# Luckick/EAGCN

Hardware: AMD Instinct MI355X
Metric: molecules/sec fwd+bwd, 2-layer 5-view EAGCN, Tox21 batch (higher is better)
Workload: dtype f32 (bf16x3 split, fp32 accumulate): every fp32 operand leaves its producer as three bf16 planes, six v_mfma_f32_32x32x16_bf16 piece products per 16 k rebuild the fp32 product (csrc/gemm_bx3.hip); aggregation, BatchNorm, head, first layer fp32

## Files before the change

### eagcn_amd/build.py

```python
import os
import shutil
import subprocess
import sys
from concurrent.futures import ThreadPoolExecutor

HERE = os.path.dirname(os.path.abspath(__file__))
CSRC = os.path.join(HERE, 'csrc')
LIBDIR = os.path.join(HERE, 'lib')
LIB = os.path.join(LIBDIR, 'libeagcn_hip.so')
HIP_SOURCES = ['index.hip', 'gemm.hip', 'gemm3.hip', 'gemm_bx3.hip', 'gemm_bx3w.hip', 'agg.hip', 'lagg.hip', 'lagg_in.hip', 'gat.hip', 'pool.hip', 'layer.hip', 'readout.hip', 'head.hip', 'head2.hip', 'loss.hip', 'attr.hip']
CPP_SOURCES = ['api.cpp']
HEADERS = ['common.h', 'kernels.h', 'lagg_kernel.h', 'gemm_x6.h', 'bx3.h', os.path.join('..', '..', 'include', 'eagcn_hip.h')]
ARCH = 'gfx950'


def _hipcc():
    for cand in (shutil.which('hipcc'), '/opt/rocm/bin/hipcc'):
        if cand and os.path.exists(cand):
            return cand
    raise RuntimeError('hipcc not found: the EAGCN HIP library cannot be built')


def _newest(paths):
    return max(os.path.getmtime(p) for p in paths)


def needs_build():
    srcs = [os.path.join(CSRC, s) for s in HIP_SOURCES + CPP_SOURCES + HEADERS if os.path.exists(os.path.join(CSRC, s))]
    return (not os.path.exists(LIB)) or os.path.getmtime(LIB) < _newest(srcs)


def build_library(force=False, verbose=False):
    if not force and not needs_build():
        return LIB
    hipcc = _hipcc()
    os.makedirs(LIBDIR, exist_ok=True)
    objdir = os.path.join(LIBDIR, 'obj')
    os.makedirs(objdir, exist_ok=True)
    flags = ['--offload-arch=' + ARCH, '-O3', '-std=c++17', '-fPIC', '-Wall', '-Wno-unused-function', '-munsafe-fp-atomics']

    hdr_time = _newest([os.path.join(CSRC, h) for h in HEADERS if os.path.exists(os.path.join(CSRC, h))])

    def compile_one(src):
        obj = os.path.join(objdir, os.path.splitext(src)[0] + '.o')
        if not force and os.path.exists(obj) and os.path.getmtime(obj) > max(hdr_time, os.path.getmtime(os.path.join(CSRC, src))):
            return obj
        cmd = [hipcc] + flags + ['-c', os.path.join(CSRC, src), '-o', obj]
        if src.endswith('.cpp'):
            cmd = [hipcc, '-O2', '-std=c++17', '-fPIC', '-c', os.path.join(CSRC, src), '-o', obj]
        r = subprocess.run(cmd, capture_output=True, text=True)
        if r.returncode != 0:
            raise RuntimeError('hipcc failed on %s:\n%s\n%s' % (src, r.stdout, r.stderr))
        if verbose and r.stderr.strip():
            print(r.stderr, file=sys.stderr)
        return obj

    sources = [s for s in HIP_SOURCES + CPP_SOURCES if os.path.exists(os.path.join(CSRC, s))]
    with ThreadPoolExecutor(max_workers=min(8, len(sources))) as ex:
        objs = list(ex.map(compile_one, sources))
    tmp = LIB + '.tmp'
    r = subprocess.run([hipcc, '--offload-arch=' + ARCH, '-shared', '-fPIC', '-o', tmp] + objs,
                       capture_output=True, text=True)
    if r.returncode != 0:
        raise RuntimeError('link failed:\n%s\n%s' % (r.stdout, r.stderr))
    os.replace(tmp, LIB)
    return LIB


if __name__ == '__main__':
    print(build_library(force='--force' in sys.argv, verbose=True))
```

### eagcn_amd/csrc/common.h

```cpp
#pragma once
#include <hip/hip_runtime.h>
#include <stdint.h>
#include <stdio.h>
#include <string.h>

#include "../../include/eagcn_hip.h"

namespace eagcn {

constexpr float TINY = 1e-9f;
constexpr int WAVE = 64;

void set_error(const char* fmt, ...);

#define EAGCN_CHECK_ARG(cond, ...)                 \
    do {                                           \
        if (!(cond)) {                             \
            ::eagcn::set_error(__VA_ARGS__);       \
            return EAGCN_ERR_ARG;                  \
        }                                          \
    } while (0)

#define EAGCN_HIP(call)                                                                   \
    do {                                                                                  \
        hipError_t e_ = (call);                                                           \
        if (e_ != hipSuccess) {                                                           \
            ::eagcn::set_error("%s:%d: %s -> %s", __FILE__, __LINE__, #call,              \
                               hipGetErrorString(e_));                                    \
            return EAGCN_ERR_HIP;                                                         \
        }                                                                                 \
    } while (0)

#define EAGCN_LAUNCH_CHECK() EAGCN_HIP(hipGetLastError())

inline int pad16(int w) { return (w + 15) & ~15; }
inline int pad4(int w) { return (w + 3) & ~3; }
inline int cdiv(int a, int b) { return (a + b - 1) / b; }
inline size_t align256(size_t x) { return (x + 255) & ~size_t(255); }

typedef float f32x4 __attribute__((ext_vector_type(4)));

__device__ __forceinline__ float sigmoidf_(float x) { return 1.0f / (1.0f + __expf(-x)); }

__device__ __forceinline__ float wave_sum(float v) {
#pragma unroll
    for (int o = 32; o > 0; o >>= 1) v += __shfl_xor(v, o);
    return v;
}
__device__ __forceinline__ double wave_sum(double v) {
#pragma unroll
    for (int o = 32; o > 0; o >>= 1) v += __shfl_xor(v, o);
    return v;
}
__device__ __forceinline__ int wave_sum(int v) {
#pragma unroll
    for (int o = 32; o > 0; o >>= 1) v += __shfl_xor(v, o);
    return v;
}
__device__ __forceinline__ int wave_max(int v) {
#pragma unroll
    for (int o = 32; o > 0; o >>= 1) v = max(v, __shfl_xor(v, o));
    return v;
}

constexpr int DOT_U = 10;
__device__ __forceinline__ float dot16(const float* __restrict__ a, const float* __restrict__ b, int sl, int n) {
    float acc = 0.0f;
    for (int c0 = sl; c0 < n; c0 += 16 * DOT_U) {
        float x[DOT_U], y[DOT_U];
#pragma unroll
        for (int u = 0; u < DOT_U; ++u) {
            const int c = c0 + 16 * u;
            const bool ok = c < n;
            x[u] = ok ? a[c] : 0.0f;
            y[u] = ok ? b[c] : 0.0f;
        }
#pragma unroll
        for (int u = 0; u < DOT_U; ++u) acc += x[u] * y[u];
    }
    return acc;
}

__device__ __forceinline__ void dot16x4(const float* __restrict__ a, const float* const (&p)[4], int sl, int n,
                                        float (&out)[4]) {
    out[0] = out[1] = out[2] = out[3] = 0.0f;
    constexpr int U = 5;
    for (int c0 = sl; c0 < n; c0 += 16 * U) {
        float x[U], y[4][U];
#pragma unroll
        for (int u = 0; u < U; ++u) {
            const int c = c0 + 16 * u;
            const bool ok = c < n;
            x[u] = ok ? a[c] : 0.0f;
#pragma unroll
            for (int h = 0; h < 4; ++h) y[h][u] = ok ? p[h][c] : 0.0f;
        }
#pragma unroll
        for (int u = 0; u < U; ++u)
#pragma unroll
            for (int h = 0; h < 4; ++h) out[h] += x[u] * y[h][u];
    }
}

constexpr int DOTV_U = 3;
__device__ __forceinline__ float dot16v(const float* __restrict__ a, const float* __restrict__ b, int sl, int n) {
    const int nf4 = n >> 2;
    float acc = 0.0f;
    for (int c0 = sl; c0 < nf4; c0 += 16 * DOTV_U) {
        float4 x[DOTV_U], y[DOTV_U];
#pragma unroll
        for (int u = 0; u < DOTV_U; ++u) {
            const int c = c0 + 16 * u;
            const bool ok = c < nf4;
            x[u] = ok ? *reinterpret_cast<const float4*>(a + 4 * c) : make_float4(0.f, 0.f, 0.f, 0.f);
            y[u] = ok ? *reinterpret_cast<const float4*>(b + 4 * c) : make_float4(0.f, 0.f, 0.f, 0.f);
        }
#pragma unroll
        for (int u = 0; u < DOTV_U; ++u) acc += (x[u].x * y[u].x + x[u].y * y[u].y) + (x[u].z * y[u].z + x[u].w * y[u].w);
    }
    return acc;
}
__device__ __forceinline__ void dot16x4v(const float* __restrict__ a, const float* const (&p)[4], int sl, int n, float (&out)[4]) {
    const int nf4 = n >> 2;
    out[0] = out[1] = out[2] = out[3] = 0.0f;
    constexpr int U = 2;
    for (int c0 = sl; c0 < nf4; c0 += 16 * U) {
        float4 x[U], y[4][U];
#pragma unroll
        for (int u = 0; u < U; ++u) {
            const int c = c0 + 16 * u;
            const bool ok = c < nf4;
            x[u] = ok ? *reinterpret_cast<const float4*>(a + 4 * c) : make_float4(0.f, 0.f, 0.f, 0.f);
#pragma unroll
            for (int h = 0; h < 4; ++h) y[h][u] = ok ? *reinterpret_cast<const float4*>(p[h] + 4 * c) : make_float4(0.f, 0.f, 0.f, 0.f);
        }
#pragma unroll
        for (int u = 0; u < U; ++u)
#pragma unroll
            for (int h = 0; h < 4; ++h)
                out[h] += (x[u].x * y[h][u].x + x[u].y * y[h][u].y) + (x[u].z * y[h][u].z + x[u].w * y[h][u].w);
    }
}

__device__ __forceinline__ uint32_t rng_u32(uint64_t seed, uint64_t idx) {
    uint64_t z = idx * 0x9E3779B97F4A7C15ull + seed;
    z ^= z >> 32;
    z *= 0xD6E8FEB86659FD93ull;
    z ^= z >> 32;
    z *= 0xD6E8FEB86659FD93ull;
    z ^= z >> 32;
    return (uint32_t)z;
}
__device__ __forceinline__ uint64_t rng_u64(uint64_t seed, uint64_t idx) {
    uint64_t z = idx * 0x9E3779B97F4A7C15ull + seed;
    z ^= z >> 32;
    z *= 0xD6E8FEB86659FD93ull;
    z ^= z >> 32;
    z *= 0xD6E8FEB86659FD93ull;
    z ^= z >> 32;
    return z;
}
constexpr uint64_t PAD_STREAM_BASE = 1ull << 40;
__device__ __forceinline__ float drop_scale(uint64_t seed, uint64_t idx, uint32_t thr, float inv_keep) {
    return rng_u32(seed, idx) >= thr ? inv_keep : 0.0f;
}

__device__ __forceinline__ float drop_scale_el(uint64_t seed, uint64_t idx, uint32_t thr, float inv_keep) {
    const uint64_t z = rng_u64(seed, idx >> 2);
    return ((uint32_t)(z >> (16 * (int)(idx & 3))) & 0xFFFFu) >= (thr >> 16) ? inv_keep : 0.0f;
}
__device__ __forceinline__ void drop_scale4(uint64_t seed, uint64_t idx, uint32_t thr, float inv_keep, float (&out)[4]) {
    const uint64_t z = rng_u64(seed, idx >> 2);
    const uint32_t lo = (uint32_t)z, hi = (uint32_t)(z >> 32), t16 = thr >> 16;
    out[0] = (lo & 0xFFFFu) >= t16 ? inv_keep : 0.0f;
    out[1] = (lo >> 16) >= t16 ? inv_keep : 0.0f;
    out[2] = (hi & 0xFFFFu) >= t16 ? inv_keep : 0.0f;
    out[3] = (hi >> 16) >= t16 ? inv_keep : 0.0f;
}

__device__ __forceinline__ int dev_rows(const eagcn_batch& bt) { return min(bt.meta[EAGCN_META_T], bt.T); }
__device__ __forceinline__ int dev_n(const eagcn_batch& bt) { const int v = bt.meta[EAGCN_META_NLOG]; return v > 0 ? min(v, bt.N) : bt.N; }
__device__ __forceinline__ int dev_tiles(const eagcn_batch& bt) { return min(bt.meta[EAGCN_META_NTILES], bt.n_tiles); }

struct ViewCols {
    int K;
    int off[EAGCN_MAX_VIEWS + 1];
    int width[EAGCN_MAX_VIEWS];
};
inline ViewCols view_cols(const eagcn_layer_params* p) {
    ViewCols v;
    v.K = p->K;
    int o = 0;
    for (int k = 0; k < p->K; ++k) {
        v.off[k] = o;
        v.width[k] = p->width[k];
        o += pad16(p->width[k]);
    }
    for (int k = p->K; k <= EAGCN_MAX_VIEWS; ++k) v.off[k] = o;
    for (int k = p->K; k < EAGCN_MAX_VIEWS; ++k) v.width[k] = 0;
    return v;
}
inline int layout_ld(const eagcn_layout* l) {
    int s = 0;
    for (int i = 0; i < l->nseg; ++i) s += l->pad[i];
    return s;
}
inline int layout_width(const eagcn_layout* l) {
    int s = 0;
    for (int i = 0; i < l->nseg; ++i) s += l->width[i];
    return s;
}

enum ProfTag { PROF_INDEX = 0, PROF_PACK, PROF_GEMM, PROF_AGG, PROF_BN, PROF_EDGE, PROF_READOUT, PROF_HEAD, PROF_GEMM_PAIR,
               PROF_NTAGS };
bool prof_on();
void prof_begin(int tag, hipStream_t s, double work);
void prof_end(int tag, hipStream_t s);
struct ProfScope {
    int tag; hipStream_t s; bool on;
    ProfScope(int t, hipStream_t st, double work = 0.0) : tag(t), s(st), on(prof_on()) { if (on) prof_begin(tag, s, work); }
    ~ProfScope() { if (on) prof_end(tag, s); }
};

hipEvent_t pool_event();
inline int stream_after(hipStream_t waiter, hipStream_t producer) {
    hipEvent_t e = pool_event();
    if (!e) return EAGCN_ERR_HIP;
    if (hipEventRecord(e, producer) != hipSuccess) return EAGCN_ERR_HIP;
    if (hipStreamWaitEvent(waiter, e, 0) != hipSuccess) return EAGCN_ERR_HIP;
    return EAGCN_OK;
}

struct GemmDesc {
    int ta, tb;
    int M, N, K;
    const float* A; int lda;
    const float* B; int ldb;
    float* C; int ldc;
    int splits;
    size_t slab;
    double work = 0.0;
    int vecA = 1, vecB = 1;
    const int* M_dev = nullptr;
    const int* K_dev = nullptr;
    int prof_tag = PROF_GEMM;
};
int launch_gemm(const GemmDesc& g, hipStream_t s);
int launch_gemm_pair(const GemmDesc& dx, const GemmDesc& dw, hipStream_t s);

}
```

### eagcn_amd/csrc/gemm.hip

```cpp
#include <stdlib.h>

#include <algorithm>

#include "common.h"
#include "gemm_x6.h"

namespace eagcn {

constexpr int gemm_lds_floats(int BM, int BN, int BK, bool a_kc, bool b_kc) {
    return 2 * ((a_kc ? BM * (BK + 2) : BK * (BM + 16)) + (b_kc ? BN * (BK + 2) : BK * (BN + 16)));
}

template <int BM, int BN, int BK, bool A_KC, bool B_KC, int D, bool EXT_LDS = false>
__device__ __forceinline__ void gemm_tile(const GemmDesc& g, const int Mx, const int Kx, const int tile_x,
                                          const int tile_y, const int z, const int nsp, float* shared = nullptr) {
    constexpr int WM = BM / 2, WN = BN / 2;
    constexpr int MR = WM / 16, NR = WN / 16;
    constexpr int LDA_S = A_KC ? (BK + 2) : (BM + 16);
    constexpr int LDB_S = B_KC ? (BK + 2) : (BN + 16);
    constexpr int A_SZ = A_KC ? BM * LDA_S : BK * LDA_S;
    constexpr int B_SZ = B_KC ? BN * LDB_S : BK * LDB_S;
    constexpr int A_TPR = A_KC ? BK / 4 : BM / 4;
    constexpr int A_RPP = 256 / A_TPR;
    constexpr int A_PASS = (A_KC ? BM : BK) / A_RPP;
    constexpr int B_TPR = B_KC ? BK / 4 : BN / 4;
    constexpr int B_RPP = 256 / B_TPR;
    constexpr int B_PASS = (B_KC ? BN : BK) / B_RPP;
    static_assert(A_PASS >= 1 && B_PASS >= 1, "tile too small for 256 threads");

    float* smem;
    if constexpr (EXT_LDS) {
        smem = shared;
    } else {
        __shared__ __attribute__((aligned(16))) float own_smem[2 * (A_SZ + B_SZ)];
        smem = own_smem;
    }
    auto kc_row = [](int x) -> int {
        if constexpr (BK == 16) {
            const int g = x >> 2, rs = x & 3;
            return ((g >> 2) << 4) + ((g & 3) << 1) + (rs & 1) + ((rs >> 1) << 3);
        } else {
            return x;
        }
    };
    auto As = [&](int buf) -> float* { return smem + buf * (A_SZ + B_SZ); };
    auto Bs = [&](int buf) -> float* { return smem + buf * (A_SZ + B_SZ) + A_SZ; };

    const int tid = threadIdx.x, lane = tid & 63, wave = tid >> 6;
    const int li = lane & 15, q = lane >> 4;
    const int wm = (wave >> 1) * WM, wn = (wave & 1) * WN;
    const int m0 = tile_y * BM, n0 = tile_x * BN;
    const int kchunk = ((Kx + nsp - 1) / nsp + BK - 1) / BK * BK;
    const int kbeg = z * kchunk;
    const int kend = min(Kx, kbeg + kchunk);
    float* C = g.C + (size_t)z * g.slab;

    float4 ra_[D][A_PASS], rb_[D][B_PASS];
    auto load_tiles = [&](int k0, float4 (&ra)[A_PASS], float4 (&rb)[B_PASS]) {
#pragma unroll
        for (int p = 0; p < A_PASS; ++p) {
            float4 v = make_float4(0.f, 0.f, 0.f, 0.f);
            if constexpr (A_KC) {
                int row = p * A_RPP + kc_row(tid / A_TPR), kq = (tid % A_TPR) * 4;
                if (m0 + row < Mx && k0 + kq < kend) {
                    const float* src = g.A + (size_t)(m0 + row) * g.lda + k0 + kq;
                    if (g.vecA) v = *reinterpret_cast<const float4*>(src);
                    else {
                        v.x = src[0];
                        if (k0 + kq + 1 < kend) v.y = src[1];
                        if (k0 + kq + 2 < kend) v.z = src[2];
                        if (k0 + kq + 3 < kend) v.w = src[3];
                    }
                }
            } else {
                int k = p * A_RPP + tid / A_TPR, mq = (tid % A_TPR) * 4;
                if (k0 + k < kend && m0 + mq < Mx) {
                    const float* src = g.A + (size_t)(k0 + k) * g.lda + m0 + mq;
                    if (g.vecA) v = *reinterpret_cast<const float4*>(src);
                    else {
                        v.x = src[0];
                        if (m0 + mq + 1 < Mx) v.y = src[1];
                        if (m0 + mq + 2 < Mx) v.z = src[2];
                        if (m0 + mq + 3 < Mx) v.w = src[3];
                    }
                }
            }
            ra[p] = v;
        }
#pragma unroll
        for (int p = 0; p < B_PASS; ++p) {
            float4 v = make_float4(0.f, 0.f, 0.f, 0.f);
            if constexpr (B_KC) {
                int row = p * B_RPP + kc_row(tid / B_TPR), kq = (tid % B_TPR) * 4;
                if (n0 + row < g.N && k0 + kq < kend) {
                    const float* src = g.B + (size_t)(n0 + row) * g.ldb + k0 + kq;
                    if (g.vecB) v = *reinterpret_cast<const float4*>(src);
                    else {
                        v.x = src[0];
                        if (k0 + kq + 1 < kend) v.y = src[1];
                        if (k0 + kq + 2 < kend) v.z = src[2];
                        if (k0 + kq + 3 < kend) v.w = src[3];
                    }
                }
            } else {
                int k = p * B_RPP + tid / B_TPR, nq = (tid % B_TPR) * 4;
                if (k0 + k < kend && n0 + nq < g.N) {
                    const float* src = g.B + (size_t)(k0 + k) * g.ldb + n0 + nq;
                    if (g.vecB) v = *reinterpret_cast<const float4*>(src);
                    else {
                        v.x = src[0];
                        if (n0 + nq + 1 < g.N) v.y = src[1];
                        if (n0 + nq + 2 < g.N) v.z = src[2];
                        if (n0 + nq + 3 < g.N) v.w = src[3];
                    }
                }
            }
            rb[p] = v;
        }
    };
    auto store_tiles = [&](int buf, const float4 (&ra)[A_PASS], const float4 (&rb)[B_PASS]) {
#pragma unroll
        for (int p = 0; p < A_PASS; ++p) {
            if constexpr (A_KC) {
                int row = p * A_RPP + kc_row(tid / A_TPR), kq = (tid % A_TPR) * 4;
                float2* d = reinterpret_cast<float2*>(As(buf) + row * LDA_S + kq);
                d[0] = make_float2(ra[p].x, ra[p].y);
                d[1] = make_float2(ra[p].z, ra[p].w);
            } else {
                int k = p * A_RPP + tid / A_TPR, mq = (tid % A_TPR) * 4;
                *reinterpret_cast<float4*>(As(buf) + k * LDA_S + mq) = ra[p];
            }
        }
#pragma unroll
        for (int p = 0; p < B_PASS; ++p) {
            if constexpr (B_KC) {
                int row = p * B_RPP + kc_row(tid / B_TPR), kq = (tid % B_TPR) * 4;
                float2* d = reinterpret_cast<float2*>(Bs(buf) + row * LDB_S + kq);
                d[0] = make_float2(rb[p].x, rb[p].y);
                d[1] = make_float2(rb[p].z, rb[p].w);
            } else {
                int k = p * B_RPP + tid / B_TPR, nq = (tid % B_TPR) * 4;
                *reinterpret_cast<float4*>(Bs(buf) + k * LDB_S + nq) = rb[p];
            }
        }
    };

    f32x4 acc[MR][NR];
#pragma unroll
    for (int i = 0; i < MR; ++i)
#pragma unroll
        for (int j = 0; j < NR; ++j) acc[i][j] = (f32x4){0.f, 0.f, 0.f, 0.f};

    const int nk = (kend > kbeg) ? (kend - kbeg + BK - 1) / BK : 0;
#pragma unroll
    for (int d = 0; d < D; ++d)
        if (d < nk) load_tiles(kbeg + d * BK, ra_[d], rb_[d]);
    if (nk > 0) store_tiles(0, ra_[0], rb_[0]);
    __syncthreads();
    for (int kt0 = 0; kt0 < nk; kt0 += D) {
#pragma unroll
        for (int d = 0; d < D; ++d) {
            const int kt = kt0 + d;
            if (kt < nk) {
                const int cur = kt & 1;
                if (kt + D < nk) load_tiles(kbeg + (kt + D) * BK, ra_[d], rb_[d]);
                const float* a_s = As(cur);
                const float* b_s = Bs(cur);
#pragma unroll
                for (int ks = 0; ks < BK / 4; ++ks) {
                    float af[MR], bf[NR];
#pragma unroll
                    for (int i = 0; i < MR; ++i) {
                        if constexpr (A_KC) af[i] = a_s[(wm + i * 16 + li) * LDA_S + ks * 4 + q];
                        else af[i] = a_s[(ks * 4 + q) * LDA_S + wm + i * 16 + li];
                    }
#pragma unroll
                    for (int j = 0; j < NR; ++j) {
                        if constexpr (B_KC) bf[j] = b_s[(wn + j * 16 + li) * LDB_S + ks * 4 + q];
                        else bf[j] = b_s[(ks * 4 + q) * LDB_S + wn + j * 16 + li];
                    }
#pragma unroll
                    for (int i = 0; i < MR; ++i)
#pragma unroll
                        for (int j = 0; j < NR; ++j)
                            acc[i][j] = __builtin_amdgcn_mfma_f32_16x16x4f32(af[i], bf[j], acc[i][j], 0, 0, 0);
                }
                if (kt + 1 < nk) store_tiles(cur ^ 1, ra_[(d + 1) % D], rb_[(d + 1) % D]);
                __syncthreads();
            }
        }
    }
#pragma unroll
    for (int i = 0; i < MR; ++i)
#pragma unroll
        for (int j = 0; j < NR; ++j) {
            const int col = n0 + wn + j * 16 + li;
#pragma unroll
            for (int r = 0; r < 4; ++r) {
                const int row = m0 + wm + i * 16 + q * 4 + r;
                if (row < Mx && col < g.N) C[(size_t)row * g.ldc + col] = acc[i][j][r];
            }
        }
}

__device__ __forceinline__ int eff_splits(const GemmDesc& g, int Kx) {
    return g.K_dev ? max(1, min(g.splits, Kx >> 7)) : g.splits;
}

__device__ __forceinline__ int xcd_remap(int lin, int nwg) {
    const int xcd = lin & 7, qn = nwg >> 3, rn = nwg & 7;
    return (xcd < rn ? xcd * (qn + 1) : rn * (qn + 1) + (xcd - rn) * qn) + (lin >> 3);
}

template <int BM, int BN, int BK, bool A_KC, bool B_KC, int D, int X6 = 0>
__global__ __launch_bounds__(256) void gemm_f32_kernel(GemmDesc g) {
    const int Mx = g.M_dev ? min(*g.M_dev, g.M) : g.M;
    const int Kx = g.K_dev ? min(*g.K_dev, g.K) : g.K;
    const int nsp = eff_splits(g, Kx);
    int tile_x, tile_y, z;
    {
        const int gx = gridDim.x;
        const int per_z = gx * ((Mx + BM - 1) / BM);
        const int nwg = per_z * nsp;
        if (blockIdx.y * gx + blockIdx.x >= per_z || (int)blockIdx.z >= nsp) return;
        const int lin = blockIdx.z * per_z + blockIdx.y * gx + blockIdx.x;
        const int nid = xcd_remap(lin, nwg);
        z = nid / per_z;
        const int rem = nid - z * per_z;
        tile_y = rem / gx;
        tile_x = rem - tile_y * gx;
    }
    if constexpr (X6 != 0) {
        constexpr int NP = X6 == 2 ? 1 : 3;
        __shared__ __attribute__((aligned(16))) unsigned char x6_smem[x6_lds_bytes(BM, BN, NP)];
        gemm_tile_x6<A_KC, B_KC, BM, BN, NP>(g, Mx, Kx, tile_x, tile_y, z, nsp, x6_smem);
    }
    else gemm_tile<BM, BN, BK, A_KC, B_KC, D>(g, Mx, Kx, tile_x, tile_y, z, nsp);
}

template <int BM, int BN, int BK, int D, int X6 = 0>
__global__ __launch_bounds__(256) void gemm_f32_pair_kernel(GemmDesc g0, GemmDesc g1, int first1) {
    constexpr int F32_LDS = gemm_lds_floats(BM, BN, BK, true, true) > gemm_lds_floats(BM, BN, BK, false, false)
                                ? gemm_lds_floats(BM, BN, BK, true, true) : gemm_lds_floats(BM, BN, BK, false, false);
    constexpr int NP = X6 == 2 ? 1 : 3;
    __shared__ __attribute__((aligned(16))) unsigned char x6_smem[X6 ? x6_lds_bytes(64, 64, NP) : F32_LDS * 4];
    float* f32_smem = reinterpret_cast<float*>(x6_smem);
    const int b = blockIdx.x;
    if (b < first1) {
        const int Mx = g0.M_dev ? min(*g0.M_dev, g0.M) : g0.M;
        const int gx = (g0.N + BN - 1) / BN;
        const int nreal = gx * ((Mx + BM - 1) / BM);
        if (b >= nreal) return;
        const int nid = xcd_remap(b, nreal);
        const int ty = nid / gx;
        if constexpr (X6 != 0) gemm_tile_x6<true, true, 64, 64, NP>(g0, Mx, g0.K, nid - ty * gx, ty, 0, 1, x6_smem);
        else gemm_tile<BM, BN, BK, true, true, D, true>(g0, Mx, g0.K, nid - ty * gx, ty, 0, 1, f32_smem);
    } else {
        const int lin = b - first1;
        const int Kx = g1.K_dev ? min(*g1.K_dev, g1.K) : g1.K;
        const int gx = (g1.N + BN - 1) / BN;
        const int per_z = gx * ((g1.M + BM - 1) / BM);
        const int nsp = eff_splits(g1, Kx);
        const int nwg = per_z * nsp;
        if (lin >= nwg) return;
        const int nid = xcd_remap(lin, nwg);
        const int z = nid / per_z, rem = nid - z * per_z;
        const int ty = rem / gx;
        if constexpr (X6 != 0) gemm_tile_x6<false, false, 64, 64, NP>(g1, g1.M, Kx, rem - ty * gx, ty, z, nsp, x6_smem);
        else gemm_tile<BM, BN, BK, false, false, D, true>(g1, g1.M, Kx, rem - ty * gx, ty, z, nsp, f32_smem);
    }
}


template <int BM, int BN, int BK, int D>
static int launch_cfg(const GemmDesc& g, hipStream_t s) {
    dim3 grid(cdiv(g.N, BN), cdiv(g.M, BM), g.splits);
    ProfScope ps(g.prof_tag, s, g.work > 0.0 ? g.work : 2.0 * g.M * g.N * g.K);
    if (g.ta == 0 && g.tb == 0) gemm_f32_kernel<BM, BN, BK, true, false, D><<<grid, 256, 0, s>>>(g);
    else if (g.ta == 0 && g.tb == 1) gemm_f32_kernel<BM, BN, BK, true, true, D><<<grid, 256, 0, s>>>(g);
    else if (g.ta == 1 && g.tb == 0) gemm_f32_kernel<BM, BN, BK, false, false, D><<<grid, 256, 0, s>>>(g);
    else gemm_f32_kernel<BM, BN, BK, false, true, D><<<grid, 256, 0, s>>>(g);
    EAGCN_LAUNCH_CHECK();
    return EAGCN_OK;
}

static int g_gemm_x6 = [] { const char* e = getenv("EAGCN_GEMM_X6"); return e ? atoi(e) : 3; }();
static int use_x6(const GemmDesc& g) { return ((g_gemm_x6 == 1 || g_gemm_x6 == 2) && g.K >= 64 && g.prof_tag != PROF_HEAD) ? g_gemm_x6 : 0; }
int gemm_mode() { return g_gemm_x6; }
template <int BM, int BN, int X6>
static int launch_x6_cfg(const GemmDesc& g, hipStream_t s) {
    dim3 grid(cdiv(g.N, BN), cdiv(g.M, BM), g.splits);
    ProfScope ps(g.prof_tag, s, g.work > 0.0 ? g.work : 2.0 * g.M * g.N * g.K);
    if (g.ta == 0 && g.tb == 0) gemm_f32_kernel<BM, BN, 16, true, false, 4, X6><<<grid, 256, 0, s>>>(g);
    else if (g.ta == 0 && g.tb == 1) gemm_f32_kernel<BM, BN, 16, true, true, 4, X6><<<grid, 256, 0, s>>>(g);
    else if (g.ta == 1 && g.tb == 0) gemm_f32_kernel<BM, BN, 16, false, false, 4, X6><<<grid, 256, 0, s>>>(g);
    else gemm_f32_kernel<BM, BN, 16, false, true, 4, X6><<<grid, 256, 0, s>>>(g);
    EAGCN_LAUNCH_CHECK();
    return EAGCN_OK;
}
static int launch_x6(const GemmDesc& g, hipStream_t s, int mode) {
    if (mode == 2) return launch_x6_cfg<64, 64, 2>(g, s);
    static const int tile = [] { const char* e = getenv("EAGCN_X6_TILE"); return e ? atoi(e) : 0; }();
    if (tile == 2 && g.M > 64 && g.N > 64) return launch_x6_cfg<128, 128, 1>(g, s);
    if (tile >= 1 && g.M > 64) return launch_x6_cfg<128, 64, 1>(g, s);
    return launch_x6_cfg<64, 64, 1>(g, s);
}

int launch_gemm(const GemmDesc& g0, hipStream_t s) {
    if (g0.M <= 0 || g0.N <= 0) return EAGCN_OK;
    EAGCN_CHECK_ARG(g0.splits >= 1, "gemm: splits must be >= 1");
    GemmDesc g = g0;
    g.vecA = (g.lda % 4) == 0 && ((g.ta ? g.M : g.K) % 4) == 0 && (reinterpret_cast<uintptr_t>(g.A) % 16) == 0;
    g.vecB = (g.ldb % 4) == 0 && ((g.tb ? g.K : g.N) % 4) == 0 && (reinterpret_cast<uintptr_t>(g.B) % 16) == 0;
    if (g.splits > 1) EAGCN_CHECK_ARG(g.vecA && g.vecB, "gemm: split-K needs float4-aligned operands");
    static const int forced = [] { const char* e = getenv("EAGCN_GEMM_CFG"); return e ? atoi(e) : -1; }();
    int cfg = forced;
    if (cfg < 0 && use_x6(g)) return launch_x6(g, s, use_x6(g));
    if (cfg < 0) {
        const long tiles128 = (long)cdiv(g.M, 128) * cdiv(g.N, 128) * g.splits;
        cfg = (g.K >= 1024 && tiles128 >= 512 && g.M > 64 && g.N > 64) ? 3 : 0;
    }
    switch (cfg) {
        case 1: return launch_cfg<64, 64, 32, 3>(g, s);
        case 2: return launch_cfg<64, 64, 16, 2>(g, s);
        case 3: return launch_cfg<128, 128, 16, 3>(g, s);
        case 4: return launch_cfg<64, 64, 16, 6>(g, s);
        case 5: return launch_cfg<64, 64, 16, 1>(g, s);
        default: return launch_cfg<64, 64, 16, 4>(g, s);
    }
}

int launch_gemm_pair(const GemmDesc& dx, const GemmDesc& dw, hipStream_t s) {
    GemmDesc g0 = dx, g1 = dw;
    g0.vecA = (g0.lda % 4) == 0 && (g0.K % 4) == 0 && (reinterpret_cast<uintptr_t>(g0.A) % 16) == 0;
    g0.vecB = (g0.ldb % 4) == 0 && (g0.K % 4) == 0 && (reinterpret_cast<uintptr_t>(g0.B) % 16) == 0;
    g1.vecA = (g1.lda % 4) == 0 && (g1.M % 4) == 0 && (reinterpret_cast<uintptr_t>(g1.A) % 16) == 0;
    g1.vecB = (g1.ldb % 4) == 0 && (g1.N % 4) == 0 && (reinterpret_cast<uintptr_t>(g1.B) % 16) == 0;
    const bool ok = g0.ta == 0 && g0.tb == 1 && g0.splits == 1 && !g0.K_dev && g1.ta == 1 && g1.tb == 0 && !g1.M_dev &&
                    (g1.splits == 1 || (g1.vecA && g1.vecB)) && g0.M > 0 && g0.N > 0 && g1.M > 0 && g1.N > 0;
    if (!ok) {
        int rc = launch_gemm(dw, s);
        return rc ? rc : launch_gemm(dx, s);
    }
    const int first1 = (cdiv(g0.M, 64) * cdiv(g0.N, 64) + 7) / 8 * 8;
    const int n1 = cdiv(g1.M, 64) * cdiv(g1.N, 64) * g1.splits;
    const double w0 = g0.work > 0.0 ? g0.work : 2.0 * g0.M * g0.N * g0.K;
    const double w1 = g1.work > 0.0 ? g1.work : 2.0 * g1.M * g1.N * g1.K;
    ProfScope ps(PROF_GEMM_PAIR, s, w0 + w1);
    if (use_x6(g0) == 2 && use_x6(g1) == 2) gemm_f32_pair_kernel<64, 64, 16, 4, 2><<<first1 + n1, 256, 0, s>>>(g0, g1, first1);
    else if (use_x6(g0) && use_x6(g1)) gemm_f32_pair_kernel<64, 64, 16, 4, 1><<<first1 + n1, 256, 0, s>>>(g0, g1, first1);
    else gemm_f32_pair_kernel<64, 64, 16, 4><<<first1 + n1, 256, 0, s>>>(g0, g1, first1);
    EAGCN_LAUNCH_CHECK();
    return EAGCN_OK;
}

}

using namespace eagcn;

extern "C" int eagcn_set_gemm_mode(int mode) {
    const int old = eagcn::g_gemm_x6;
    eagcn::g_gemm_x6 = mode;
    return old;
}

extern "C" int eagcn_gemm_f32(int ta, int tb, int M, int N, int K, const float* A, int lda, const float* B,
                              int ldb, float* C, int ldc, void* stream) {
    EAGCN_CHECK_ARG(A && B && C, "eagcn_gemm_f32: null operand");
    GemmDesc g{ta, tb, M, N, K, A, lda, B, ldb, C, ldc, 1, 0};
    return launch_gemm(g, (hipStream_t)stream);
}

extern "C" int eagcn_gemm_f32_dev(int ta, int tb, int M, int N, int K, const float* A, int lda, const float* B,
                                  int ldb, float* C, int ldc, const int32_t* extent_dev, int which, void* stream) {
    EAGCN_CHECK_ARG(A && B && C && extent_dev && (which == 0 || which == 2), "eagcn_gemm_f32_dev: bad argument");
    GemmDesc g{ta, tb, M, N, K, A, lda, B, ldb, C, ldc, 1, 0};
    if (which == 0) g.M_dev = extent_dev; else g.K_dev = extent_dev;
    return launch_gemm(g, (hipStream_t)stream);
}
```

### eagcn_amd/csrc/head.hip

```cpp
#include <stdlib.h>

#include <algorithm>

#include "common.h"
#include "kernels.h"

namespace eagcn {

__global__ void wait_counter_kernel(const uint32_t* __restrict__ word, uint32_t value, int* __restrict__ err,
                                    unsigned long long budget_ticks) {
    if (threadIdx.x == 0) {
        const unsigned long long t0 = wall_clock64();
        while ((int32_t)(__hip_atomic_load(word, __ATOMIC_ACQUIRE, __HIP_MEMORY_SCOPE_AGENT) - value) < 0) {
            __builtin_amdgcn_s_sleep(64);
            if (wall_clock64() - t0 > budget_ticks) {
                if (err) __hip_atomic_store(err, 1, __ATOMIC_RELAXED, __HIP_MEMORY_SCOPE_SYSTEM);
                break;
            }
        }
    }
}



static int* g_wait_err_host = nullptr;
static int* g_wait_err_dev = nullptr;
static int* wait_err_word() {
    if (!g_wait_err_dev) {
        void* h = nullptr;
        if (hipHostMalloc(&h, 64, hipHostMallocMapped) != hipSuccess) return nullptr;
        memset(h, 0, 64);
        void* d = nullptr;
        if (hipHostGetDevicePointer(&d, h, 0) != hipSuccess) return nullptr;
        g_wait_err_host = (int*)h;
        g_wait_err_dev = (int*)d;
    }
    return g_wait_err_dev;
}
__global__ void signal_flag_kernel(uint32_t* __restrict__ flag) {
    if (threadIdx.x == 0) __hip_atomic_store(flag, 1u, __ATOMIC_RELEASE, __HIP_MEMORY_SCOPE_AGENT);
}
__global__ void wait_flag_kernel(uint32_t* __restrict__ flag, int* __restrict__ err, unsigned long long budget_ticks) {
    if (threadIdx.x == 0) {
        const unsigned long long t0 = wall_clock64();
        while (__hip_atomic_load(flag, __ATOMIC_ACQUIRE, __HIP_MEMORY_SCOPE_AGENT) == 0u) {
            __builtin_amdgcn_s_sleep(8);
            if (wall_clock64() - t0 > budget_ticks) {
                if (err) __hip_atomic_store(err, 1, __ATOMIC_RELAXED, __HIP_MEMORY_SCOPE_SYSTEM);
                break;
            }
        }
        __hip_atomic_store(flag, 0u, __ATOMIC_RELAXED, __HIP_MEMORY_SCOPE_AGENT);
    }
}
__global__ void handoff_kernel(HandOff h) {
    if (threadIdx.x == 0) handoff_body(h);
}
static int launch_wait_flag(uint32_t* flag, double budget_s, hipStream_t s) {
    wait_flag_kernel<<<1, 64, 0, s>>>(flag, wait_err_word(), (unsigned long long)(budget_s * 1e8));
    EAGCN_LAUNCH_CHECK();
    return EAGCN_OK;
}

struct Carver2 {
    char* base;
    size_t off = 0;
    explicit Carver2(void* p) : base((char*)p) {}
    template <typename T>
    T* take(size_t n) {
        T* p = base ? (T*)(base + off) : nullptr;
        off = align256(off + std::max<size_t>(n, 1) * sizeof(T));
        return p;
    }
};

struct LayerSaved { float *P, *Y, *rscale, *bn, *xout, *pad_row; void* packed; size_t packed_bytes; int fp, ldo, ld_in;
                    uint16_t* xout_planes; };
struct ModelSaved {
    float* x0;
    LayerSaved L[4];
    float *g, *h1, *h2, *bn_g, *bn_1, *bn_2;
    uint16_t* pad_cnt;
    float* padc;
    uint32_t* pad_tab;
    size_t xout_last_off, pad_last_off;
};
static bool pad_sampled(const eagcn_model* m) {
    const eagcn_layer_params* last = &m->layer[m->n_layers - 1];
    return last->structure == EAGCN_STRUCT_WEIGHTED && m->training && last->dropout > 0.0f;
}

static size_t carve_saved(void* base, const eagcn_batch* b, const eagcn_model* m, ModelSaved* out) {
    Carver2 c(base);
    ModelSaved s;
    const size_t T = (size_t)b->T;
    s.x0 = c.take<float>(T * layout_ld(&m->layer[0].in));
    for (int l = 0; l < m->n_layers; ++l) {
        const eagcn_layer_params* p = &m->layer[l];
        LayerSaved& L = s.L[l];
        L.fp = eagcn_layer_fp(p);
        L.ldo = eagcn_layer_out_ld(p);
        L.ld_in = layout_ld(&p->in);
        L.P = c.take<float>(T * L.fp);
        L.Y = c.take<float>(T * L.fp);
        L.rscale = c.take<float>((size_t)p->K * T);
        L.bn = c.take<float>((size_t)4 * L.fp);
        if (l == m->n_layers - 1) s.xout_last_off = c.off;
        L.xout = c.take<float>(T * L.ldo);
        if (l == m->n_layers - 1) s.pad_last_off = c.off;
        L.pad_row = c.take<float>(L.ldo);
        L.packed_bytes = eagcn_layer_packed_bytes(b, p);
        L.packed = c.take<char>(L.packed_bytes);
        const int np = (l + 1 < m->n_layers && L.ldo >= 128 && (L.ldo & 15) == 0) ? gemm_planes() : 0;
        L.xout_planes = np ? c.take<uint16_t>((size_t)np * bx_plane_elems(T, L.ldo)) : nullptr;
    }
    const eagcn_head_params* h = &m->head;
    const size_t B = (size_t)b->B;
    s.g = c.take<float>(B * h->f_in);
    s.h1 = c.take<float>(B * h->n_den1);
    s.h2 = c.take<float>(B * h->n_den2);
    s.bn_g = c.take<float>((size_t)4 * h->f_in);
    s.bn_1 = c.take<float>((size_t)4 * h->n_den1);
    s.bn_2 = c.take<float>((size_t)4 * h->n_den2);
    {
        const eagcn_layer_params* last = &m->layer[m->n_layers - 1];
        const size_t ldo = (size_t)eagcn_layer_out_ld(last);
        const bool need = last->structure == EAGCN_STRUCT_WEIGHTED;
        s.pad_cnt = c.take<uint16_t>(need ? B * last->K * ldo : 1);
        s.padc = c.take<float>(need ? B * ldo : 1);
        const size_t nt = (size_t)(b->N + 1) * (b->N + 1);
        s.pad_tab = c.take<uint32_t>(need ? nt : 1);
    }
    if (out) *out = s;
    return c.off;
}

struct ModelScratch {
    float *da2, *da1, *dgn, *dg, *dxa, *dxb, *dpad;
    float* hdw; int hdw_ks;
    double* hst; int n_hst;
    double* hws;
    double* hsb;
    void* layer; size_t layer_bytes;
};
static size_t carve_scratch(void* base, const eagcn_batch* b, const eagcn_model* m, ModelScratch* out) {
    Carver2 c(base);
    ModelScratch s;
    const eagcn_head_params* h = &m->head;
    const size_t B = (size_t)b->B, T = (size_t)b->T;
    s.n_hst = 2 * (h->f_in + h->n_den1 + h->n_den2) + 6;
    s.hst = c.take<double>((size_t)(HEAD_COPIES + 1) * s.n_hst + HEAD_WS);
    s.hsb = s.hst + (size_t)HEAD_COPIES * s.n_hst;
    s.hws = s.hsb + s.n_hst;
    s.da2 = c.take<float>(B * h->n_den2);
    s.da1 = c.take<float>(B * h->n_den1);
    s.dgn = c.take<float>(B * h->f_in);
    s.dg = c.take<float>(B * h->f_in);
    s.hdw_ks = head_dw_chunks(b->B);
    s.hdw = c.take<float>(s.hdw_ks > 1 ? (size_t)s.hdw_ks * ((size_t)h->f_in * h->n_den1 + (size_t)h->n_den1 * h->n_den2 +
                                                             (size_t)h->n_den2 * h->nclass) : 1);
    int ldmax = 0;
    size_t lbytes = 0;
    for (int l = 0; l < m->n_layers; ++l) {
        ldmax = std::max(ldmax, eagcn_layer_out_ld(&m->layer[l]));
        lbytes = std::max(lbytes, eagcn_layer_fwd_scratch_bytes(b, &m->layer[l]));
        lbytes = std::max(lbytes, eagcn_layer_bwd_scratch_bytes(b, &m->layer[l]));
    }
    s.dxa = c.take<float>(T * ldmax);
    s.dxb = c.take<float>(T * ldmax);
    s.dpad = c.take<float>((size_t)EAGCN_MAX_VIEWS * ldmax);
    s.layer_bytes = lbytes;
    s.layer = c.take<char>(lbytes);
    if (out) *out = s;
    return c.off;
}

static int check_model(const eagcn_batch* b, const eagcn_model* m, const char* who) {
    EAGCN_CHECK_ARG(b && m, "%s: null argument", who);
    EAGCN_CHECK_ARG(m->n_layers >= 1 && m->n_layers <= 4, "%s: n_layers=%d", who, m->n_layers);
    const eagcn_head_params* h = &m->head;
    EAGCN_CHECK_ARG(h->f_in >= 1 && h->n_den1 >= 1 && h->n_den2 >= 1 && h->nclass >= 1, "%s: bad head sizes", who);
    EAGCN_CHECK_ARG(h->den1_w && h->den2_w && h->den3_w && h->gbn_w && h->gbn_b && h->gbn_rm && h->gbn_rv &&
                        h->bn1_w && h->bn1_b && h->bn1_rm && h->bn1_rv && h->bn2_w && h->bn2_b && h->bn2_rm &&
                        h->bn2_rv, "%s: null head parameter", who);
    const eagcn_layer_params* last = &m->layer[m->n_layers - 1];
    const int f_last = last->structure == EAGCN_STRUCT_CONCATE ? [&] { int s = 0; for (int k = 0; k < last->K; ++k) s += last->width[k]; return s; }()
                                                                 : last->width[0];
    EAGCN_CHECK_ARG(f_last == h->f_in, "%s: head expects %d features, last layer yields %d", who, h->f_in, f_last);
    EAGCN_CHECK_ARG(!m->training || b->B > 1, "%s: BatchNorm in training mode needs more than one molecule", who);
    return EAGCN_OK;
}

static eagcn_layout out_layout(const eagcn_layer_params* p) {
    eagcn_layout l;
    memset(&l, 0, sizeof(l));
    if (p->structure == EAGCN_STRUCT_CONCATE) {
        l.nseg = p->K;
        for (int k = 0; k < p->K; ++k) { l.width[k] = p->width[k]; l.pad[k] = pad16(p->width[k]); }
    } else {
        l.nseg = 1;
        l.width[0] = p->width[0];
        l.pad[0] = pad16(p->width[0]);
    }
    return l;
}

static bool fused_readout(const eagcn_model* m) {
    static const bool env = [] { const char* v = getenv("EAGCN_NO_FUSED_READOUT"); return !(v && v[0] == '1'); }();
    return env && m->fuse_readout && m->layer[m->n_layers - 1].structure == EAGCN_STRUCT_CONCATE;
}

static bool hidden_planes_only(const eagcn_batch* b, const eagcn_model* m, const ModelSaved& sv, int l) {
    return l + 1 < m->n_layers && sv.L[l].xout_planes && layer_reads_planes_only(b, &m->layer[l + 1], m->aux_stream != nullptr);
}

static void fill_drop(float p, int training, int* do_drop, uint32_t* thr, float* inv_keep) {
    *do_drop = (training && p > 0.0f) ? 1 : 0;
    *thr = (uint32_t)std::min(4294967295.0, (double)p * 4294967296.0);
    *inv_keep = 1.0f / (1.0f - p);
}

}

using namespace eagcn;

#define RC(call) do { int rc_ = (call); if (rc_) return rc_; } while (0)

extern "C" size_t eagcn_model_saved_bytes(const eagcn_batch* b, const eagcn_model* m) {
    return carve_saved(nullptr, b, m, nullptr);
}
extern "C" size_t eagcn_model_scratch_bytes(const eagcn_batch* b, const eagcn_model* m) {
    return carve_scratch(nullptr, b, m, nullptr);
}
extern "C" int eagcn_model_atom_rep(const eagcn_batch* b, const eagcn_model* m, size_t* xout_offset,
                                    size_t* pad_row_offset, int* ld) {
    EAGCN_CHECK_ARG(b && m && xout_offset && pad_row_offset && ld, "eagcn_model_atom_rep: null argument");
    ModelSaved s;
    carve_saved(nullptr, b, m, &s);
    *xout_offset = s.xout_last_off;
    *pad_row_offset = s.pad_last_off;
    *ld = eagcn_layer_out_ld(&m->layer[m->n_layers - 1]);
    return EAGCN_OK;
}

extern "C" int eagcn_model_atom_rep_materialize(const eagcn_batch* b, const eagcn_model* m, void* saved, size_t saved_bytes,
                                                 void* stream) {
    EAGCN_CHECK_ARG(b && m && saved, "eagcn_model_atom_rep_materialize: null argument");
    if (!fused_readout(m)) return EAGCN_OK;
    ModelSaved sv;
    EAGCN_CHECK_ARG(carve_saved(saved, b, m, &sv) <= saved_bytes, "eagcn_model_atom_rep_materialize: saved block too small");
    const int l = m->n_layers - 1;
    LayerSaved& L = sv.L[l];
    eagcn_layer_bufs w;
    memset(&w, 0, sizeof(w));
    w.Y = L.Y; w.bn = L.bn; w.xout = L.xout; w.pad_row = L.pad_row; w.packed = L.packed; w.packed_bytes = L.packed_bytes;
    return layer_apply_impl(b, &m->layer[l], &w, stream);
}

extern "C" int eagcn_model_pack_input(const eagcn_batch* b, const eagcn_model* m, const float* afm, void* saved,
                                      size_t saved_bytes, void* stream) {
    EAGCN_CHECK_ARG(b && m && afm && saved, "eagcn_model_pack_input: null argument");
    ModelSaved sv;
    EAGCN_CHECK_ARG(carve_saved(saved, b, m, &sv) <= saved_bytes, "eagcn_model_pack_input: saved block too small");
    return eagcn_pack_rows(b, afm, layout_width(&m->layer[0].in), &m->layer[0].in, sv.x0, stream);
}

struct HeadPlan {
    HeadFwd f1, f2, f3;
    HeadBwd b3, b2, b1;
    HeadGbn bg;
    double *st_g, *st_1, *st_2, *sb_g, *sb_1, *sb_2;
    bool sync;
};
static HeadPlan head_plan(const eagcn_batch* b, const eagcn_model* m, const ModelSaved& sv, const ModelScratch& sc, float* out,
                          float* graph_rep, const float* dout, const float* dgraph_rep, const eagcn_head_grads* hg) {
    HeadPlan P;
    const eagcn_head_params* h = &m->head;
    const int B = b->B, F = h->f_in, n1 = h->n_den1, n2 = h->n_den2, nc = h->nclass;
    P.st_g = sc.hst; P.st_1 = sc.hst + 2 * F + 2; P.st_2 = sc.hst + 2 * (F + n1) + 4;
    P.sb_g = sc.hsb; P.sb_1 = sc.hsb + 2 * F + 2; P.sb_2 = sc.hsb + 2 * (F + n1) + 4;
    P.sync = m->stats_hook && m->training;
    const int copies = P.sync ? 1 : HEAD_COPIES;
    HeadDrop nodrop{0, 0u, 1.0f, 0, nullptr}, drop1 = nodrop;
    {
        int on; uint32_t thr; float inv_keep;
        fill_drop(h->dropout, m->training, &on, &thr, &inv_keep);
        drop1 = HeadDrop{on, thr, inv_keep, m->head_seed, m->head_seed_dev};
    }
    P.f1 = HeadFwd{B, F, n1, sv.g, P.st_g, h->gbn_w, h->gbn_b, h->gbn_rm, h->gbn_rv, sv.bn_g, h->den1_w, sv.h1, nullptr, P.st_1,
                   m->training, 0, h->bn_eps, h->bn_momentum, nodrop};
    P.f2 = HeadFwd{B, n1, n2, sv.h1, P.st_1, h->bn1_w, h->bn1_b, h->bn1_rm, h->bn1_rv, sv.bn_1, h->den2_w, sv.h2, graph_rep, P.st_2,
                   m->training, 1, h->bn_eps, h->bn_momentum, drop1};
    P.f3 = HeadFwd{B, n2, nc, sv.h2, P.st_2, h->bn2_w, h->bn2_b, h->bn2_rm, h->bn2_rv, sv.bn_2, h->den3_w, out, nullptr, nullptr,
                   m->training, 1, h->bn_eps, h->bn_momentum, nodrop};
    if (P.sync) { P.f1.cnt_in = P.st_g + 2 * F; P.f2.cnt_in = P.st_1 + 2 * n1; P.f3.cnt_in = P.st_2 + 2 * n2; }
    P.f3.nw = 8;
    P.f1.signal = m->fwd_signal;
    P.f1.st_copies = P.f2.st_copies = P.f3.st_copies = copies;
    P.f1.st_stride = P.f2.st_stride = P.f3.st_stride = sc.n_hst;
    if (!hg) return P;
    const double *cn_g = sc.hst + 2 * F, *cn_1 = sc.hst + 2 * F + 2 + 2 * n1, *cn_2 = sc.hst + 2 * (F + n1) + 4 + 2 * n2;
    const float gscale = P.sync && m->stats_world > 1 ? 1.0f / (float)m->stats_world : 1.0f;
    P.b3 = HeadBwd{B, n2, nc, sv.h2, sv.bn_2, 1, nodrop, h->den3_w, dout, nullptr, nullptr, nullptr, nullptr, nullptr, nullptr,
                   sc.da2, P.sb_2, hg->d_den3_w, m->training};
    P.b2 = HeadBwd{B, n1, n2, sv.h1, sv.bn_1, 1, drop1, h->den2_w, sc.da2, sv.h2, sv.bn_2, P.sb_2, dgraph_rep, hg->d_bn2_w, hg->d_bn2_b,
                   sc.da1, P.sb_1, hg->d_den2_w, m->training};
    P.b1 = HeadBwd{B, F, n1, sv.g, sv.bn_g, 0, nodrop, h->den1_w, sc.da1, sv.h1, sv.bn_1, P.sb_1, nullptr, hg->d_bn1_w, hg->d_bn1_b,
                   sc.dgn, P.sb_g, hg->d_den1_w, m->training};
    if (P.sync) { P.b2.cnt_y = cn_2; P.b2.gscale = gscale; P.b1.cnt_y = cn_1; P.b1.gscale = gscale; }
    P.b3.nw = 8;
    const int ks = sc.hdw_ks;
    float* part3 = sc.hdw;
    float* part2 = part3 + (size_t)ks * n2 * nc;
    float* part1 = part2 + (size_t)ks * n1 * n2;
    if (ks > 1) {
        P.b3.ks = ks; P.b3.dW_part = part3;
        P.b2.ks = ks; P.b2.dW_part = part2;
        P.b1.ks = ks; P.b1.dW_part = part1;
    }
    P.bg = HeadGbn{B, F, sc.dgn, sv.g, sv.bn_g, P.sb_g, sc.dg, hg->d_gbn_w, hg->d_gbn_b, m->training};
    if (P.sync) { P.bg.cnt = cn_g; P.bg.gscale = gscale; }
    if (ks > 1) {
        P.bg.sum[0] = HeadDwSum{hg->d_den3_w, part3, n2 * nc, ks};
        P.bg.sum[1] = HeadDwSum{hg->d_den2_w, part2, n1 * n2, ks};
        P.bg.sum[2] = HeadDwSum{hg->d_den1_w, part1, F * n1, ks};
        P.bg.nsum = 3;
    }
    return P;
}

static int model_forward_trunk(const eagcn_batch* b, const eagcn_model* m, const float* afm, const int64_t* size, void* saved,
                               size_t saved_bytes, void* scratch, size_t scratch_bytes, ModelSaved& sv, ModelScratch& sc,
                               void* stream, const char* who) {
    hipStream_t s = (hipStream_t)stream;
    RC(check_model(b, m, who));
    EAGCN_CHECK_GEMM3(who);
    EAGCN_CHECK_ARG((afm || m->input_packed) && saved && scratch, "%s: null buffer", who);
    EAGCN_CHECK_ARG(m->molfp_mode == 0 || size, "%s: 'ave' read-out needs size", who);
    EAGCN_CHECK_ARG(carve_saved(saved, b, m, &sv) <= saved_bytes, "%s: saved block too small", who);
    EAGCN_CHECK_ARG(carve_scratch(scratch, b, m, &sc) <= scratch_bytes, "%s: scratch too small", who);
    const eagcn_head_params* h = &m->head;
    HandOff ho{m->start_signal, m->wait_flag, wait_err_word(), 200000000ull};
    if (!m->input_packed && (m->wait_flag || m->start_signal)) {
        handoff_kernel<<<1, 64, 0, s>>>(ho);
        EAGCN_LAUNCH_CHECK();
        ho.start = nullptr; ho.flag = nullptr;
    }
    ZeroJob zj;
    RC(gemm3_zero_job(sc.layer, sc.layer_bytes, sc.hst, (HEAD_COPIES + 1) * sc.n_hst + HEAD_WS, &zj));
    if (!m->input_packed)
        RC(eagcn_pack_rows(b, afm, layout_width(&m->layer[0].in), &m->layer[0].in, sv.x0, stream));
    const float* x = sv.x0;
    {
        const eagcn_layer_params* ps[4];
        void* pk[4];
        size_t pkb[4];
        for (int l = 0; l < m->n_layers; ++l) { ps[l] = &m->layer[l]; pk[l] = sv.L[l].packed; pkb[l] = sv.L[l].packed_bytes; }
        RC(pack_params_all(b, ps, pk, pkb, m->n_layers, stream, &zj, &ho));
    }
    for (int l = 0; l < m->n_layers; ++l) {
        LayerSaved& L = sv.L[l];
        eagcn_layer_bufs w;
        memset(&w, 0, sizeof(w));
        w.x = x; w.P = L.P; w.Y = L.Y; w.rscale = L.rscale; w.bn = L.bn; w.xout = L.xout; w.pad_row = L.pad_row;
        w.scratch = sc.layer; w.scratch_bytes = sc.layer_bytes; w.packed = L.packed; w.packed_bytes = L.packed_bytes;
        w.stats_hook = m->stats_hook; w.stats_user = m->stats_user;
        w.x_planes = l > 0 ? sv.L[l - 1].xout_planes : nullptr; w.xout_planes = L.xout_planes;
        const bool po = hidden_planes_only(b, m, sv, l);
        RC(layer_forward_impl(b, &m->layer[l], &w, stream, true, l == m->n_layers - 1 && fused_readout(m), po));
        x = po ? nullptr : L.xout;
    }
    const eagcn_layer_params* last = &m->layer[m->n_layers - 1];
    const LayerSaved& LL = sv.L[m->n_layers - 1];
    const eagcn_layout lay = out_layout(last);
    const int B = b->B, F = h->f_in, n1 = h->n_den1, n2 = h->n_den2;
    double *st_g = sc.hst, *st_1 = sc.hst + 2 * F + 2, *st_2 = sc.hst + 2 * (F + n1) + 4;
    const int copies = (m->stats_hook && m->training) ? 1 : HEAD_COPIES;
    if (fused_readout(m)) {
        ReadoutBn rb;
        rb.Y = LL.Y; rb.ldy = LL.fp; rb.bn = LL.bn; rb.fp = LL.fp;
        fill_drop(last->dropout, last->training, &rb.do_drop, &rb.thr, &rb.inv_keep);
        rb.seed = last->seed; rb.seed_dev = last->seed_dev;
        rb.size = size; rb.mode = m->molfp_mode; rb.g = sv.g; rb.F = F; rb.st = st_g;
        rb.cnt0 = st_g + 2 * F; rb.cnt1 = st_1 + 2 * n1; rb.cnt2 = st_2 + 2 * n2;
        rb.st_copies = copies; rb.st_stride = sc.n_hst;
        RC(readout_bn_forward(b, &lay, rb, stream));
    } else if (pad_sampled(m))
        RC(readout_forward_sampled(b, LL.xout, &lay, last, LL.bn + (size_t)LL.fp , size,
                                   m->molfp_mode, sv.g, F, sv.pad_cnt, sv.padc, sv.pad_tab, stream));
    else
        RC(eagcn_readout_forward(b, LL.xout, &lay, last->structure == EAGCN_STRUCT_WEIGHTED ? LL.pad_row : nullptr,
                                 size, m->molfp_mode, sv.g, F, stream));
    if (!fused_readout(m)) RC(head_colstats(sv.g, B, F, st_g, s, st_g + 2 * F, st_1 + 2 * n1, st_2 + 2 * n2));
    return EAGCN_OK;
}

static int stats_hook_call(const eagcn_model* m, bool sync, double* buf, int n, void* stream) {
    if (!sync) return EAGCN_OK;
    if (m->stats_hook(buf, n, stream, m->stats_user)) {
        set_error("eagcn_model: the sync-BatchNorm all-reduce hook failed");
        return EAGCN_ERR_HIP;
    }
    return EAGCN_OK;
}

static int head_forward_launches(const eagcn_model* m, const HeadPlan& P, void* stream) {
    hipStream_t s = (hipStream_t)stream;
    const eagcn_head_params* h = &m->head;
    RC(stats_hook_call(m, P.sync, P.st_g, 2 * h->f_in + 1, stream));
    RC(head_fwd(P.f1, s));
    RC(stats_hook_call(m, P.sync, P.st_1, 2 * h->n_den1 + 1, stream));
    RC(head_fwd(P.f2, s));
    RC(stats_hook_call(m, P.sync, P.st_2, 2 * h->n_den2 + 1, stream));
    RC(head_fwd(P.f3, s));
    return EAGCN_OK;
}
static int head_backward_launches(const eagcn_model* m, const HeadPlan& P, void* stream) {
    hipStream_t s = (hipStream_t)stream;
    const eagcn_head_params* h = &m->head;
    RC(head_bwd(P.b3, s));
    RC(stats_hook_call(m, P.sync, P.sb_2, 2 * h->n_den2, stream));
    RC(head_bwd(P.b2, s));
    RC(stats_hook_call(m, P.sync, P.sb_1, 2 * h->n_den1, stream));
    RC(head_bwd(P.b1, s));
    RC(stats_hook_call(m, P.sync, P.sb_g, 2 * h->f_in, stream));
    RC(head_gbn_bwd(P.bg, s));
    return EAGCN_OK;
}
static int readout_pad_backward(const eagcn_batch* b, const eagcn_model* m, const int64_t* size, const ModelSaved& sv,
                                const ModelScratch& sc, void* stream) {
    const eagcn_layer_params* last = &m->layer[m->n_layers - 1];
    const eagcn_layout lay = out_layout(last);
    const int F = m->head.f_in;
    if (pad_sampled(m)) return readout_backward_pad_views(b, sc.dg, &lay, size, m->molfp_mode, F, last->K, sv.pad_cnt, last->dropout, sc.dpad, stream);
    if (last->structure == EAGCN_STRUCT_WEIGHTED) return readout_backward_pad(b, sc.dg, &lay, size, m->molfp_mode, F, sc.dpad, stream);
    return EAGCN_OK;
}

extern "C" int eagcn_model_forward(const eagcn_batch* b, const eagcn_model* m, const float* afm,
                                   const int64_t* size, void* saved, size_t saved_bytes, void* scratch,
                                   size_t scratch_bytes, float* out, float* graph_rep, void* stream) {
    EAGCN_CHECK_ARG(out && graph_rep, "eagcn_model_forward: null buffer");
    ModelSaved sv;
    ModelScratch sc;
    RC(model_forward_trunk(b, m, afm, size, saved, saved_bytes, scratch, scratch_bytes, sv, sc, stream, "eagcn_model_forward"));
    const HeadPlan P = head_plan(b, m, sv, sc, out, graph_rep, nullptr, nullptr, nullptr);
    return head_forward_launches(m, P, stream);
}

namespace eagcn {
static int check_head(const eagcn_head_params* h, int B, int training, const char* who) {
    EAGCN_CHECK_ARG(h, "%s: null argument", who);
    EAGCN_CHECK_ARG(B >= 1 && h->f_in >= 1 && h->n_den1 >= 1 && h->n_den2 >= 1 && h->nclass >= 1, "%s: bad head sizes", who);
    EAGCN_CHECK_ARG(h->den1_w && h->den2_w && h->den3_w && h->gbn_w && h->gbn_b && h->gbn_rm && h->gbn_rv && h->bn1_w && h->bn1_b &&
                        h->bn1_rm && h->bn1_rv && h->bn2_w && h->bn2_b && h->bn2_rm && h->bn2_rv, "%s: null head parameter", who);
    EAGCN_CHECK_ARG(!training || B > 1, "%s: BatchNorm in training mode needs more than one molecule", who);
    return EAGCN_OK;
}
static size_t carve_head_saved(void* base, const eagcn_head_params* h, int B, ModelSaved* out) {
    Carver2 c(base);
    ModelSaved s;
    memset(&s, 0, sizeof(s));
    s.h1 = c.take<float>((size_t)B * h->n_den1);
    s.h2 = c.take<float>((size_t)B * h->n_den2);
    s.bn_g = c.take<float>((size_t)4 * h->f_in);
    s.bn_1 = c.take<float>((size_t)4 * h->n_den1);
    s.bn_2 = c.take<float>((size_t)4 * h->n_den2);
    if (out) *out = s;
    return c.off;
}
static size_t carve_head_scratch(void* base, const eagcn_head_params* h, int B, ModelScratch* out) {
    Carver2 c(base);
    ModelScratch s;
    memset(&s, 0, sizeof(s));
    s.n_hst = 2 * (h->f_in + h->n_den1 + h->n_den2) + 6;
    s.hst = c.take<double>((size_t)(HEAD_COPIES + 1) * s.n_hst + HEAD_WS);
    s.hsb = s.hst + (size_t)HEAD_COPIES * s.n_hst;
    s.hws = s.hsb + s.n_hst;
    s.da2 = c.take<float>((size_t)B * h->n_den2);
    s.da1 = c.take<float>((size_t)B * h->n_den1);
    s.dgn = c.take<float>((size_t)B * h->f_in);
    s.hdw_ks = head_dw_chunks(B);
    s.hdw = c.take<float>(s.hdw_ks > 1 ? (size_t)s.hdw_ks * ((size_t)h->f_in * h->n_den1 + (size_t)h->n_den1 * h->n_den2 +
                                                             (size_t)h->n_den2 * h->nclass) : 1);
    if (out) *out = s;
    return c.off;
}
__global__ __launch_bounds__(256) void head_zero_kernel(double* __restrict__ p, int n) {
    for (int i = blockIdx.x * blockDim.x + threadIdx.x; i < n; i += gridDim.x * blockDim.x) p[i] = 0.0;
}
static int head_zero(double* p, size_t n, hipStream_t s) {
    head_zero_kernel<<<(unsigned)std::max<size_t>(1, std::min<size_t>((n + 255) / 256, 64)), 256, 0, s>>>(p, (int)n);
    EAGCN_LAUNCH_CHECK();
    return EAGCN_OK;
}
static void head_alone_model(const eagcn_head_params* h, int B, int training, uint64_t seed, const uint64_t* seed_dev,
                             eagcn_batch* b, eagcn_model* m) {
    memset(b, 0, sizeof(*b));
    memset(m, 0, sizeof(*m));
    b->B = B;
    m->head = *h; m->training = training ? 1 : 0; m->head_seed = seed; m->head_seed_dev = seed_dev;
}
}

extern "C" size_t eagcn_head_saved_bytes(const eagcn_head_params* h, int B) { return h ? carve_head_saved(nullptr, h, B, nullptr) : 0; }
extern "C" size_t eagcn_head_scratch_bytes(const eagcn_head_params* h, int B) { return h ? carve_head_scratch(nullptr, h, B, nullptr) : 0; }

extern "C" int eagcn_head_forward(const eagcn_head_params* h, int B, int training, uint64_t seed, const uint64_t* seed_dev,
                                  const float* g, void* saved, size_t saved_bytes, void* scratch, size_t scratch_bytes, float* out,
                                  float* graph_rep, void* stream) {
    hipStream_t s = (hipStream_t)stream;
    RC(check_head(h, B, training, "eagcn_head_forward"));
    EAGCN_CHECK_GEMM3("eagcn_head_forward");
    EAGCN_CHECK_ARG(g && saved && scratch && out && graph_rep, "eagcn_head_forward: null buffer");
    ModelSaved sv;
    ModelScratch sc;
    EAGCN_CHECK_ARG(carve_head_saved(saved, h, B, &sv) <= saved_bytes, "eagcn_head_forward: saved block too small");
    EAGCN_CHECK_ARG(carve_head_scratch(scratch, h, B, &sc) <= scratch_bytes, "eagcn_head_forward: scratch too small");
    eagcn_batch b;
    eagcn_model m;
    head_alone_model(h, B, training, seed, seed_dev, &b, &m);
    sv.g = const_cast<float*>(g);
    const int F = h->f_in, n1 = h->n_den1, n2 = h->n_den2;
    RC(head_zero(sc.hst, (size_t)(HEAD_COPIES + 1) * sc.n_hst + HEAD_WS, s));
    double *st_g = sc.hst, *st_1 = sc.hst + 2 * F + 2, *st_2 = sc.hst + 2 * (F + n1) + 4;
    RC(head_colstats(g, B, F, st_g, s, st_g + 2 * F, st_1 + 2 * n1, st_2 + 2 * n2));
    const HeadPlan P = head_plan(&b, &m, sv, sc, out, graph_rep, nullptr, nullptr, nullptr);
    return head_forward_launches(&m, P, stream);
}

extern "C" int eagcn_head_backward(const eagcn_head_params* h, int B, int training, uint64_t seed, const uint64_t* seed_dev,
                                   const float* g, void* saved, size_t saved_bytes, void* scratch, size_t scratch_bytes,
                                   const float* dout, const float* dgraph_rep, const eagcn_head_grads* hg, float* dg, void* stream) {
    hipStream_t s = (hipStream_t)stream;
    RC(check_head(h, B, training, "eagcn_head_backward"));
    EAGCN_CHECK_GEMM3("eagcn_head_backward");
    EAGCN_CHECK_ARG(g && saved && scratch && dout && hg && dg, "eagcn_head_backward: null buffer");
    EAGCN_CHECK_ARG(hg->d_den1_w && hg->d_den2_w && hg->d_den3_w && hg->d_gbn_w && hg->d_gbn_b && hg->d_bn1_w && hg->d_bn1_b &&
                        hg->d_bn2_w && hg->d_bn2_b, "eagcn_head_backward: null head gradient");
    ModelSaved sv;
    ModelScratch sc;
    EAGCN_CHECK_ARG(carve_head_saved(saved, h, B, &sv) <= saved_bytes, "eagcn_head_backward: saved block too small");
    EAGCN_CHECK_ARG(carve_head_scratch(scratch, h, B, &sc) <= scratch_bytes, "eagcn_head_backward: scratch too small");
    eagcn_batch b;
    eagcn_model m;
    head_alone_model(h, B, training, seed, seed_dev, &b, &m);
    sv.g = const_cast<float*>(g);
    sc.dg = dg;
    RC(head_zero(sc.hsb, (size_t)sc.n_hst, s));
    const HeadPlan P = head_plan(&b, &m, sv, sc, nullptr, nullptr, dout, dgraph_rep, hg);
    return head_backward_launches(&m, P, stream);
}

namespace eagcn {
__global__ void scale_loss_kernel(float* __restrict__ loss, float* __restrict__ dout, int n, const float* __restrict__ scale) {
    const float sc = *scale;
    const int i = blockIdx.x * blockDim.x + threadIdx.x;
    if (i < n) dout[i] *= sc;
    if (i == 0) loss[0] *= sc;
}
}

extern "C" int eagcn_model_forward_step(const eagcn_batch* b, const eagcn_model* m, const float* afm, const int64_t* size,
                                        void* saved, size_t saved_bytes, void* scratch, size_t scratch_bytes, float* out,
                                        float* graph_rep, const eagcn_step_loss* loss, const float* dgraph_rep,
                                        const eagcn_head_grads* hg, void* stream) {
    hipStream_t s = (hipStream_t)stream;
    EAGCN_CHECK_ARG(out && graph_rep && loss && hg, "eagcn_model_forward_step: null argument");
    EAGCN_CHECK_ARG(m && m->training, "eagcn_model_forward_step: a training-mode model is required");
    EAGCN_CHECK_ARG((loss->kind == 0 || loss->kind == 1) && loss->labels && loss->loss && loss->dout && (loss->kind == 1 || loss->class_weight),
                    "eagcn_model_forward_step: bad loss descriptor");
    EAGCN_CHECK_ARG(hg->d_den1_w && hg->d_den2_w && hg->d_den3_w && hg->d_gbn_w && hg->d_gbn_b && hg->d_bn1_w &&
                        hg->d_bn1_b && hg->d_bn2_w && hg->d_bn2_b, "eagcn_model_forward_step: null head gradient");
    ModelSaved sv;
    ModelScratch sc;
    RC(model_forward_trunk(b, m, afm, size, saved, saved_bytes, scratch, scratch_bytes, sv, sc, stream, "eagcn_model_forward_step"));
    const HeadPlan P = head_plan(b, m, sv, sc, out, graph_rep, loss->dout, dgraph_rep, hg);
    const eagcn_head_params* h = &m->head;
    if (!P.sync && head_mid_ok(h->n_den2, h->nclass)) {
        HeadPlan Q = P;
        unsigned* words = reinterpret_cast<unsigned*>(sc.hws);
        if (loss->kind == 0) { Q.f2.lab = loss->labels; Q.f2.nlab = b->B * h->nclass; Q.f2.lab_cnt = words + 1; }
        RC(head_fwd(Q.f1, s));
        RC(head_fwd(Q.f2, s));
        HeadMid M;
        M.f3 = Q.f3; M.b3 = Q.b3;
        M.L = HeadLoss{loss->kind, loss->labels, loss->class_weight, loss->loss, loss->scale, loss->dout};
        M.ws = sc.hws;
        RC(head_mid(M, s));
        RC(head_bwd_pair(Q.b2, Q.b3, HeadLossFin{loss->loss, sc.hws, loss->scale, loss->kind, b->B * h->nclass}, s));
        RC(head_bwd(Q.b1, s));
        RC(head_gbn_bwd(Q.bg, s));
    } else {
        RC(head_forward_launches(m, P, stream));
        if (loss->kind == 0) RC(eagcn_bce_loss(out, loss->labels, loss->class_weight, b->B, h->nclass, loss->loss, loss->dout, stream));
        else RC(eagcn_mse_loss(out, loss->labels, b->B * h->nclass, loss->loss, loss->dout, stream));
        if (loss->scale) {
            const int n = b->B * h->nclass;
            scale_loss_kernel<<<cdiv(n, 256), 256, 0, s>>>(loss->loss, loss->dout, n, loss->scale);
            EAGCN_LAUNCH_CHECK();
        }
        RC(head_backward_launches(m, P, stream));
    }
    return readout_pad_backward(b, m, size, sv, sc, stream);
}

extern "C" int eagcn_model_backward(const eagcn_batch* b, const eagcn_model* m, const int64_t* size, void* saved,
                                    size_t saved_bytes, void* scratch, size_t scratch_bytes, const float* dout,
                                    const float* dgraph_rep, const eagcn_layer_grads* lg,
                                    const eagcn_head_grads* hg, void* stream) {
    EAGCN_CHECK_ARG(m, "eagcn_model_backward: null model");
    return eagcn_model_backward_range(b, m, size, saved, saved_bytes, scratch, scratch_bytes, dout, dgraph_rep, lg, hg, 1,
                                      m->n_layers - 1, 0, stream);
}

static int model_backward_impl(const eagcn_batch* b, const eagcn_model* m, const int64_t* size, void* saved, size_t saved_bytes,
                               void* scratch, size_t scratch_bytes, const float* dout, const float* dgraph_rep,
                               const eagcn_layer_grads* lg, const eagcn_head_grads* hg, int with_head, int layer_hi, int layer_lo,
                               float* dx0, bool input_only, void* stream) {
    hipStream_t s = (hipStream_t)stream;
    EAGCN_CHECK_ARG(saved && scratch && dout && (lg || input_only) && hg, "eagcn_model_backward: null buffer");
    EAGCN_CHECK_ARG(hg->d_den1_w && hg->d_den2_w && hg->d_den3_w && hg->d_gbn_w && hg->d_gbn_b && hg->d_bn1_w &&
                        hg->d_bn1_b && hg->d_bn2_w && hg->d_bn2_b, "eagcn_model_backward: null head gradient");
    EAGCN_CHECK_ARG(layer_hi < m->n_layers && layer_lo >= 0 && layer_lo <= layer_hi + 1,
                    "eagcn_model_backward_range: layers %d..%d of %d", layer_hi, layer_lo, m->n_layers);
    EAGCN_CHECK_ARG(!with_head || layer_hi == m->n_layers - 1 || layer_hi < layer_lo,
                    "eagcn_model_backward_range: the head's backward is followed by the top layer");
    ModelSaved sv;
    ModelScratch sc;
    EAGCN_CHECK_ARG(carve_saved(saved, b, m, &sv) <= saved_bytes, "eagcn_model_backward: saved block too small");
    EAGCN_CHECK_ARG(carve_scratch(scratch, b, m, &sc) <= scratch_bytes, "eagcn_model_backward: scratch too small");
    const int F = m->head.f_in;
    const ZeroJob zb{nullptr, 0, sc.hsb, sc.n_hst};
    hipStream_t side = m->aux_stream ? (hipStream_t)m->aux_stream : s;
    const bool forked = side != s;
    const eagcn_layer_params* last = &m->layer[m->n_layers - 1];
    const eagcn_layout lay = out_layout(last);
    const bool weighted = last->structure == EAGCN_STRUCT_WEIGHTED;
    const bool sampled = pad_sampled(m);
    if (with_head) {
        const HeadPlan P = head_plan(b, m, sv, sc, nullptr, nullptr, dout, dgraph_rep, hg);
        RC(head_backward_launches(m, P, stream));
        if (!(input_only && !m->training)) RC(readout_pad_backward(b, m, size, sv, sc, stream));
    }
    ReadoutGrad rgd;
    memset(&rgd, 0, sizeof(rgd));
    rgd.dg = sc.dg; rgd.F = F; rgd.size = size; rgd.mode = m->molfp_mode; rgd.map = make_colmap(&lay);
    const int top_l = m->n_layers - 1;
    EdgeDrain pend_in, pend_out;
    pend_in.eacc = nullptr;
    pend_out.eacc = nullptr;
    for (int l = layer_hi; l >= layer_lo; --l) {
        const int t = top_l - l;
        float* cur = (t & 1) ? sc.dxb : sc.dxa;
        float* other = (t & 1) ? sc.dxa : sc.dxb;
        LayerSaved& L = sv.L[l];
        eagcn_layer_bufs w;
        memset(&w, 0, sizeof(w));
        w.x = l == 0 ? sv.x0 : (hidden_planes_only(b, m, sv, l - 1) ? nullptr : sv.L[l - 1].xout);
        w.P = L.P; w.Y = L.Y; w.rscale = L.rscale; w.bn = L.bn; w.xout = L.xout; w.pad_row = L.pad_row;
        w.scratch = sc.layer; w.scratch_bytes = sc.layer_bytes; w.packed = L.packed; w.packed_bytes = L.packed_bytes;
        w.aux_stream = m->aux_stream;
        w.stats_hook = m->stats_hook; w.stats_user = m->stats_user;
        w.x_planes = l > 0 ? sv.L[l - 1].xout_planes : nullptr;
        const bool top = l == top_l;
        const float* dpad = (weighted && top) ? sc.dpad : nullptr;
        RC(layer_backward_impl(b, &m->layer[l], &w, top ? nullptr : cur, top ? &rgd : nullptr, dpad,
                               l > 0 ? other : dx0, input_only ? nullptr : &lg[l], stream, top && sampled, top ? &zb : nullptr,
                               pend_in.eacc ? &pend_in : nullptr, (l > layer_lo && !input_only) ? &pend_out : nullptr, input_only));
        pend_in = pend_out;
        if (l == layer_lo) pend_in.eacc = nullptr;
    }
    if (forked) RC(stream_after(s, side));
    return EAGCN_OK;
}

extern "C" int eagcn_model_backward_range(const eagcn_batch* b, const eagcn_model* m, const int64_t* size, void* saved,
                                          size_t saved_bytes, void* scratch, size_t scratch_bytes, const float* dout,
                                          const float* dgraph_rep, const eagcn_layer_grads* lg,
                                          const eagcn_head_grads* hg, int with_head, int layer_hi, int layer_lo, void* stream) {
    RC(check_model(b, m, "eagcn_model_backward"));
    EAGCN_CHECK_GEMM3("eagcn_model_backward");
    return model_backward_impl(b, m, size, saved, saved_bytes, scratch, scratch_bytes, dout, dgraph_rep, lg, hg, with_head, layer_hi,
                               layer_lo, nullptr, false, stream);
}

struct InputScratch { float* dx0; eagcn_head_grads hg; };
static size_t carve_input_scratch(void* base, const eagcn_batch* b, const eagcn_model* m, InputScratch* out) {
    Carver2 c(base);
    c.off = carve_scratch(nullptr, b, m, nullptr);
    InputScratch t;
    const eagcn_head_params* h = &m->head;
    const size_t F = h->f_in, n1 = h->n_den1, n2 = h->n_den2, nc = h->nclass;
    t.dx0 = c.take<float>((size_t)std::max(b->T, 1) * layout_ld(&m->layer[0].in));
    t.hg.d_den1_w = c.take<float>(F * n1);
    t.hg.d_den2_w = c.take<float>(n1 * n2);
    t.hg.d_den3_w = c.take<float>(n2 * nc);
    t.hg.d_gbn_w = c.take<float>(F);
    t.hg.d_gbn_b = c.take<float>(F);
    t.hg.d_bn1_w = c.take<float>(n1);
    t.hg.d_bn1_b = c.take<float>(n1);
    t.hg.d_bn2_w = c.take<float>(n2);
    t.hg.d_bn2_b = c.take<float>(n2);
    if (out) *out = t;
    return c.off;
}

static int check_engine_model(const eagcn_batch* b, const eagcn_model* m, const char* who) {
    RC(check_model(b, m, who));
    EAGCN_CHECK_ARG(m->molfp_mode == 0 || m->molfp_mode == 1, "%s: read-out mode %d has no engine path", who, m->molfp_mode);
    for (int l = 0; l < m->n_layers; ++l)
        EAGCN_CHECK_ARG(m->layer[l].structure == EAGCN_STRUCT_CONCATE || m->layer[l].structure == EAGCN_STRUCT_WEIGHTED,
                        "%s: layer %d has structure %d, which the engine does not run", who, l, m->layer[l].structure);
    return EAGCN_OK;
}

int eagcn::model_backward_input_packed(const eagcn_batch* b, const eagcn_model* m, const int64_t* size, void* saved, size_t saved_bytes,
                                       void* scratch, size_t scratch_bytes, const float* dout, const float* dgraph_rep,
                                       const eagcn_layer_grads* lg, const eagcn_head_grads* hg, float** dx0, void* stream,
                                       const char* who) {
    EAGCN_CHECK_ARG(b && m, "%s: null argument", who);
    EAGCN_CHECK_ARG((lg == nullptr) == (hg == nullptr), "%s: lg and hg are both given (full backward) or both NULL (input-only)", who);
    RC(check_engine_model(b, m, who));
    EAGCN_CHECK_GEMM3(who);
    EAGCN_CHECK_ARG(saved && scratch && dout, "%s: null buffer", who);
    InputScratch is;
    EAGCN_CHECK_ARG(carve_input_scratch(scratch, b, m, &is) <= scratch_bytes, "%s: scratch too small (eagcn_model_input_scratch_bytes)", who);
    *dx0 = is.dx0;
    const bool input_only = lg == nullptr;
    return model_backward_impl(b, m, size, saved, saved_bytes, scratch, scratch_bytes, dout, dgraph_rep, lg, input_only ? &is.hg : hg, 1,
                               m->n_layers - 1, 0, is.dx0, input_only, stream);
}

int eagcn::model_input_slot(const eagcn_batch* b, const eagcn_model* m, void* saved, size_t saved_bytes, float** x0, const char* who) {
    ModelSaved sv;
    EAGCN_CHECK_ARG(carve_saved(saved, b, m, &sv) <= saved_bytes, "%s: saved block too small", who);
    *x0 = sv.x0;
    return EAGCN_OK;
}

extern "C" size_t eagcn_model_input_scratch_bytes(const eagcn_batch* b, const eagcn_model* m) {
    return (b && m) ? carve_input_scratch(nullptr, b, m, nullptr) : 0;
}

extern "C" int eagcn_model_backward_input(const eagcn_batch* b, const eagcn_model* m, const int64_t* size, void* saved,
                                          size_t saved_bytes, void* scratch, size_t scratch_bytes, const float* dout,
                                          const float* dgraph_rep, const eagcn_layer_grads* lg, const eagcn_head_grads* hg,
                                          float* dafm, void* stream) {
    EAGCN_CHECK_ARG(dafm, "eagcn_model_backward_input: null dafm");
    float* dx0 = nullptr;
    RC(model_backward_input_packed(b, m, size, saved, saved_bytes, scratch, scratch_bytes, dout, dgraph_rep, lg, hg, &dx0, stream,
                                   "eagcn_model_backward_input"));
    return launch_attr_dense(b, &m->layer[0].in, dx0, nullptr, nullptr, dafm, nullptr, (hipStream_t)stream);
}

extern "C" int eagcn_stream_signal_flag(uint32_t* flag, void* stream) {
    EAGCN_CHECK_ARG(flag != nullptr, "eagcn_stream_signal_flag: null flag");
    eagcn::signal_flag_kernel<<<1, 64, 0, (hipStream_t)stream>>>(flag);
    EAGCN_LAUNCH_CHECK();
    return EAGCN_OK;
}
extern "C" int eagcn_stream_wait_flag(uint32_t* flag, double budget_seconds, void* stream) {
    EAGCN_CHECK_ARG(flag != nullptr && budget_seconds > 0.0, "eagcn_stream_wait_flag: null flag / no budget");
    return eagcn::launch_wait_flag(flag, budget_seconds, (hipStream_t)stream);
}
extern "C" int eagcn_stream_wait_timeouts(void) {
    return eagcn::g_wait_err_host ? __atomic_load_n(eagcn::g_wait_err_host, __ATOMIC_RELAXED) : 0;
}
extern "C" void eagcn_stream_wait_reset(void) {
    if (eagcn::g_wait_err_host) __atomic_store_n(eagcn::g_wait_err_host, 0, __ATOMIC_RELAXED);
}

extern "C" int eagcn_stream_wait_counter(const uint32_t* counter, uint32_t value, void* stream) {
    EAGCN_CHECK_ARG(counter != nullptr, "eagcn_stream_wait_counter: null counter");
    eagcn::wait_counter_kernel<<<1, 64, 0, (hipStream_t)stream>>>(counter, value, eagcn::wait_err_word(), 200000000ull);
    EAGCN_LAUNCH_CHECK();
    return EAGCN_OK;
}
```

### eagcn_amd/csrc/kernels.h

```cpp
#pragma once
#include "bx3.h"
#include "common.h"

namespace eagcn {

struct AggArgs {
    eagcn_batch bt;
    ViewCols vc;
    const float* src; int lds;
    float* dst; int ldd;
    const float* sig;
    const float* rsig;
    float* rscale;
    double* stats;
    int nchunk;
    int cpw = 1;
    int xcd = 0;
    bool w_rowm = false;
    BxOut planes = {nullptr, 0, 0, 0};
    const float* bn_tab = nullptr; const float* bn_cc = nullptr; int bn_fp = 0;
    const float* w_aw = nullptr;
    int w_drop = 0; uint32_t w_thr = 0; float w_inv_keep = 1.0f; uint64_t w_seed = 0; const uint64_t* w_seed_dev = nullptr;
};
int agg_grid_x(const eagcn_batch* b);
bool agg_ksplit(const eagcn_batch* b);
int launch_agg(AggArgs a, bool trans, hipStream_t s);
constexpr int LAGG_RB = 256;
constexpr int LAGG_MAXM = 16;
struct EdgeArgs;
int lagg_parts();
bool lagg_wfuse();
bool lagg_use(const eagcn_batch* b, int dir, bool absorbs_bn, const ViewCols* vc = nullptr);
bool lagg_wanted(int B, int N, int structure);
int lagg_block_rows(const eagcn_batch* b);
int lagg_slabs(const eagcn_batch* b);
int launch_lagg_fwd(AggArgs a, hipStream_t s);
int launch_lagg_bwd(AggArgs a, const EdgeArgs& e, hipStream_t s, bool edge = true);
int launch_lagg_bwd_input(const AggArgs& a, const EdgeArgs& e, dim3 grid, hipStream_t s);

struct EdgeArgs {
    eagcn_batch bt;
    ViewCols vc;
    const float* dY; const float* Y; const float* P; int ld;
    const float* sig; const float* rsig; const float* rscale;
    double* datt;
    int atomic;
    int xcd = 0;
};
constexpr int EDGE_SLAB = 264;
constexpr int EDGE_COPIES = 8;
inline size_t edge_acc_bytes() { return align256((size_t)EDGE_COPIES * EAGCN_MAX_VIEWS * EDGE_SLAB * sizeof(double)); }
int edge_grid_x(const eagcn_batch* b);
int launch_edge_grad(const EdgeArgs& a, hipStream_t s);
int launch_agg_edge(AggArgs a, const EdgeArgs& e, hipStream_t s);

enum { BN_SC = 0, BN_SH, BN_MU, BN_INV };

struct ColMapD {
    int nseg;
    int w[EAGCN_MAX_SEGS], p[EAGCN_MAX_SEGS];
};
inline ColMapD make_colmap(const eagcn_layout* l) {
    ColMapD m;
    m.nseg = l->nseg;
    for (int i = 0; i < EAGCN_MAX_SEGS; ++i) {
        m.w[i] = i < l->nseg ? l->width[i] : 0;
        m.p[i] = i < l->nseg ? l->pad[i] : 0;
    }
    return m;
}

struct ReadoutGrad {
    const float* dg; int F;
    const int64_t* size; int mode;
    ColMapD map;
};
int launch_readout_bwd_rows(const eagcn_batch* b, const ReadoutGrad& rg, int ld, float* dx, hipStream_t s);
struct G2Prob {
    const float* A; const float* B; float* C;
    int lda, ldb, ldc;
    int M, N, K;
    const int* M_dev;
    const int* K_dev;
};
struct DwScatter {
    float* dW[EAGCN_MAX_VIEWS];
    ViewCols vc;
    ColMapD in;
    int in_identity;
};
constexpr int G3_XSEG = 8;
struct G3Plan {
    int a[G3_XSEG + 1];
    int c[G3_XSEG + 1];
};
__host__ __device__ inline void g3_plan(int RB, int CT0, int ipt0, int T1, int ipt1, int G, G3Plan& pl) {
    const long total = (long)RB * CT0 * ipt0 + (long)T1 * ipt1;
    const int R = 4 * G;
    const long per = total / R, rem = total - per * R;
    const int qn = G >> 3, rn = G & 7;
    pl.a[0] = 0;
    pl.c[0] = 0;
    for (int x = 1; x < G3_XSEG; ++x) {
        const long L = 4L * (x * qn + (x < rn ? x : rn));
        const long tgt = L * per + (L < rem ? L : rem);
        int a = (int)(((long)RB * L + R / 2) / R);
        a = a < pl.a[x - 1] ? pl.a[x - 1] : (a > RB ? RB : a);
        long cc = T1 > 0 ? (tgt - (long)a * CT0 * ipt0 + T1 / 2) / T1 : 0;
        if (tgt - (long)a * CT0 * ipt0 < 0) cc = 0;
        int c = (int)(cc > ipt1 ? ipt1 : cc);
        c = c < pl.c[x - 1] ? pl.c[x - 1] : c;
        pl.a[x] = a;
        pl.c[x] = c;
    }
    pl.a[G3_XSEG] = RB;
    pl.c[G3_XSEG] = ipt1;
}
size_t gemm3_workspace_bytes();
bool gemm3_xk_enabled();
int gemm3_grid();
int gemm3_clear_flags(void* workspace, size_t bytes, hipStream_t s, double* zero = nullptr, int nzero = 0);
int gemm3_failed();
#define EAGCN_CHECK_GEMM3(who)                                                                                         \
    do {                                                                                                               \
        if (::eagcn::gemm3_failed()) {                                                                                 \
            ::eagcn::set_error("%s: a stream-K hand-off of an earlier GEMM launch timed out (a contributor wave was not " \
                               "co-resident with its owner): that launch's results are NaN-poisoned; call "           \
                               "eagcn_gemm_sk_reset_failed() after fixing the cause (EAGCN_GEMM3_WGS, concurrent work)", who); \
            return EAGCN_ERR_HIP;                                                                                      \
        }                                                                                                              \
    } while (0)
int gemm_mode();
inline int gemm_planes() { const int m = gemm_mode(); return m == 3 ? 3 : m == 4 ? 1 : 0; }
struct ZeroJob { unsigned* u; int nu; double* d; int nd; };
struct HandOff { uint32_t* start; uint32_t* flag; int* err; unsigned long long budget; };
__device__ __forceinline__ void handoff_body(const HandOff& h) {
    if (h.start) __hip_atomic_fetch_add(h.start, 1u, __ATOMIC_RELEASE, __HIP_MEMORY_SCOPE_AGENT);
    if (h.flag) {
        const unsigned long long t0 = wall_clock64();
        while (__hip_atomic_load(h.flag, __ATOMIC_ACQUIRE, __HIP_MEMORY_SCOPE_AGENT) == 0u) {
            __builtin_amdgcn_s_sleep(8);
            if (wall_clock64() - t0 > h.budget) {
                if (h.err) __hip_atomic_store(h.err, 1, __ATOMIC_RELAXED, __HIP_MEMORY_SCOPE_SYSTEM);
                break;
            }
        }
        __hip_atomic_store(h.flag, 0u, __ATOMIC_RELAXED, __HIP_MEMORY_SCOPE_AGENT);
    }
}
int gemm3_zero_job(void* workspace, size_t bytes, double* zero, int nzero, ZeroJob* out);
int zero_fill(void* p, size_t bytes, hipStream_t s);
bool gemm3_ok(const GemmDesc& g);
int launch_gemm3(const GemmDesc& g, const DwScatter* sc, void* workspace, size_t bytes, hipStream_t s);
int launch_gemm3_pair(const GemmDesc& dx, const GemmDesc& dw, const DwScatter* sc, void* workspace, size_t bytes, hipStream_t s,
                      size_t xk_slab = 0);

constexpr int HEAD_COPIES = 8;
struct HeadDrop { int on; uint32_t thr; float inv_keep; uint64_t seed; const uint64_t* seed_dev; };
struct HeadFwd {
    int B, K, N;
    const float* x; const double* st_in; const float *gamma, *beta; float *run_mean, *run_var; float* bn;
    const float* W; float* y; float* y2; double* st_out;
    int training, relu; float eps, momentum; HeadDrop drop;
    const double* cnt_in = nullptr;
    int st_copies = 1, st_stride = 0;
    const float* lab = nullptr; int nlab = 0; unsigned* lab_cnt = nullptr;
    int nw = 0;
    uint32_t* signal = nullptr;
};
struct HeadBwd {
    int B, K, N;
    const float* x; const float* bnp; int relu_p; HeadDrop drop; const float* W;
    const float* dy; const float* y; const float* bny; const double* sb_y; const float* extra;
    float *dgamma_y, *dbeta_y; float* dyp; double* sb_p; float* dW; int training;
    const double* cnt_y = nullptr;
    float gscale = 1.0f;
    int ks = 1; float* dW_part = nullptr;
    int nw = 0;
};
inline int head_dw_chunks(int B) { return B > 256 ? (B + 255) / 256 < 16 ? (B + 255) / 256 : 16 : 1; }
struct HeadDwSum { float* dst; const float* part; int n, ks; };
struct HeadGbn { int B, F; const float *dgn, *g, *bn; const double* sb; float *dg, *dgamma, *dbeta; int training;
                 const double* cnt = nullptr; float gscale = 1.0f;
                 HeadDwSum sum[3] = {}; int nsum = 0; };
struct HeadLoss { int kind;
                  const float* labels; const float* weight; float* loss; const float* scale; float* dout; };
struct HeadMid { HeadFwd f3; HeadBwd b3; HeadLoss L;
                 double* ws; };
constexpr int HEAD_WS = 4;
struct HeadLossFin { float* loss; const double* ws; const float* scale; int kind, n; };
bool head_mid_ok(int n_den2, int nclass);
int head_mid(const HeadMid& a, hipStream_t s);
int head_bwd_pair(const HeadBwd& a, const HeadBwd& e, const HeadLossFin& lf, hipStream_t s);
int head_colstats(const float* g, int B, int F, double* st, hipStream_t s, double* cnt0 = nullptr, double* cnt1 = nullptr,
                  double* cnt2 = nullptr);
int head_fwd(const HeadFwd& a, hipStream_t s);
int head_bwd(const HeadBwd& a, hipStream_t s);
int head_gbn_bwd(const HeadGbn& a, hipStream_t s);

struct EdgeDrain {
    double* eacc; int K;
    float* datt_w[EAGCN_MAX_VIEWS]; float* dself_r[EAGCN_MAX_VIEWS]; int channels[EAGCN_MAX_VIEWS];
    const float* rsig;
};
int layer_backward_impl(const eagcn_batch* b, const eagcn_layer_params* p, const eagcn_layer_bufs* w,
                        const float* dxout, const ReadoutGrad* rg, const float* dpad_row, float* dx,
                        const eagcn_layer_grads* g, void* stream, bool dpad_views = false,
                        const ZeroJob* zero_after = nullptr, const EdgeDrain* drain_in = nullptr, EdgeDrain* drain_out = nullptr,
                        bool input_only = false);
int model_backward_input_packed(const eagcn_batch* b, const eagcn_model* m, const int64_t* size, void* saved, size_t saved_bytes,
                                void* scratch, size_t scratch_bytes, const float* dout, const float* dgraph_rep,
                                const eagcn_layer_grads* lg, const eagcn_head_grads* hg, float** dx0, void* stream, const char* who);
int launch_attr_dense(const eagcn_batch* b, const eagcn_layout* in, const float* acc, const float* x, const float* base, float* attr,
                      float* score, hipStream_t s);
int model_input_slot(const eagcn_batch* b, const eagcn_model* m, void* saved, size_t saved_bytes, float** x0, const char* who);
int layer_forward_impl(const eagcn_batch* b, const eagcn_layer_params* p, const eagcn_layer_bufs* w, void* stream,
                       bool prepacked, bool skip_apply = false, bool planes_only = false);
bool layer_reads_planes_only(const eagcn_batch* b, const eagcn_layer_params* p, bool aux_stream);
int layer_apply_impl(const eagcn_batch* b, const eagcn_layer_params* p, const eagcn_layer_bufs* w, void* stream);
int pack_params_all(const eagcn_batch* b, const eagcn_layer_params* const* ps, void* const* packed,
                    const size_t* packed_bytes, int n, void* stream, const ZeroJob* zj = nullptr, const HandOff* ho = nullptr);
struct ReadoutBn {
    const float* Y; int ldy;
    const float* bn; int fp;
    int do_drop; uint32_t thr; float inv_keep; uint64_t seed; const uint64_t* seed_dev;
    const int64_t* size; int mode;
    float* g; int F;
    double* st;
    int st_copies = 1, st_stride = 0;
    bool pair = false;
    double *cnt0, *cnt1, *cnt2;
};
int readout_bn_forward(const eagcn_batch* b, const eagcn_layout* lay, const ReadoutBn& a, void* stream);
int readout_forward_sampled(const eagcn_batch* b, const float* x, const eagcn_layout* lay, const eagcn_layer_params* p,
                            const float* bn_sh, const int64_t* size, int mode, float* g, int F, uint16_t* cnt, float* padc,
                            uint32_t* tab, void* stream);
int readout_backward_pad_views(const eagcn_batch* b, const float* dg, const eagcn_layout* lay, const int64_t* size, int mode,
                               int F, int K, const uint16_t* cnt, float dropout, float* dpad, void* stream);
int readout_backward_pad(const eagcn_batch* b, const float* dg, const eagcn_layout* lay, const int64_t* size,
                         int mode, int F, float* dpad_row, void* stream);

}
```

### eagcn_amd/csrc/layer.hip

```cpp
#include <algorithm>

#include <stdlib.h>

#include "common.h"
#include "kernels.h"

namespace eagcn {

struct ParamPtrs {
    const float* att_w[EAGCN_MAX_VIEWS];
    const float* self_r[EAGCN_MAX_VIEWS];
    const float* W[EAGCN_MAX_VIEWS];
    const float* bias[EAGCN_MAX_VIEWS];
    const float* gamma[EAGCN_MAX_VIEWS];
    const float* beta[EAGCN_MAX_VIEWS];
    float* run_mean[EAGCN_MAX_VIEWS];
    float* run_var[EAGCN_MAX_VIEWS];
    const float* ave_w;
    int channels[EAGCN_MAX_VIEWS];
    const float* rel_vec[EAGCN_MAX_VIEWS];
    int rel_c[EAGCN_MAX_VIEWS];
};
__device__ __forceinline__ float att_logit(const ParamPtrs& pp, int k, int c) {
    if (!pp.rel_vec[k]) return pp.att_w[k][c - 1];
    const float* v = pp.rel_vec[k] + (size_t)(c - 1) * pp.rel_c[k];
    float s = 0.0f;
    for (int ch = 0; ch < pp.rel_c[k]; ++ch) s = fmaf(pp.att_w[k][ch], v[ch], s);
    return s;
}
struct GradPtrs {
    float* dW[EAGCN_MAX_VIEWS];
    float* dbias[EAGCN_MAX_VIEWS];
    float* dgamma[EAGCN_MAX_VIEWS];
    float* dbeta[EAGCN_MAX_VIEWS];
    float* datt_w[EAGCN_MAX_VIEWS];
    float* dself_r[EAGCN_MAX_VIEWS];
    float* dave_w;
};

enum { CP_GAMMA = 0, CP_BETA, CP_BIAS, CP_RMEAN, CP_RVAR, CP_AVEW, CP_ROWS = 8 };

__device__ __forceinline__ int col_view(const ViewCols& vc, int cp) {
    int k = 0;
#pragma unroll
    for (int v = 1; v < EAGCN_MAX_VIEWS; ++v) k += (v < vc.K && cp >= vc.off[v]) ? 1 : 0;
    return k;
}
__device__ __forceinline__ int packed_to_exact(const ColMapD& m, int cp) {
    int eo = 0, po = 0;
    for (int s = 0; s < m.nseg; ++s) {
        if (cp < po + m.p[s]) return (cp - po < m.w[s]) ? eo + (cp - po) : -1;
        eo += m.w[s];
        po += m.p[s];
    }
    return -1;
}

__device__ __forceinline__ void pack_params_body(const ParamPtrs& pp, const ViewCols& vc, const ColMapD& in, int ld_in,
                                                 int fp, float* __restrict__ Wcat, float* __restrict__ WcatT,
                                                 float* __restrict__ colp, float* __restrict__ sig, float* __restrict__ rsig,
                                                 const BxOut wp = BxOut{nullptr, 0, 0, 0}, const BxOut wtp = BxOut{nullptr, 0, 0, 0}) {
    __shared__ float tile[32][33];
    const int tx = threadIdx.x & 31, ty = threadIdx.x >> 5;
    const int ntx = (fp + 31) >> 5, nty = (ld_in + 31) >> 5;
    for (int t = blockIdx.x; t < ntx * nty; t += gridDim.x) {
        const int ip0 = (t / ntx) << 5, cp0 = (t % ntx) << 5;
        {
            const int cp = cp0 + tx;
            const int k = cp < fp ? col_view(vc, cp) : 0;
            const int f = cp - vc.off[k];
#pragma unroll
            for (int j = 0; j < 4; ++j) {
                const int ip = ip0 + ty + 8 * j;
                float v = 0.0f;
                if (ip < ld_in && cp < fp) {
                    const int fi = packed_to_exact(in, ip);
                    if (fi >= 0 && f < vc.width[k]) v = pp.W[k][(size_t)fi * vc.width[k] + f];
                    Wcat[(size_t)ip * fp + cp] = v;
                }
                tile[ty + 8 * j][tx] = v;
            }
        }
        __syncthreads();
#pragma unroll
        for (int j = 0; j < 4; ++j) {
            const int cp = cp0 + ty + 8 * j, ip = ip0 + tx;
            if (cp < fp && ip < ld_in) WcatT[(size_t)cp * ld_in + ip] = tile[tx][ty + 8 * j];
        }
        if (wp.p) {
            const int r = threadIdx.x >> 3, c4 = (threadIdx.x & 7) << 2;
            if (ip0 + r < ld_in && cp0 + c4 < fp)
                bx_store4(wp, ip0 + r, cp0 + c4, make_float4(tile[r][c4], tile[r][c4 + 1], tile[r][c4 + 2], tile[r][c4 + 3]));
            if (cp0 + r < fp && ip0 + c4 < ld_in)
                bx_store4(wtp, cp0 + r, ip0 + c4, make_float4(tile[c4][r], tile[c4 + 1][r], tile[c4 + 2][r], tile[c4 + 3][r]));
        }
        __syncthreads();
    }
    for (int cp = blockIdx.x * blockDim.x + threadIdx.x; cp < fp; cp += gridDim.x * blockDim.x) {
        const int k = col_view(vc, cp), f = cp - vc.off[k];
        const bool ok = f < vc.width[k];
        colp[CP_GAMMA * fp + cp] = ok ? pp.gamma[k][f] : 0.0f;
        colp[CP_BETA * fp + cp] = ok ? pp.beta[k][f] : 0.0f;
        colp[CP_BIAS * fp + cp] = ok ? pp.bias[k][f] : 0.0f;
        colp[CP_RMEAN * fp + cp] = ok ? pp.run_mean[k][f] : 0.0f;
        colp[CP_RVAR * fp + cp] = ok ? pp.run_var[k][f] : 1.0f;
        colp[CP_AVEW * fp + cp] = pp.ave_w ? pp.ave_w[k] : 1.0f;
    }
    for (int e = blockIdx.x * blockDim.x + threadIdx.x; e < vc.K * 256; e += gridDim.x * blockDim.x) {
        const int k = e >> 8, c = e & 255;
        sig[e] = (c >= 1 && c <= pp.channels[k]) ? sigmoidf_(att_logit(pp, k, c)) : 0.0f;
    }
    if (blockIdx.x == 0 && threadIdx.x < vc.K) rsig[threadIdx.x] = sigmoidf_(pp.self_r[threadIdx.x][0]);
}
__global__ __launch_bounds__(256) void pack_params_kernel(ParamPtrs pp, ViewCols vc, ColMapD in, int ld_in, int fp,
                                                           float* __restrict__ Wcat, float* __restrict__ WcatT,
                                                           float* __restrict__ colp, float* __restrict__ sig,
                                                           float* __restrict__ rsig, BxOut wp, BxOut wtp) {
    pack_params_body(pp, vc, in, ld_in, fp, Wcat, WcatT, colp, sig, rsig, wp, wtp);
}
struct PackJob {
    ParamPtrs pp; ViewCols vc; ColMapD in; int ld_in, fp;
    float *Wcat, *WcatT, *colp, *sig, *rsig;
    BxOut wp, wtp;
};
struct PackJobs { PackJob j0, j1, j2, j3; };
__global__ __launch_bounds__(256) void pack_params_multi_kernel(PackJobs jobs, ZeroJob zj, HandOff ho) {
    if (blockIdx.y == 0) {
        for (int i = blockIdx.x * blockDim.x + threadIdx.x; i < max(zj.nu, zj.nd); i += gridDim.x * blockDim.x) {
            if (i < zj.nu) zj.u[i] = 0u;
            if (i < zj.nd) zj.d[i] = 0.0;
        }
    }
    if (blockIdx.y == 0) pack_params_body(jobs.j0.pp, jobs.j0.vc, jobs.j0.in, jobs.j0.ld_in, jobs.j0.fp, jobs.j0.Wcat, jobs.j0.WcatT, jobs.j0.colp, jobs.j0.sig, jobs.j0.rsig, jobs.j0.wp, jobs.j0.wtp);
    else if (blockIdx.y == 1) pack_params_body(jobs.j1.pp, jobs.j1.vc, jobs.j1.in, jobs.j1.ld_in, jobs.j1.fp, jobs.j1.Wcat, jobs.j1.WcatT, jobs.j1.colp, jobs.j1.sig, jobs.j1.rsig, jobs.j1.wp, jobs.j1.wtp);
    else if (blockIdx.y == 2) pack_params_body(jobs.j2.pp, jobs.j2.vc, jobs.j2.in, jobs.j2.ld_in, jobs.j2.fp, jobs.j2.Wcat, jobs.j2.WcatT, jobs.j2.colp, jobs.j2.sig, jobs.j2.rsig, jobs.j2.wp, jobs.j2.wtp);
    else pack_params_body(jobs.j3.pp, jobs.j3.vc, jobs.j3.in, jobs.j3.ld_in, jobs.j3.fp, jobs.j3.Wcat, jobs.j3.WcatT, jobs.j3.colp, jobs.j3.sig, jobs.j3.rsig, jobs.j3.wp, jobs.j3.wtp);
    if (blockIdx.x == 0 && blockIdx.y == 0 && threadIdx.x == 0) handoff_body(ho);
}

template <int L>
__device__ __forceinline__ void slab_sum(const double* __restrict__ slab, int nslab, int fp, int cp, int sl,
                                           double& s1, double& s2) {
    s1 = 0.0;
    s2 = 0.0;
    for (int s0 = sl; s0 < nslab; s0 += L * 8) {
        double2 v[8];
#pragma unroll
        for (int u = 0; u < 8; ++u) {
            const int s = s0 + L * u;
            v[u] = s < nslab ? *reinterpret_cast<const double2*>(slab + ((size_t)s * fp + cp) * 2) : make_double2(0.0, 0.0);
        }
#pragma unroll
        for (int u = 0; u < 8; ++u) { s1 += v[u].x; s2 += v[u].y; }
    }
#pragma unroll
    for (int o = L / 2; o > 0; o >>= 1) {
        s1 += __shfl_xor(s1, o);
        s2 += __shfl_xor(s2, o);
    }
}

constexpr int BWD_ROWS = 7;
template <int L>
__global__ __launch_bounds__(256) void bn_stats_sum_kernel(const double* __restrict__ slab, int nslab, int fp, double M,
                                                            double* __restrict__ out, const int32_t* __restrict__ meta,
                                                            int mode, int tiles_per_wg, int nvirt, int batch_B) {
    if (meta[EAGCN_META_NLOG] > 0) M = (double)batch_B * (double)meta[EAGCN_META_NLOG];
    if (mode == 1 && tiles_per_wg > 0) nslab = min(nslab, (meta[EAGCN_META_NTILES] + tiles_per_wg - 1) / tiles_per_wg);
    if (mode == 1 && tiles_per_wg < 0) nslab = min(nslab, meta[EAGCN_META_NBLK]);
    if (mode == 2) nslab = max(1, min(nslab, (meta[EAGCN_META_T] + nvirt + BWD_ROWS - 1) / BWD_ROWS));
    const int cpr = blockIdx.x * (256 / L) + threadIdx.x / L, sl = threadIdx.x % L;
    const int cp = min(cpr, fp - 1);
    double s1, s2;
    slab_sum<L>(slab, nslab, fp, cp, sl, s1, s2);
    if (cpr < fp && sl == 0) { out[2 * cp] = s1; out[2 * cp + 1] = s2; }
    if (blockIdx.x == 0 && threadIdx.x == 0) out[2 * fp] = M;
}

template <int L>
__global__ __launch_bounds__(256) void bn_finalize_kernel(const double* __restrict__ slab, int nslab, int fp,
                                                           double M, int training, float eps, float momentum,
                                                           const float* __restrict__ colp, ParamPtrs pp,
                                                           ViewCols vc, float* __restrict__ bn,
                                                           const int32_t* __restrict__ meta, int tiles_per_wg, int batch_B,
                                                           const double* __restrict__ M_dev) {
    if (meta[EAGCN_META_NLOG] > 0) M = (double)batch_B * (double)meta[EAGCN_META_NLOG];
    if (M_dev) M = *M_dev;
    if (tiles_per_wg > 0) nslab = min(nslab, (meta[EAGCN_META_NTILES] + tiles_per_wg - 1) / tiles_per_wg);
    if (tiles_per_wg < 0) nslab = min(nslab, meta[EAGCN_META_NBLK]);
    const int cpr = blockIdx.x * (256 / L) + threadIdx.x / L, sl = threadIdx.x % L;
    const int cp = min(cpr, fp - 1);
    double s1 = 0.0, s2 = 0.0;
    if (training) slab_sum<L>(slab, nslab, fp, cp, sl, s1, s2);
    if (cpr >= fp || sl != 0) return;
    const int k = col_view(vc, cp), f = cp - vc.off[k];
    const float gamma = colp[CP_GAMMA * fp + cp], beta = colp[CP_BETA * fp + cp];
    const float bias = colp[CP_BIAS * fp + cp];
    float mu, inv;
    if (training) {
        const double mean = s1 / M;
        double var = s2 / M - mean * mean;
        var = var > 0.0 ? var : 0.0;
        mu = (float)mean;
        inv = (float)(1.0 / sqrt(var + (double)eps));
        if (f < vc.width[k]) {
            const double unbiased = var * (M / (M - 1.0));
            pp.run_mean[k][f] = (float)((1.0 - momentum) * (double)colp[CP_RMEAN * fp + cp] + momentum * (mean + (double)bias));
            pp.run_var[k][f] = (float)((1.0 - momentum) * (double)colp[CP_RVAR * fp + cp] + momentum * unbiased);
        }
    } else {
        mu = colp[CP_RMEAN * fp + cp] - bias;
        inv = 1.0f / sqrtf(colp[CP_RVAR * fp + cp] + eps);
    }
    const float sc = gamma * inv;
    bn[BN_SC * fp + cp] = sc;
    bn[BN_SH * fp + cp] = beta - mu * sc;
    bn[BN_MU * fp + cp] = mu;
    bn[BN_INV * fp + cp] = inv;
}

struct ApplyArgs {
    eagcn_batch bt;
    ViewCols vc;
    int structure, fp;
    const float* Y; int ldy;
    const float* bn;
    const float* colp;
    float* out; int ldo;
    float* pad_row;
    int do_drop; uint32_t thr; float inv_keep; uint64_t seed; const uint64_t* seed_dev;
    BxOut planes;
    int tile_map;
};

__global__ __launch_bounds__(256) void bn_apply_kernel(ApplyArgs a) {
    const int fp = a.fp;
    const uint64_t seed = a.seed_dev ? *a.seed_dev : a.seed;
    if (blockIdx.x == 0) {
        for (int c = threadIdx.x; c < a.ldo; c += blockDim.x) {
            float v = 0.0f;
            if (a.structure == EAGCN_STRUCT_WEIGHTED)
                for (int k = 0; k < a.vc.K; ++k) {
                    const int cp = a.vc.off[k] + c;
                    v += a.colp[CP_AVEW * fp + cp] * fmaxf(a.bn[BN_SH * fp + cp], 0.0f);
                }
            a.pad_row[c] = v;
        }
    }
    const int T = dev_rows(a.bt);
    if (a.structure == EAGCN_STRUCT_CONCATE) {
        const uint32_t g4 = a.tile_map ? ((uint32_t)(fp + 31) >> 5) : fp / 4;
        const uint32_t total = a.tile_map ? (((uint32_t)T + 7) >> 3) * g4 * 64u : (uint32_t)T * g4;
        for (uint32_t e = blockIdx.x * blockDim.x + threadIdx.x; e < total; e += gridDim.x * blockDim.x) {
            int r, c;
            if (a.tile_map) {
                const uint32_t it = e >> 6, rg = it / g4;
                r = (int)(rg * 8u + ((e >> 3) & 7u)); c = (int)((it - rg * g4) * 32u + (e & 7u) * 4u);
                if (r >= T || c >= fp) continue;
            } else {
                r = (int)(e / g4); c = (int)(e - (uint32_t)r * g4) * 4;
            }
            const float4 y = *reinterpret_cast<const float4*>(a.Y + (size_t)r * a.ldy + c);
            const float4 sc = *reinterpret_cast<const float4*>(a.bn + BN_SC * fp + c);
            const float4 sh = *reinterpret_cast<const float4*>(a.bn + BN_SH * fp + c);
            const float m = a.bt.row_m[r];
            float4 o;
            o.x = fmaxf(y.x * sc.x + sh.x, 0.0f) * m;
            o.y = fmaxf(y.y * sc.y + sh.y, 0.0f) * m;
            o.z = fmaxf(y.z * sc.z + sh.z, 0.0f) * m;
            o.w = fmaxf(y.w * sc.w + sh.w, 0.0f) * m;
            if (a.do_drop) {
                float ds[4];
                drop_scale4(seed, (uint64_t)r * fp + c, a.thr, a.inv_keep, ds);
                o.x *= ds[0]; o.y *= ds[1]; o.z *= ds[2]; o.w *= ds[3];
            }
            if (a.out) *reinterpret_cast<float4*>(a.out + (size_t)r * a.ldo + c) = o;
            if (a.planes.p) bx_store4(a.planes, r, c, o);
        }
    } else {
        const uint32_t g4 = a.tile_map ? ((uint32_t)(a.ldo + 31) >> 5) : a.ldo / 4;
        const uint32_t total = a.tile_map ? (((uint32_t)T + 7) >> 3) * g4 * 64u : (uint32_t)T * g4;
        for (uint32_t e = blockIdx.x * blockDim.x + threadIdx.x; e < total; e += gridDim.x * blockDim.x) {
            int r, f;
            if (a.tile_map) {
                const uint32_t it = e >> 6, rg = it / g4;
                r = (int)(rg * 8u + ((e >> 3) & 7u)); f = (int)((it - rg * g4) * 32u + (e & 7u) * 4u);
                if (r >= T || f >= a.ldo) continue;
            } else {
                r = (int)(e / g4); f = (int)(e - (uint32_t)r * g4) * 4;
            }
            float4 y[EAGCN_MAX_VIEWS];
#pragma unroll
            for (int k = 0; k < EAGCN_MAX_VIEWS; ++k)
                if (k < a.vc.K) y[k] = *reinterpret_cast<const float4*>(a.Y + (size_t)r * a.ldy + a.vc.off[k] + f);
            float4 acc = {0.0f, 0.0f, 0.0f, 0.0f};
#pragma unroll
            for (int k = 0; k < EAGCN_MAX_VIEWS; ++k)
                if (k < a.vc.K) {
                    const int cp = a.vc.off[k] + f;
                    const float4 sc = *reinterpret_cast<const float4*>(a.bn + BN_SC * fp + cp);
                    const float4 sh = *reinterpret_cast<const float4*>(a.bn + BN_SH * fp + cp);
                    const float4 w = *reinterpret_cast<const float4*>(a.colp + CP_AVEW * fp + cp);
                    float4 p;
                    p.x = fmaxf(y[k].x * sc.x + sh.x, 0.0f);
                    p.y = fmaxf(y[k].y * sc.y + sh.y, 0.0f);
                    p.z = fmaxf(y[k].z * sc.z + sh.z, 0.0f);
                    p.w = fmaxf(y[k].w * sc.w + sh.w, 0.0f);
                    if (a.do_drop) {
                        float ds[4];
                        drop_scale4(seed, (uint64_t)r * fp + cp, a.thr, a.inv_keep, ds);
                        p.x *= ds[0]; p.y *= ds[1]; p.z *= ds[2]; p.w *= ds[3];
                    }
                    acc.x += w.x * p.x; acc.y += w.y * p.y; acc.z += w.z * p.z; acc.w += w.w * p.w;
                }
            if (a.out) *reinterpret_cast<float4*>(a.out + (size_t)r * a.ldo + f) = acc;
            if (a.planes.p) bx_store4(a.planes, r, f, acc);
        }
    }
}

struct BwdArgs {
    const int32_t* meta; int Tcap;
    const int32_t* row_mol;
    const float* row_m;
    ViewCols vc;
    int structure, fp, nvirt;
    const float* dxout; int ldo;
    ReadoutGrad rg;
    const float* dpad;
    int dpad_views;
    const float* Y; int ldy;
    const float* bn;
    const float* colp;
    float* dH;
    double* slab;
    double* slab_da;
    int do_drop; uint32_t thr; float inv_keep; uint64_t seed; const uint64_t* seed_dev;
    double* zero; int nzero;
    EdgeDrain drain;
    const float* cc;
    int store_dh;
};

template <bool WEIGHTED, bool DG, bool DROP, bool APPLY>
__global__ __launch_bounds__(256) void bn_bwd_reduce_kernel(BwdArgs a) {
    __shared__ double da_s[EAGCN_MAX_VIEWS];
    const uint64_t seed = DROP ? (a.seed_dev ? *a.seed_dev : a.seed) : 0ull;
    const int fp = a.fp, T = min(a.meta[EAGCN_META_T], a.Tcap);
    const int rows = T + (APPLY ? 0 : a.nvirt);
    const int nwg = max(1, min((int)gridDim.x, (rows + BWD_ROWS - 1) / BWD_ROWS));
    if (!APPLY && a.drain.eacc && blockIdx.x == 0 && blockIdx.y == 0) {
        const int K = a.drain.K;
        for (int e = threadIdx.x; e < K * EDGE_SLAB; e += blockDim.x) {
            const int k = e / EDGE_SLAB, c = e - k * EDGE_SLAB;
            if (c > 256) continue;
            double v[EDGE_COPIES];
#pragma unroll
            for (int z = 0; z < EDGE_COPIES; ++z) v[z] = a.drain.eacc[((size_t)z * K + k) * EDGE_SLAB + c];
            double t = 0.0;
#pragma unroll
            for (int z = 0; z < EDGE_COPIES; ++z) { t += v[z]; a.drain.eacc[((size_t)z * K + k) * EDGE_SLAB + c] = 0.0; }
            float* dw = nullptr;
            float* dr = nullptr;
            int ch = 0;
#pragma unroll
            for (int q = 0; q < EAGCN_MAX_VIEWS; ++q)
                if (q == k) { dw = a.drain.datt_w[q]; dr = a.drain.dself_r[q]; ch = a.drain.channels[q]; }
            if (c == 256) {
                const double r = (double)a.drain.rsig[k];
                dr[0] = (float)(t * r * (1.0 - r));
            } else if (c >= 1 && c <= ch) {
                dw[c - 1] = (float)t;
            }
        }
    }
    if ((int)blockIdx.x >= nwg || (APPLY && T == 0)) return;
    if constexpr (!APPLY) {
        if (threadIdx.x < EAGCN_MAX_VIEWS) da_s[threadIdx.x] = 0.0;
        __syncthreads();
    }
    constexpr bool weighted = WEIGHTED;
    double da[EAGCN_MAX_VIEWS];
#pragma unroll
    for (int k = 0; k < EAGCN_MAX_VIEWS; ++k) da[k] = 0.0;
    const int c_lo = blockIdx.y * (int)blockDim.x * 4;
    for (int cp = c_lo + threadIdx.x * 4; cp < min(fp, c_lo + (int)blockDim.x * 4); cp += blockDim.x * 4) {
        const int k = col_view(a.vc, cp), f = cp - a.vc.off[k];
        const float4 sc = *reinterpret_cast<const float4*>(a.bn + BN_SC * fp + cp);
        const float4 sh = *reinterpret_cast<const float4*>(a.bn + BN_SH * fp + cp);
        const float4 mu = *reinterpret_cast<const float4*>(a.bn + BN_MU * fp + cp);
        const float4 iv = *reinterpret_cast<const float4*>(a.bn + BN_INV * fp + cp);
        const float4 aw = *reinterpret_cast<const float4*>(a.colp + CP_AVEW * fp + cp);
        float4 c1 = make_float4(0.f, 0.f, 0.f, 0.f), c2 = c1;
        if constexpr (APPLY) {
            c1 = *reinterpret_cast<const float4*>(a.cc + cp);
            c2 = *reinterpret_cast<const float4*>(a.cc + fp + cp);
        }
        const int cu = weighted ? f : cp;
        auto exact = [&](int c) {
            int eo = 0, po = 0, res = -1;
            bool done = false;
#pragma unroll
            for (int sg = 0; sg < EAGCN_MAX_SEGS; ++sg) {
                if (sg < a.rg.map.nseg && !done) {
                    if (c < po + a.rg.map.p[sg]) { res = (c - po < a.rg.map.w[sg]) ? eo + (c - po) : -1; done = true; }
                    eo += a.rg.map.w[sg];
                    po += a.rg.map.p[sg];
                }
            }
            return res;
        };
        int ce0 = -1, ce1 = -1, ce2 = -1, ce3 = -1;
        bool ce4 = false;
        if constexpr (DG) {
            ce0 = exact(cu); ce1 = exact(cu + 1); ce2 = exact(cu + 2); ce3 = exact(cu + 3);
            ce4 = ce0 >= 0 && ce3 == ce0 + 3 && (ce0 & 3) == 0 && (a.rg.F & 3) == 0 &&
                  (reinterpret_cast<uintptr_t>(a.rg.dg) & 15) == 0;
        }
        double s1[4] = {0.0, 0.0, 0.0, 0.0}, s2[4] = {0.0, 0.0, 0.0, 0.0}, dak = 0.0;
        for (int rb = blockIdx.x; rb < rows; rb += BWD_ROWS * nwg) {
            float4 yv[BWD_ROWS], upv[BWD_ROWS];
#pragma unroll
            for (int u = 0; u < BWD_ROWS; ++u) {
                const int r = rb + u * nwg;
                yv[u] = make_float4(0.f, 0.f, 0.f, 0.f);
                upv[u] = make_float4(0.f, 0.f, 0.f, 0.f);
                if (r < T) {
                    yv[u] = *reinterpret_cast<const float4*>(a.Y + (size_t)r * a.ldy + cp);
                    if constexpr (DG) {
                        const int mol = a.row_mol[r];
                        const float* g = a.rg.dg + (size_t)mol * a.rg.F;
                        float4 v;
                        if (ce4) {
                            v = *reinterpret_cast<const float4*>(g + ce0);
                        } else {
                            v.x = ce0 >= 0 ? g[ce0] : 0.0f;
                            v.y = ce1 >= 0 ? g[ce1] : 0.0f;
                            v.z = ce2 >= 0 ? g[ce2] : 0.0f;
                            v.w = ce3 >= 0 ? g[ce3] : 0.0f;
                        }
                        if (a.rg.mode == 1) {
                            const float is = 1.0f / (float)a.rg.size[mol];
                            v.x *= is; v.y *= is; v.z *= is; v.w *= is;
                        }
                        upv[u] = v;
                    } else {
                        upv[u] = *reinterpret_cast<const float4*>(a.dxout + (size_t)r * a.ldo + cu);
                    }
                    if (!weighted) {
                        const float m = a.row_m[r];
                        upv[u].x *= m; upv[u].y *= m; upv[u].z *= m; upv[u].w *= m;
                    }
                } else if (r < rows) {
                    upv[u] = *reinterpret_cast<const float4*>(a.dpad + (size_t)(a.dpad_views ? k : (r - T)) * a.ldo + cu);
                }
            }
#pragma unroll
            for (int u = 0; u < BWD_ROWS; ++u) {
                const int r = rb + u * nwg;
                if (r >= rows) continue;
                const float yy[4] = {yv[u].x, yv[u].y, yv[u].z, yv[u].w};
                const float uu[4] = {upv[u].x, upv[u].y, upv[u].z, upv[u].w};
                const float scv[4] = {sc.x, sc.y, sc.z, sc.w}, shv[4] = {sh.x, sh.y, sh.z, sh.w};
                const float muv[4] = {mu.x, mu.y, mu.z, mu.w}, ivv[4] = {iv.x, iv.y, iv.z, iv.w};
                const float awv[4] = {aw.x, aw.y, aw.z, aw.w};
                const float c1v[4] = {c1.x, c1.y, c1.z, c1.w}, c2v[4] = {c2.x, c2.y, c2.z, c2.w};
                float dh[4], dsv[4] = {1.0f, 1.0f, 1.0f, 1.0f};
                if (DROP && r < T) drop_scale4(seed, (uint64_t)r * fp + cp, a.thr, a.inv_keep, dsv);
#pragma unroll
                for (int j = 0; j < 4; ++j) {
                    float up = uu[j];
                    const float ds = dsv[j];
                    const float h = yy[j] * scv[j] + shv[j];
                    if (weighted) { if constexpr (!APPLY) dak += (double)(up * ds * fmaxf(h, 0.0f)); up *= awv[j]; }
                    dh[j] = h > 0.0f ? up * ds : 0.0f;
                    const float xh = (yy[j] - muv[j]) * ivv[j];
                    if constexpr (APPLY) {
                        dh[j] = scv[j] * (dh[j] - c1v[j] - xh * c2v[j]);
                    } else {
                        s1[j] += (double)dh[j];
                        s2[j] += (double)(dh[j] * xh);
                    }
                }
                if ((APPLY || a.store_dh) && r < T)
                    *reinterpret_cast<float4*>(a.dH + (size_t)r * fp + cp) = make_float4(dh[0], dh[1], dh[2], dh[3]);
            }
        }
        if constexpr (!APPLY) {
            double* sl = a.slab + ((size_t)blockIdx.x * fp + cp) * 2;
            *reinterpret_cast<double4*>(sl) = make_double4(s1[0], s2[0], s1[1], s2[1]);
            *reinterpret_cast<double4*>(sl + 4) = make_double4(s1[2], s2[2], s1[3], s2[3]);
            if (weighted) {
#pragma unroll
                for (int v = 0; v < EAGCN_MAX_VIEWS; ++v) da[v] += (v == k) ? dak : 0.0;
            }
        }
    }
    if (weighted && !APPLY) {
#pragma unroll
        for (int v = 0; v < EAGCN_MAX_VIEWS; ++v) {
            const double t = wave_sum(da[v]);
            if ((threadIdx.x & 63) == 0 && t != 0.0) atomicAdd(&da_s[v], t);
        }
        __syncthreads();
        if (threadIdx.x < EAGCN_MAX_VIEWS)
            a.slab_da[((size_t)blockIdx.y * gridDim.x + blockIdx.x) * EAGCN_MAX_VIEWS + threadIdx.x] = da_s[threadIdx.x];
    }
}

template <int L>
__global__ __launch_bounds__(256) void bn_bwd_finalize_kernel(const double* __restrict__ slab,
                                                               const double* __restrict__ slab_da, int nslab,
                                                               int fp, double M, int training,
                                                               const float* __restrict__ bn, ViewCols vc,
                                                               GradPtrs gp, float* __restrict__ cc, const int32_t* __restrict__ meta, int nvirt,
                                                               int batch_B, int da_chunks, int da_stride,
                                                               const double* __restrict__ gsum, double* __restrict__ zero, int nzero) {
    if (blockIdx.x == 0 && zero)
        for (int i = threadIdx.x; i < nzero; i += blockDim.x) zero[i] = 0.0;
    if (meta[EAGCN_META_NLOG] > 0) M = (double)batch_B * (double)meta[EAGCN_META_NLOG];
    nslab = max(1, min(nslab, (meta[EAGCN_META_T] + nvirt + BWD_ROWS - 1) / BWD_ROWS));
    const int cpr = blockIdx.x * (256 / L) + threadIdx.x / L, sl = threadIdx.x % L;
    const int cp = min(cpr, fp - 1);
    if (blockIdx.x == 0 && gp.dave_w) {
        const int v = threadIdx.x >> 5, l = threadIdx.x & 31;
        double t = 0.0;
        if (v < vc.K)
            for (int y = 0; y < da_chunks; ++y)
                for (int s = l; s < nslab; s += 32) t += slab_da[((size_t)y * da_stride + s) * EAGCN_MAX_VIEWS + v];
#pragma unroll
        for (int o = 16; o > 0; o >>= 1) t += __shfl_xor(t, o);
        if (v < vc.K && l == 0) gp.dave_w[v] = (float)t;
    }
    double s1, s2;
    slab_sum<L>(slab, nslab, fp, cp, sl, s1, s2);
    if (cpr >= fp || sl != 0) return;
    {
        double g1 = s1, g2 = s2;
        if (gsum) { g1 = gsum[2 * cp]; g2 = gsum[2 * cp + 1]; M = gsum[2 * fp]; }
        cc[cp] = training ? (float)(g1 / M) : 0.0f;
        cc[fp + cp] = training ? (float)(g2 / M) : 0.0f;
    }
    const int k = col_view(vc, cp), f = cp - vc.off[k];
    if (f < vc.width[k]) {
        gp.dgamma[k][f] = (float)s2;
        gp.dbeta[k][f] = (float)s1;
        gp.dbias[k][f] = training ? 0.0f : (float)((double)bn[BN_SC * fp + cp] * s1);
    }
}

__global__ __launch_bounds__(256) void bn_bwd_apply_kernel(eagcn_batch bt, int fp, const float* __restrict__ Y, int ldy,
                                                            const float* __restrict__ bn,
                                                            const float* __restrict__ cc, float* __restrict__ dH) {
    const uint32_t g4 = fp / 4;
    const uint32_t total = (uint32_t)dev_rows(bt) * g4;
    for (uint32_t e = blockIdx.x * blockDim.x + threadIdx.x; e < total; e += gridDim.x * blockDim.x) {
        const int r = (int)(e / g4), c = (int)(e - (uint32_t)r * g4) * 4;
        const float4 y = *reinterpret_cast<const float4*>(Y + (size_t)r * ldy + c);
        float4 d = *reinterpret_cast<float4*>(dH + (size_t)r * fp + c);
        const float4 sc = *reinterpret_cast<const float4*>(bn + BN_SC * fp + c);
        const float4 mu = *reinterpret_cast<const float4*>(bn + BN_MU * fp + c);
        const float4 iv = *reinterpret_cast<const float4*>(bn + BN_INV * fp + c);
        const float4 c1 = *reinterpret_cast<const float4*>(cc + c);
        const float4 c2 = *reinterpret_cast<const float4*>(cc + fp + c);
        d.x = sc.x * (d.x - c1.x - (y.x - mu.x) * iv.x * c2.x);
        d.y = sc.y * (d.y - c1.y - (y.y - mu.y) * iv.y * c2.y);
        d.z = sc.z * (d.z - c1.z - (y.z - mu.z) * iv.z * c2.z);
        d.w = sc.w * (d.w - c1.w - (y.w - mu.w) * iv.w * c2.w);
        *reinterpret_cast<float4*>(dH + (size_t)r * fp + c) = d;
    }
}

__global__ __launch_bounds__(256) void unpack_grads_kernel(GradPtrs gp, ParamPtrs pp, ViewCols vc, ColMapD in,
                                                            int ld_in, int fp, const float* __restrict__ dWcat,
                                                            int nsplit, size_t slab, double* __restrict__ datt,
                                                            int nedge, const float* __restrict__ rsig, int wblocks,
                                                            const int32_t* __restrict__ meta, int xk_G, int edge_drain, int bx_per, int bx_wide) {
    nedge = nedge < 0 ? -nedge : min(nedge, (meta[EAGCN_META_T] + 15) / 16);
    const int bxm = bx_wide ? BX3W_BM : BX3_BM, bxn = bx_wide ? BX3W_BN : BX3_BN;
    nsplit = nsplit < 0 ? bx3_used_splits_wave(-nsplit, meta[EAGCN_META_T], ((ld_in + bxm - 1) / bxm) * ((fp + bxn - 1) / bxn),
                                          bx_per > 0 ? ((meta[EAGCN_META_T] + bxm - 1) / bxm) * ((ld_in + bxn - 1) / bxn) : 0, max(1, (fp + 31) >> 5), bx_per)
                        : max(1, min(nsplit, meta[EAGCN_META_T] >> 7));
    if ((int)blockIdx.x < wblocks) {
        const int tid = blockIdx.x * blockDim.x + threadIdx.x;
        if (xk_G > 0) {
            const int e = tid;
            if (e >= ld_in * fp) return;
            const int ip = e / fp, cp = e % fp;
            const int k = col_view(vc, cp), f = cp - vc.off[k];
            const int fi = packed_to_exact(in, ip);
            if (fi < 0 || f >= vc.width[k]) return;
            const int T = meta[EAGCN_META_T];
            G3Plan pl;
            g3_plan((T + 63) / 64, (ld_in + 63) / 64, max(1, (fp + 15) / 16), ((ld_in + 63) / 64) * ((fp + 63) / 64),
                    max(1, (T + 15) / 16), xk_G, pl);
            float v[G3_XSEG];
#pragma unroll
            for (int x = 0; x < G3_XSEG; ++x) v[x] = pl.c[x + 1] > pl.c[x] ? dWcat[(size_t)x * slab + e] : 0.0f;
            float t = 0.0f;
#pragma unroll
            for (int x = 0; x < G3_XSEG; ++x) t += v[x];
            gp.dW[k][(size_t)fi * vc.width[k] + f] = T > 0 ? t : 0.0f;
            return;
        }
        const int sub = tid & 3;
        const int e = (tid >> 2) * 4;
        if (e >= ld_in * fp) return;
        const int ip = e / fp, cp = e % fp;
        const int k = col_view(vc, cp), f = cp - vc.off[k];
        const int fi = packed_to_exact(in, ip);
        if (fi < 0 || f >= vc.width[k]) return;
        float4 s0 = make_float4(0.f, 0.f, 0.f, 0.f), s1 = s0;
        int z = sub;
#pragma unroll 4
        for (; z + 4 < nsplit; z += 8) {
            const float4 a0 = *reinterpret_cast<const float4*>(dWcat + (size_t)z * slab + e);
            const float4 a1 = *reinterpret_cast<const float4*>(dWcat + (size_t)(z + 4) * slab + e);
            s0.x += a0.x; s0.y += a0.y; s0.z += a0.z; s0.w += a0.w;
            s1.x += a1.x; s1.y += a1.y; s1.z += a1.z; s1.w += a1.w;
        }
        if (z < nsplit) {
            const float4 a0 = *reinterpret_cast<const float4*>(dWcat + (size_t)z * slab + e);
            s0.x += a0.x; s0.y += a0.y; s0.z += a0.z; s0.w += a0.w;
        }
        float t[4] = {s0.x + s1.x, s0.y + s1.y, s0.z + s1.z, s0.w + s1.w};
#pragma unroll
        for (int j = 0; j < 4; ++j) { t[j] += __shfl_xor(t[j], 1); t[j] += __shfl_xor(t[j], 2); }
        const float tv = sub == 0 ? t[0] : sub == 1 ? t[1] : sub == 2 ? t[2] : t[3];
        if (f + sub < vc.width[k]) gp.dW[k][(size_t)fi * vc.width[k] + f + sub] = tv;
        return;
    }
    const int er = ((int)blockIdx.x - wblocks) * 16 + (threadIdx.x >> 4), sl = threadIdx.x & 15;
    const int tot = vc.K * EDGE_SLAB;
    const int e = min(er, tot - 1);
    const int k = e / EDGE_SLAB, c = e % EDGE_SLAB;
    const bool general = pp.rel_vec[k] != nullptr && c != 256;
    double t = 0.0;
    if (!general) {
        for (int z0 = sl; z0 < nedge; z0 += 16 * 8) {
            double v[8];
#pragma unroll
            for (int u = 0; u < 8; ++u) {
                const int z = z0 + 16 * u;
                v[u] = z < nedge ? datt[(size_t)z * tot + e] : 0.0;
            }
#pragma unroll
            for (int u = 0; u < 8; ++u) t += v[u];
            if (edge_drain && er < tot) {
#pragma unroll
                for (int u = 0; u < 8; ++u) {
                    const int z = z0 + 16 * u;
                    if (z < nedge) datt[(size_t)z * tot + e] = 0.0;
                }
            }
        }
    } else if (c >= 1 && c <= pp.rel_c[k]) {
        const float* vec = pp.rel_vec[k];
        const int C = pp.rel_c[k], D = pp.channels[k];
        for (int z = sl; z < nedge; z += 16)
            for (int code = 1; code <= D; ++code)
                t += datt[(size_t)z * tot + k * EDGE_SLAB + code] * (double)vec[(size_t)(code - 1) * C + (c - 1)];
    }
#pragma unroll
    for (int o = 8; o > 0; o >>= 1) t += __shfl_xor(t, o);
    if (er >= tot || sl != 0) return;
    if (c == 256) {
        const double r = (double)rsig[k];
        gp.dself_r[k][0] = (float)(t * r * (1.0 - r));
    } else if (c >= 1 && c <= (pp.rel_vec[k] ? pp.rel_c[k] : pp.channels[k])) {
        gp.datt_w[k][c - 1] = (float)t;
    }
}

__global__ __launch_bounds__(256) void attention_dense_kernel(eagcn_batch bt, ParamPtrs pp, float* __restrict__ out) {
    const size_t total = (size_t)bt.K * bt.B * bt.N * bt.N;
    for (size_t e = (size_t)blockIdx.x * blockDim.x + threadIdx.x; e < total;
         e += (size_t)gridDim.x * blockDim.x) {
        const int j = (int)(e % bt.N);
        const size_t kbi = e / bt.N;
        const int k = (int)(kbi / ((size_t)bt.B * bt.N));
        const size_t bi = kbi - (size_t)k * bt.B * bt.N;
        const uint32_t c = bt.deg_bn[bi] > 0 ? bt.code[kbi * bt.ldc + j] : 0u;
        out[e] = (c >= 1 && (int)c <= pp.channels[k]) ? sigmoidf_(att_logit(pp, k, (int)c)) : 0.0f;
    }
}

struct Carver {
    char* base;
    size_t off = 0;
    explicit Carver(void* p) : base((char*)p) {}
    template <typename T>
    T* take(size_t n) {
        T* p = base ? (T*)(base + off) : nullptr;
        off = align256(off + n * sizeof(T));
        return p;
    }
};

struct LayerDims {
    ViewCols vc;
    int fp, ld_in, fin, ldo, gx, gxb, nsplit;
    int gslab;
    size_t wslab;
    size_t wpslab, wtpslab;
    int np;
    int bx_splits;
};
static LayerDims layer_dims(const eagcn_batch* b, const eagcn_layer_params* p) {
    LayerDims d;
    d.vc = view_cols(p);
    d.fp = d.vc.off[p->K];
    d.ld_in = layout_ld(&p->in);
    d.fin = layout_width(&p->in);
    d.ldo = p->structure == EAGCN_STRUCT_CONCATE ? d.fp : pad16(p->width[0]);
    d.gx = agg_grid_x(b);
    d.gslab = std::max(d.gx, lagg_use(b, 0, false, &d.vc) ? lagg_slabs(b) : 0);
    {
        const long by_rows = cdiv(b->T + 1, BWD_ROWS);
        const long by_bytes = std::max<long>(64, (32L << 20) / ((long)d.fp * 16));
        d.gxb = (int)std::max<long>(1, std::min<long>(std::min<long>(by_rows, 2048), by_bytes));
    }
    const int tiles = cdiv(d.ld_in, 64) * cdiv(d.fp, 64);
    d.nsplit = std::max(1, std::min(std::max(1, 1024 / tiles), cdiv(std::max(b->T, 1), 128)));
    d.wslab = (size_t)d.ld_in * d.fp;
    d.wpslab = bx_plane_elems(d.ld_in, d.fp);
    d.wtpslab = bx_plane_elems(d.fp, d.ld_in);
    d.np = (d.ld_in >= 128 && (d.ld_in & 15) == 0 && (d.fp & 15) == 0) ? gemm_planes() : 0;
    d.bx_splits = std::max(1, std::min(std::min(1023, std::max(64, cdiv(std::max(b->T, 1), 4096))), std::max(cdiv(std::max(b->T, 1), 4096), cdiv(std::max(b->T, 1), 256))));
    return d;
}

static bool gemm3_layer(int ld_in) {
    static const bool on = [] { const char* v = getenv("EAGCN_NO_GEMM3"); return !(v && v[0] == '1'); }();
    return on && ld_in >= 128 && gemm_mode() != 2;
}

struct Packed { float *Wcat, *WcatT, *colp, *sig, *rsig; uint16_t *Wp, *WTp; };
struct FwdScratch { void* gws; double* eacc; float *Wcat, *WcatT, *colp, *sig, *rsig; uint16_t *Wp, *WTp; double* stats; double* gsum;
                    uint16_t* xp; };
static size_t carve_packed(void* base, const LayerDims& d, Packed* s) {
    Carver c(base);
    Packed t;
    t.Wcat = c.take<float>(d.wslab);
    t.WcatT = c.take<float>(d.wslab);
    t.colp = c.take<float>((size_t)CP_ROWS * d.fp);
    t.sig = c.take<float>(EAGCN_MAX_VIEWS * 256);
    t.rsig = c.take<float>(EAGCN_MAX_VIEWS);
    t.Wp = c.take<uint16_t>(d.np ? (size_t)d.np * d.wpslab : 1);
    t.WTp = c.take<uint16_t>(d.np ? (size_t)d.np * d.wtpslab : 1);
    if (s) *s = t;
    return c.off;
}
struct BwdScratch {
    void* gws;
    double* eacc;
    float *Wcat, *WcatT, *colp, *sig, *rsig, *dY, *dP, *cc, *dWcat;
    uint16_t *Wp, *WTp;
    double *slab, *slab_da, *datt, *gsum;
    uint16_t *dPp, *xp;
};
static size_t carve_fwd(void* base, const eagcn_batch* b, const LayerDims& d, FwdScratch* s) {
    Carver c(base);
    FwdScratch t;
    t.gws = c.take<char>(gemm3_workspace_bytes());
    t.eacc = (double*)c.take<char>(edge_acc_bytes());
    t.Wcat = c.take<float>(d.wslab);
    t.WcatT = c.take<float>(d.wslab);
    t.colp = c.take<float>((size_t)CP_ROWS * d.fp);
    t.sig = c.take<float>(EAGCN_MAX_VIEWS * 256);
    t.rsig = c.take<float>(EAGCN_MAX_VIEWS);
    t.Wp = c.take<uint16_t>(d.np ? (size_t)d.np * d.wpslab : 1);
    t.WTp = c.take<uint16_t>(d.np ? (size_t)d.np * d.wtpslab : 1);
    t.stats = c.take<double>((size_t)d.gslab * d.fp * 2);
    t.gsum = c.take<double>((size_t)2 * d.fp + 8);
    t.xp = c.take<uint16_t>(d.np ? (size_t)d.np * bx_plane_elems(b->T, d.ld_in) : 1);
    if (s) *s = t;
    return c.off;
}
static size_t carve_bwd(void* base, const eagcn_batch* b, const LayerDims& d, BwdScratch* s) {
    Carver c(base);
    BwdScratch t;
    t.gws = c.take<char>(gemm3_workspace_bytes());
    t.eacc = (double*)c.take<char>(edge_acc_bytes());
    t.Wcat = c.take<float>(d.wslab);
    t.WcatT = c.take<float>(d.wslab);
    t.colp = c.take<float>((size_t)CP_ROWS * d.fp);
    t.sig = c.take<float>(EAGCN_MAX_VIEWS * 256);
    t.rsig = c.take<float>(EAGCN_MAX_VIEWS);
    t.Wp = c.take<uint16_t>(d.np ? (size_t)d.np * d.wpslab : 1);
    t.WTp = c.take<uint16_t>(d.np ? (size_t)d.np * d.wtpslab : 1);
    t.dY = c.take<float>((size_t)std::max(b->T, 1) * d.fp);
    t.dP = c.take<float>((size_t)std::max(b->T, 1) * d.fp);
    t.cc = c.take<float>((size_t)2 * d.fp);
    t.dWcat = c.take<float>(d.wslab * std::max(std::max(d.nsplit, G3_XSEG), d.np ? d.bx_splits : 1));
    t.slab = c.take<double>((size_t)d.gxb * d.fp * 2);
    t.slab_da = c.take<double>((size_t)d.gxb * cdiv(d.fp, 1024) * EAGCN_MAX_VIEWS);
    t.datt = c.take<double>((size_t)edge_grid_x(b) * EAGCN_MAX_VIEWS * EDGE_SLAB);
    t.gsum = c.take<double>((size_t)2 * d.fp + 8);
    t.dPp = c.take<uint16_t>(d.np ? (size_t)d.np * bx_plane_elems(b->T, d.fp) : 1);
    t.xp = c.take<uint16_t>(d.np ? (size_t)d.np * bx_plane_elems(b->T, d.ld_in) : 1);
    if (s) *s = t;
    return c.off;
}

static int check_layer(const eagcn_batch* b, const eagcn_layer_params* p, const char* who) {
    EAGCN_CHECK_ARG(b && p, "%s: null argument", who);
    EAGCN_CHECK_ARG(p->K >= 1 && p->K <= EAGCN_MAX_VIEWS && p->K == b->K,
                    "%s: layer has %d views, batch index has %d", who, p->K, b->K);
    EAGCN_CHECK_ARG(p->structure == EAGCN_STRUCT_CONCATE || p->structure == EAGCN_STRUCT_WEIGHTED,
                    "%s: unknown structure %d", who, p->structure);
    EAGCN_CHECK_ARG(p->in.nseg >= 1 && p->in.nseg <= EAGCN_MAX_SEGS, "%s: bad input layout", who);
    for (int s = 0; s < p->in.nseg; ++s)
        EAGCN_CHECK_ARG(p->in.width[s] >= 1 && p->in.pad[s] >= p->in.width[s] && (p->in.pad[s] % 4) == 0,
                        "%s: input segment %d: width %d pad %d (pad must be a multiple of 4 >= width)", who, s,
                        p->in.width[s], p->in.pad[s]);
    for (int k = 0; k < p->K; ++k) {
        EAGCN_CHECK_ARG(p->width[k] >= 1, "%s: view %d has width %d", who, k, p->width[k]);
        EAGCN_CHECK_ARG(p->att_w[k] && p->self_r[k] && p->W[k] && p->bias[k] && p->gamma[k] && p->beta[k] &&
                            p->run_mean[k] && p->run_var[k], "%s: view %d has a null parameter", who, k);
        if (p->structure == EAGCN_STRUCT_WEIGHTED)
            EAGCN_CHECK_ARG(p->width[k] == p->width[0], "%s: Weighted_sum needs equal view widths", who);
    }
    if (p->structure == EAGCN_STRUCT_WEIGHTED) EAGCN_CHECK_ARG(p->ave_w, "%s: Weighted_sum needs ave_w", who);
    EAGCN_CHECK_ARG(p->dropout >= 0.0f && p->dropout < 1.0f, "%s: dropout %f out of [0,1)", who, p->dropout);
    EAGCN_CHECK_ARG((uint64_t)std::max(b->T, 0) * (uint64_t)view_cols(p).off[p->K] / 4 < (1ull << 32),
                    "%s: %d rows x %d packed columns exceed the 32-bit element index of the BatchNorm passes", who, b->T,
                    view_cols(p).off[p->K]);
    return EAGCN_OK;
}

static ParamPtrs param_ptrs(const eagcn_batch* b, const eagcn_layer_params* p) {
    ParamPtrs pp;
    memset(&pp, 0, sizeof(pp));
    for (int k = 0; k < p->K; ++k) {
        pp.att_w[k] = p->att_w[k]; pp.self_r[k] = p->self_r[k]; pp.W[k] = p->W[k]; pp.bias[k] = p->bias[k];
        pp.gamma[k] = p->gamma[k]; pp.beta[k] = p->beta[k]; pp.run_mean[k] = p->run_mean[k];
        pp.run_var[k] = p->run_var[k]; pp.channels[k] = b->channels[k];
        pp.rel_vec[k] = b->rel_vec[k]; pp.rel_c[k] = b->rel_c[k];
    }
    pp.ave_w = p->structure == EAGCN_STRUCT_WEIGHTED ? p->ave_w : nullptr;
    return pp;
}

static inline int ew_grid(size_t n) { return (int)std::max<size_t>(1, std::min<size_t>((n + 255) / 256, 2048)); }

}

static int apply_launch_(const eagcn_batch* b, const eagcn_layer_params* p, const eagcn_layer_bufs* w, const eagcn::LayerDims& d,
                         const float* colp, hipStream_t s, bool planes_only = false);
#define apply_launch apply_launch_

using namespace eagcn;

extern "C" int eagcn_pad16(int w) { return pad16(w); }
extern "C" int eagcn_layer_fp(const eagcn_layer_params* p) { return view_cols(p).off[p->K]; }
extern "C" int eagcn_layer_out_ld(const eagcn_layer_params* p) {
    return p->structure == EAGCN_STRUCT_CONCATE ? eagcn_layer_fp(p) : pad16(p->width[0]);
}
extern "C" size_t eagcn_layer_packed_bytes(const eagcn_batch* b, const eagcn_layer_params* p) {
    LayerDims d = layer_dims(b, p);
    return carve_packed(nullptr, d, nullptr);
}
extern "C" size_t eagcn_layer_fwd_scratch_bytes(const eagcn_batch* b, const eagcn_layer_params* p) {
    LayerDims d = layer_dims(b, p);
    return carve_fwd(nullptr, b, d, nullptr);
}
extern "C" size_t eagcn_layer_bwd_scratch_bytes(const eagcn_batch* b, const eagcn_layer_params* p) {
    LayerDims d = layer_dims(b, p);
    return carve_bwd(nullptr, b, d, nullptr);
}

extern "C" int eagcn_layer_forward(const eagcn_batch* b, const eagcn_layer_params* p, const eagcn_layer_bufs* w,
                                   void* stream) {
    EAGCN_CHECK_GEMM3("eagcn_layer_forward");
    if (w && w->scratch && w->scratch_bytes >= gemm3_workspace_bytes()) {
        int rc = gemm3_clear_flags(w->scratch, w->scratch_bytes, (hipStream_t)stream);
        if (rc) return rc;
    }
    return layer_forward_impl(b, p, w, stream, false);
}

int eagcn::pack_params_all(const eagcn_batch* b, const eagcn_layer_params* const* ps, void* const* packed,
                           const size_t* packed_bytes, int n, void* stream, const ZeroJob* zj, const HandOff* ho) {
    hipStream_t s = (hipStream_t)stream;
    EAGCN_CHECK_ARG(n >= 1 && n <= 4, "pack_params_all: 1..4 layers");
    PackJob jobs[4];
    size_t wmax = 0;
    for (int l = 0; l < 4; ++l) {
        const int ll = l < n ? l : n - 1;
        int rc = check_layer(b, ps[ll], "eagcn_model_forward");
        if (rc) return rc;
        const LayerDims d = layer_dims(b, ps[ll]);
        Packed pk;
        const size_t pneed = carve_packed(packed[ll], d, &pk);
        if (pneed > packed_bytes[ll]) {
            set_error("pack_params_all: packed buffer of layer %d too small (%zu < %zu)", ll, packed_bytes[ll], pneed);
            return EAGCN_ERR_SCRATCH;
        }
        jobs[l].pp = param_ptrs(b, ps[ll]); jobs[l].vc = d.vc; jobs[l].in = make_colmap(&ps[ll]->in);
        jobs[l].ld_in = d.ld_in; jobs[l].fp = d.fp;
        jobs[l].Wcat = pk.Wcat; jobs[l].WcatT = pk.WcatT; jobs[l].colp = pk.colp; jobs[l].sig = pk.sig; jobs[l].rsig = pk.rsig;
        jobs[l].wp = BxOut{d.np ? pk.Wp : nullptr, d.wpslab, d.np, d.ld_in};
        jobs[l].wtp = BxOut{d.np ? pk.WTp : nullptr, d.wtpslab, d.np, d.fp};
        if (l < n) wmax = std::max(wmax, d.wslab);
    }
    PackJobs pj{jobs[0], jobs[1], jobs[2], jobs[3]};
    ProfScope ps_(PROF_PACK, s);
    const ZeroJob none{nullptr, 0, nullptr, 0};
    const HandOff noho{nullptr, nullptr, nullptr, 0};
    pack_params_multi_kernel<<<dim3(ew_grid(wmax), n), 256, 0, s>>>(pj, zj ? *zj : none, ho ? *ho : noho);
    EAGCN_LAUNCH_CHECK();
    return EAGCN_OK;
}

int eagcn::layer_forward_impl(const eagcn_batch* b, const eagcn_layer_params* p, const eagcn_layer_bufs* w,
                              void* stream, bool prepacked, bool skip_apply, bool planes_only) {
    hipStream_t s = (hipStream_t)stream;
    int rc = check_layer(b, p, "eagcn_layer_forward");
    if (rc) return rc;
    EAGCN_CHECK_ARG(w && w->bn && w->xout && w->pad_row && w->scratch, "eagcn_layer_forward: null buffer");
    EAGCN_CHECK_ARG(b->T == 0 || ((w->x || w->x_planes) && w->P && w->Y && w->rscale), "eagcn_layer_forward: null activation buffer");
    EAGCN_CHECK_ARG(!planes_only || (w->xout_planes && gemm_planes()), "eagcn_layer_forward: planes-only output without plane images");
    const LayerDims d = layer_dims(b, p);
    FwdScratch sc;
    const size_t need = carve_fwd(w->scratch, b, d, &sc);
    if (need > w->scratch_bytes) {
        set_error("eagcn_layer_forward: scratch too small (%zu < %zu)", w->scratch_bytes, need);
        return EAGCN_ERR_SCRATCH;
    }
    const ParamPtrs pp = param_ptrs(b, p);
    const ColMapD in = make_colmap(&p->in);
    if (w->packed) {
        Packed pk;
        const size_t pneed = carve_packed(w->packed, d, &pk);
        if (pneed > w->packed_bytes) {
            set_error("eagcn_layer_forward: packed buffer too small (%zu < %zu)", w->packed_bytes, pneed);
            return EAGCN_ERR_SCRATCH;
        }
        sc.Wcat = pk.Wcat; sc.WcatT = pk.WcatT; sc.colp = pk.colp; sc.sig = pk.sig; sc.rsig = pk.rsig;
        sc.Wp = pk.Wp; sc.WTp = pk.WTp;
    }
    EAGCN_CHECK_ARG(!prepacked || w->packed, "eagcn_layer_forward: prepacked parameters need the packed block");
    if (!prepacked) {
        ProfScope ps(PROF_PACK, s);
        pack_params_kernel<<<ew_grid(d.wslab), 256, 0, s>>>(pp, d.vc, in, d.ld_in, d.fp, sc.Wcat, sc.WcatT, sc.colp, sc.sig, sc.rsig,
                                                            BxOut{d.np ? sc.Wp : nullptr, d.wpslab, d.np, d.ld_in},
                                                            BxOut{d.np ? sc.WTp : nullptr, d.wtpslab, d.np, d.fp});
    }
    EAGCN_LAUNCH_CHECK();
    double fsum = 0.0;
    for (int k = 0; k < p->K; ++k) fsum += p->width[k];
    const double gemm_work = 2.0 * (double)b->T * (double)d.fin * fsum;
    int nslab = 0, tiles_per_wg = agg_ksplit(b) ? 1 : 4;
    if (b->T > 0) {
        GemmDesc g3{0, 1, b->T, d.fp, d.ld_in, w->x, d.ld_in, sc.WcatT, d.ld_in, w->P, d.fp, 1, 0, gemm_work};
        g3.M_dev = b->meta + EAGCN_META_T;
        BxProb bp;
        memset(&bp, 0, sizeof(bp));
        if (d.np) {
            const size_t xstride = bx_plane_elems(b->T, d.ld_in);
            const uint16_t* xp = w->x_planes;
            if (!xp) {
                EAGCN_CHECK_ARG(w->x, "eagcn_layer_forward: neither an fp32 input nor its plane images");
                rc = launch_bx3_split(w->x, b->T, b->meta + EAGCN_META_T, d.ld_in, sc.xp, xstride, b->T, d.np, s);
                if (rc) return rc;
                xp = sc.xp;
            }
            bp.A = BxPlanes{xp, xstride, d.ld_in, b->T}; bp.B = BxPlanes{sc.WTp, d.wtpslab, d.ld_in, d.fp}; bp.C = w->P; bp.ldc = d.fp;
            bp.M = b->T; bp.N = d.fp; bp.K = d.ld_in; bp.M_dev = b->meta + EAGCN_META_T; bp.tn = 0; bp.splits = 1;
        }
        if (d.np && bx3_ok(bp)) {
            rc = launch_bx3(bp, nullptr, d.np, s, gemm_work, PROF_GEMM, bx3_pick_wide(bp, nullptr, b->t_hint));
        } else if (!w->x) {
            set_error("eagcn_layer_forward: the input exists as plane images only and the plane product does not apply");
            return EAGCN_ERR_ARG;
        } else if (gemm3_layer(d.ld_in) && gemm3_ok(g3)) {
            rc = launch_gemm3(g3, nullptr, sc.gws, gemm3_workspace_bytes(), s);
        } else {
            GemmDesc g{0, 0, b->T, d.fp, d.ld_in, w->x, d.ld_in, sc.Wcat, d.fp, w->P, d.fp, 1, 0, gemm_work};
            g.M_dev = b->meta + EAGCN_META_T;
            rc = launch_gemm(g, s);
        }
        if (rc) return rc;
        {
            AggArgs a;
            a.bt = *b; a.vc = d.vc; a.src = w->P; a.lds = d.fp; a.dst = w->Y; a.ldd = d.fp;
            a.sig = sc.sig; a.rsig = sc.rsig; a.rscale = w->rscale; a.stats = sc.stats; a.nchunk = 1;
            if (lagg_use(b, 0, false, &d.vc)) {
                rc = launch_lagg_fwd(a, s);
                nslab = lagg_slabs(b);
                tiles_per_wg = -1;
            } else {
                rc = launch_agg(a, false, s);
                nslab = d.gx;
            }
            if (rc) return rc;
        }
    }
    const double M = (double)b->B * (double)b->N;
    {
    ProfScope psbn(PROF_BN, s);
    if (w->stats_hook && p->training) {
        if (nslab > 64) bn_stats_sum_kernel<64><<<cdiv(d.fp, 4), 256, 0, s>>>(sc.stats, nslab, d.fp, M, sc.gsum, b->meta, 1, tiles_per_wg, 0, b->B);
        else bn_stats_sum_kernel<16><<<cdiv(d.fp, 16), 256, 0, s>>>(sc.stats, nslab, d.fp, M, sc.gsum, b->meta, 1, tiles_per_wg, 0, b->B);
        EAGCN_LAUNCH_CHECK();
        if (w->stats_hook(sc.gsum, 2 * d.fp + 1, stream, w->stats_user)) {
            set_error("eagcn_layer_forward: the sync-BatchNorm all-reduce hook failed");
            return EAGCN_ERR_HIP;
        }
        bn_finalize_kernel<16><<<cdiv(d.fp, 16), 256, 0, s>>>(sc.gsum, 1, d.fp, M, p->training, p->bn_eps, p->bn_momentum, sc.colp,
                                                                pp, d.vc, w->bn, b->meta, 0, b->B, sc.gsum + 2 * d.fp);
    } else if (nslab > 64)
        bn_finalize_kernel<64><<<cdiv(d.fp, 4), 256, 0, s>>>(sc.stats, nslab, d.fp, M, p->training, p->bn_eps,
                                                               p->bn_momentum, sc.colp, pp, d.vc, w->bn, b->meta, tiles_per_wg, b->B, nullptr);
    else
        bn_finalize_kernel<16><<<cdiv(d.fp, 16), 256, 0, s>>>(sc.stats, nslab, d.fp, M, p->training, p->bn_eps,
                                                                p->bn_momentum, sc.colp, pp, d.vc, w->bn, b->meta, tiles_per_wg, b->B, nullptr);
    EAGCN_LAUNCH_CHECK();
    }
    if (skip_apply) return EAGCN_OK;
    return apply_launch(b, p, w, d, sc.colp, s, planes_only);
}

bool eagcn::layer_reads_planes_only(const eagcn_batch* b, const eagcn_layer_params* p, bool aux_stream) {
    static const bool on = [] { const char* v = getenv("EAGCN_PLANES_ONLY"); return !(v && v[0] == '0'); }();
    if (!on || aux_stream || !b || !p || b->T <= 0) return false;
    const LayerDims d = layer_dims(b, p);
    if (!d.np) return false;
    const uint16_t* pl = reinterpret_cast<const uint16_t*>(static_cast<uintptr_t>(4096));
    float* fo = reinterpret_cast<float*>(static_cast<uintptr_t>(4096));
    const size_t xstride = bx_plane_elems(b->T, d.ld_in), pstride = bx_plane_elems(b->T, d.fp);
    BxProb bp, bx, bw;
    memset(&bp, 0, sizeof(bp)); memset(&bx, 0, sizeof(bx)); memset(&bw, 0, sizeof(bw));
    bp.A = BxPlanes{pl, xstride, d.ld_in, b->T}; bp.B = BxPlanes{pl, d.wtpslab, d.ld_in, d.fp}; bp.C = fo; bp.ldc = d.fp;
    bp.M = b->T; bp.N = d.fp; bp.K = d.ld_in; bp.M_dev = b->meta + EAGCN_META_T; bp.tn = 0; bp.splits = 1;
    bx.A = BxPlanes{pl, pstride, d.fp, b->T}; bx.B = BxPlanes{pl, d.wpslab, d.fp, d.ld_in}; bx.C = fo; bx.ldc = d.ld_in;
    bx.M = b->T; bx.N = d.ld_in; bx.K = d.fp; bx.M_dev = b->meta + EAGCN_META_T; bx.tn = 0; bx.splits = 1;
    bw.A = BxPlanes{pl, xstride, d.ld_in, b->T}; bw.B = BxPlanes{pl, pstride, d.fp, b->T};
    bw.C = fo; bw.ldc = d.fp; bw.M = d.ld_in; bw.N = d.fp; bw.K = b->T; bw.K_dev = b->meta + EAGCN_META_T; bw.tn = 1;
    bw.splits = d.bx_splits; bw.slab = d.wslab;
    return bx3_ok(bp) && bx3_ok(bw) && bx3_ok(bx);
}

int eagcn::layer_apply_impl(const eagcn_batch* b, const eagcn_layer_params* p, const eagcn_layer_bufs* w, void* stream) {
    EAGCN_CHECK_ARG(b && p && w && w->bn && w->xout && w->pad_row && w->packed, "layer_apply: null buffer");
    const LayerDims d = layer_dims(b, p);
    Packed pk;
    EAGCN_CHECK_ARG(carve_packed(w->packed, d, &pk) <= w->packed_bytes, "layer_apply: packed buffer too small");
    return apply_launch(b, p, w, d, pk.colp, (hipStream_t)stream);
}

static int apply_launch_(const eagcn_batch* b, const eagcn_layer_params* p, const eagcn_layer_bufs* w, const LayerDims& d,
                         const float* colp, hipStream_t s, bool planes_only) {
    ProfScope psbn(PROF_BN, s);
    ApplyArgs aa;
    aa.bt = *b; aa.vc = d.vc; aa.structure = p->structure; aa.fp = d.fp; aa.Y = w->Y; aa.ldy = d.fp;
    aa.bn = w->bn; aa.colp = colp; aa.out = w->xout; aa.ldo = d.ldo; aa.pad_row = w->pad_row;
    aa.do_drop = (p->training && p->dropout > 0.0f) ? 1 : 0;
    aa.thr = (uint32_t)std::min(4294967295.0, (double)p->dropout * 4294967296.0);
    aa.inv_keep = 1.0f / (1.0f - p->dropout);
    aa.seed = p->seed;
    aa.seed_dev = p->seed_dev;
    aa.planes = BxOut{gemm_planes() ? w->xout_planes : nullptr, bx_plane_elems(b->T, d.ldo), gemm_planes(), b->T};
    if (planes_only && aa.planes.p) aa.out = nullptr;
    static const int map_env = [] { const char* v = getenv("EAGCN_BN_APPLY_MAP"); return v ? atoi(v) : -1; }();
    aa.tile_map = map_env >= 0 ? map_env : (aa.planes.p ? 1 : 0);
    const size_t nthr = aa.tile_map ? (size_t)cdiv(std::max(b->T, 1), 8) * cdiv(d.ldo, 32) * 64 : (size_t)std::max(b->T, 1) * d.ldo / 4;
    bn_apply_kernel<<<ew_grid(nthr), 256, 0, s>>>(aa);
    EAGCN_LAUNCH_CHECK();
    return EAGCN_OK;
}

static bool lagg_fuses_bn() {
    static const bool on = [] { const char* v = getenv("EAGCN_LAGG_FUSE_BN"); return !(v && v[0] == '0'); }();
    return on;
}
static bool bn_bwd_two_pass(bool weighted) {
    static const int force = [] { const char* v = getenv("EAGCN_BWD_STORE_DH"); return v ? (v[0] == '1' ? 1 : 0) : -1; }();
    return force < 0 ? weighted : force == 0;
}
static void launch_bn_bwd_pass(bool apply, bool wt, bool dg, bool dr, dim3 grid, const BwdArgs& ba, hipStream_t s) {
#define EAGCN_BWD(W, G, D) do { if (apply) bn_bwd_reduce_kernel<W, G, D, true><<<grid, 256, 0, s>>>(ba); \
                                else bn_bwd_reduce_kernel<W, G, D, false><<<grid, 256, 0, s>>>(ba); } while (0)
    if (wt) { if (dg) { if (dr) EAGCN_BWD(true, true, true); else EAGCN_BWD(true, true, false); }
              else    { if (dr) EAGCN_BWD(true, false, true); else EAGCN_BWD(true, false, false); } }
    else    { if (dg) { if (dr) EAGCN_BWD(false, true, true); else EAGCN_BWD(false, true, false); }
              else    { if (dr) EAGCN_BWD(false, false, true); else EAGCN_BWD(false, false, false); } }
#undef EAGCN_BWD
}

extern "C" int eagcn_layer_backward(const eagcn_batch* b, const eagcn_layer_params* p, const eagcn_layer_bufs* w,
                                    const float* dxout, const float* dpad_row, float* dx,
                                    const eagcn_layer_grads* g, void* stream) {
    EAGCN_CHECK_GEMM3("eagcn_layer_backward");
    if (w && w->scratch && w->scratch_bytes >= gemm3_workspace_bytes()) {
        int rc = gemm3_clear_flags(w->scratch, w->scratch_bytes, (hipStream_t)stream);
        if (rc) return rc;
    }
    return layer_backward_impl(b, p, w, dxout, nullptr, dpad_row, dx, g, stream);
}

int eagcn::layer_backward_impl(const eagcn_batch* b, const eagcn_layer_params* p, const eagcn_layer_bufs* w,
                               const float* dxout, const ReadoutGrad* rg, const float* dpad_row, float* dx,
                               const eagcn_layer_grads* g, void* stream, bool dpad_views, const ZeroJob* zero_after,
                               const EdgeDrain* drain_in, EdgeDrain* drain_out, bool input_only) {
    if (drain_out) drain_out->eacc = nullptr;
    hipStream_t s = (hipStream_t)stream;
    int rc = check_layer(b, p, "eagcn_layer_backward");
    if (rc) return rc;
    EAGCN_CHECK_ARG(w && (g || input_only) && w->bn && w->scratch, "eagcn_layer_backward: null buffer");
    EAGCN_CHECK_ARG(!input_only || (dx && !drain_in), "eagcn_layer_backward: the input-only form needs dx and takes no edge reduction");
    EAGCN_CHECK_ARG(b->T == 0 || ((dxout || rg) && (input_only || w->x || w->x_planes) && w->P && w->Y && w->rscale),
                    "eagcn_layer_backward: null activation buffer");
    if (!input_only)
        for (int k = 0; k < p->K; ++k)
            EAGCN_CHECK_ARG(g->dW[k] && g->dbias[k] && g->dgamma[k] && g->dbeta[k] && g->datt_w[k] && g->dself_r[k],
                            "eagcn_layer_backward: view %d has a null gradient buffer", k);
    const LayerDims d = layer_dims(b, p);
    BwdScratch sc;
    const size_t need = carve_bwd(w->scratch, b, d, &sc);
    if (need > w->scratch_bytes) {
        set_error("eagcn_layer_backward: scratch too small (%zu < %zu)", w->scratch_bytes, need);
        return EAGCN_ERR_SCRATCH;
    }
    const ParamPtrs pp = param_ptrs(b, p);
    GradPtrs gp;
    memset(&gp, 0, sizeof(gp));
    if (input_only) {
        EAGCN_CHECK_ARG(d.wslab >= (size_t)3 * d.fp + EAGCN_MAX_VIEWS, "eagcn_layer_backward: no room for the discarded BatchNorm gradients");
        for (int k = 0; k < p->K; ++k) {
            gp.dgamma[k] = sc.dWcat + d.vc.off[k];
            gp.dbeta[k] = sc.dWcat + d.fp + d.vc.off[k];
            gp.dbias[k] = sc.dWcat + 2 * d.fp + d.vc.off[k];
        }
        gp.dave_w = p->structure == EAGCN_STRUCT_WEIGHTED ? sc.dWcat + 3 * d.fp : nullptr;
    } else {
        for (int k = 0; k < p->K; ++k) {
            gp.dW[k] = g->dW[k]; gp.dbias[k] = g->dbias[k]; gp.dgamma[k] = g->dgamma[k]; gp.dbeta[k] = g->dbeta[k];
            gp.datt_w[k] = g->datt_w[k]; gp.dself_r[k] = g->dself_r[k];
        }
        gp.dave_w = p->structure == EAGCN_STRUCT_WEIGHTED ? g->dave_w : nullptr;
    }
    const ColMapD in = make_colmap(&p->in);
    if (w->packed) {
        Packed pk;
        const size_t pneed = carve_packed(w->packed, d, &pk);
        if (pneed > w->packed_bytes) {
            set_error("eagcn_layer_backward: packed buffer too small (%zu < %zu)", w->packed_bytes, pneed);
            return EAGCN_ERR_SCRATCH;
        }
        sc.Wcat = pk.Wcat; sc.WcatT = pk.WcatT; sc.colp = pk.colp; sc.sig = pk.sig; sc.rsig = pk.rsig;
        sc.Wp = pk.Wp; sc.WTp = pk.WTp;
    } else {
        ProfScope ps(PROF_PACK, s);
        pack_params_kernel<<<ew_grid(d.wslab), 256, 0, s>>>(pp, d.vc, in, d.ld_in, d.fp, sc.Wcat, sc.WcatT, sc.colp, sc.sig, sc.rsig,
                                                            BxOut{d.np ? sc.Wp : nullptr, d.wpslab, d.np, d.ld_in},
                                                            BxOut{d.np ? sc.WTp : nullptr, d.wtpslab, d.np, d.fp});
    }
    EAGCN_LAUNCH_CHECK();
    double fsum = 0.0;
    for (int k = 0; k < p->K; ++k) fsum += p->width[k];
    const double gemm_work = 2.0 * (double)b->T * (double)d.fin * fsum;

    BwdArgs ba;
    ba.meta = b->meta; ba.Tcap = b->T; ba.row_mol = b->row_mol; ba.row_m = b->row_m;
    ba.vc = d.vc; ba.structure = p->structure; ba.fp = d.fp;
    ba.nvirt = (dpad_row && p->structure == EAGCN_STRUCT_WEIGHTED) ? 1 : 0;
    ba.dxout = dxout; ba.ldo = d.ldo; ba.dpad = dpad_row; ba.dpad_views = dpad_views ? 1 : 0;
    if (rg) ba.rg = *rg; else memset(&ba.rg, 0, sizeof(ba.rg)); ba.Y = w->Y; ba.ldy = d.fp; ba.bn = w->bn;
    ba.colp = sc.colp; ba.dH = sc.dY; ba.slab = sc.slab; ba.slab_da = sc.slab_da;
    ba.do_drop = (p->training && p->dropout > 0.0f) ? 1 : 0;
    ba.thr = (uint32_t)std::min(4294967295.0, (double)p->dropout * 4294967296.0);
    ba.inv_keep = 1.0f / (1.0f - p->dropout);
    ba.seed = p->seed;
    ba.seed_dev = p->seed_dev;
    ba.zero = zero_after ? zero_after->d : nullptr;
    ba.nzero = zero_after ? zero_after->nd : 0;
    if (drain_in && drain_in->eacc) ba.drain = *drain_in; else memset(&ba.drain, 0, sizeof(ba.drain));
    const int rows = b->T + ba.nvirt;
    const int gxb = std::max(1, std::min(rows, d.gxb));
    bool fused_bn_apply = false, fused_w_apply = false, w_rows = false, fused_c_apply = false;
    bool lagg_bwd = false;
    {
        static const bool edge_atomic0 = [] { const char* v = getenv("EAGCN_EDGE_SLABS"); return !(v && v[0] == '1'); }();
        bool general0 = false;
        for (int k = 0; k < p->K; ++k) general0 = general0 || pp.rel_vec[k] != nullptr;
        const bool wt0 = p->structure == EAGCN_STRUCT_WEIGHTED;
        const bool absorbs = lagg_fuses_bn() && (!bn_bwd_two_pass(wt0) || (wt0 && lagg_wfuse()));
        lagg_bwd = b->T > 0 && edge_atomic0 && !general0 && lagg_use(b, 1, absorbs);
        if (input_only) lagg_bwd = b->T > 0 && lagg_use(b, 1, true);
    }
    const double M = (double)b->B * (double)b->N;
    const bool eval_in = input_only && !p->training;
    if (eval_in) {
        const bool wt = p->structure == EAGCN_STRUCT_WEIGHTED, dg = ba.rg.dg != nullptr;
        if (b->T > 0 && lagg_bwd) {
            if (dg) {
                rc = launch_readout_bwd_rows(b, ba.rg, d.ldo, sc.dY, s);
                if (rc) return rc;
                w_rows = true;
            }
            if (wt) fused_w_apply = true; else fused_c_apply = true;
        } else if (b->T > 0) {
            rc = zero_fill(sc.cc, (size_t)2 * d.fp * sizeof(float), s);
            if (rc) return rc;
            ba.cc = sc.cc;
            launch_bn_bwd_pass(true, wt, dg, false, dim3(std::max(1, std::min(b->T, d.gxb)), cdiv(d.fp, 1024)), ba, s);
            EAGCN_LAUNCH_CHECK();
        }
        if (zero_after && zero_after->nd) { rc = zero_fill(zero_after->d, (size_t)zero_after->nd * sizeof(double), s); if (rc) return rc; }
    } else {
        ProfScope ps(PROF_BN, s);
        const int ny = cdiv(d.fp, 1024);
        {
            const bool wt = p->structure == EAGCN_STRUCT_WEIGHTED, dr = ba.do_drop != 0;
            bool dg = ba.rg.dg != nullptr;
            const dim3 grid(gxb, ny);
            ba.cc = sc.cc;
            ba.store_dh = bn_bwd_two_pass(wt) ? 0 : 1;
            static const bool rows_first = [] { const char* v = getenv("EAGCN_W_ROWS_FIRST"); return !(v && v[0] == '0'); }();
            if (wt && dg && b->T > 0 && bn_bwd_two_pass(wt) && lagg_bwd && lagg_fuses_bn() && lagg_wfuse() && rows_first) {
                rc = launch_readout_bwd_rows(b, ba.rg, d.ldo, sc.dY, s);
                if (rc) return rc;
                w_rows = true;
                ba.dxout = sc.dY;
                dg = false;
            }
            launch_bn_bwd_pass(false, wt, dg, dr, grid, ba, s);
        }
        EAGCN_LAUNCH_CHECK();
        const double* gsum = nullptr;
        if (w->stats_hook && p->training) {
            if (gxb > 64) bn_stats_sum_kernel<64><<<cdiv(d.fp, 4), 256, 0, s>>>(sc.slab, gxb, d.fp, M, sc.gsum, b->meta, 2, 0, ba.nvirt, b->B);
            else bn_stats_sum_kernel<16><<<cdiv(d.fp, 16), 256, 0, s>>>(sc.slab, gxb, d.fp, M, sc.gsum, b->meta, 2, 0, ba.nvirt, b->B);
            EAGCN_LAUNCH_CHECK();
            if (w->stats_hook(sc.gsum, 2 * d.fp + 1, stream, w->stats_user)) {
                set_error("eagcn_layer_backward: the sync-BatchNorm all-reduce hook failed");
                return EAGCN_ERR_HIP;
            }
            gsum = sc.gsum;
        }
        if (gxb > 64)
            bn_bwd_finalize_kernel<64><<<cdiv(d.fp, 4), 256, 0, s>>>(sc.slab, sc.slab_da, gxb, d.fp, M, p->training, w->bn,
                                                                       d.vc, gp, sc.cc, b->meta, ba.nvirt, b->B, ny, gxb, gsum, ba.zero, ba.nzero);
        else
            bn_bwd_finalize_kernel<16><<<cdiv(d.fp, 16), 256, 0, s>>>(sc.slab, sc.slab_da, gxb, d.fp, M, p->training, w->bn,
                                                                        d.vc, gp, sc.cc, b->meta, ba.nvirt, b->B, ny, gxb, gsum, ba.zero, ba.nzero);
        EAGCN_LAUNCH_CHECK();
        if (b->T > 0) {
            const bool wt = p->structure == EAGCN_STRUCT_WEIGHTED, dg = ba.rg.dg != nullptr, dr = ba.do_drop != 0;
            if (bn_bwd_two_pass(wt) && wt && lagg_bwd && lagg_fuses_bn() && lagg_wfuse()) {
                fused_w_apply = true;
                if (dg && !w_rows) {
                    rc = launch_readout_bwd_rows(b, ba.rg, d.ldo, sc.dY, s);
                    if (rc) return rc;
                }
            } else if (bn_bwd_two_pass(wt)) launch_bn_bwd_pass(true, wt, dg, dr, dim3(std::max(1, std::min(b->T, d.gxb)), ny), ba, s);
            else if (lagg_bwd && lagg_fuses_bn()) fused_bn_apply = true;
            else bn_bwd_apply_kernel<<<ew_grid((size_t)b->T * d.fp / 4), 256, 0, s>>>(*b, d.fp, w->Y, d.fp, w->bn, sc.cc, sc.dY);
            EAGCN_LAUNCH_CHECK();
        }
    }
    int nsplit = 0, nedge = 0, xk_G = 0;
    bool bx_slabs = false;
    int bx_per = 0;
    int bx_wide = 0;
    hipStream_t side = w->aux_stream ? (hipStream_t)w->aux_stream : s;
    const bool forked = side != s;
    if (b->T > 0) {
        AggArgs a;
        a.bt = *b; a.vc = d.vc; a.src = sc.dY; a.lds = d.fp; a.dst = sc.dP; a.ldd = d.fp;
        a.sig = sc.sig; a.rsig = sc.rsig; a.rscale = w->rscale; a.stats = nullptr; a.nchunk = 1;
        const size_t xstride = bx_plane_elems(b->T, d.ld_in), pstride = bx_plane_elems(b->T, d.fp);
        BxProb bx, bw;
        memset(&bx, 0, sizeof(bx));
        memset(&bw, 0, sizeof(bw));
        bool use_bx = false;
        if (d.np && !w->aux_stream) {
            bx.A = BxPlanes{sc.dPp, pstride, d.fp, b->T}; bx.B = BxPlanes{sc.Wp, d.wpslab, d.fp, d.ld_in}; bx.C = dx; bx.ldc = d.ld_in;
            bx.M = b->T; bx.N = d.ld_in; bx.K = d.fp; bx.M_dev = b->meta + EAGCN_META_T; bx.tn = 0; bx.splits = 1;
            bw.A = BxPlanes{w->x_planes ? w->x_planes : sc.xp, xstride, d.ld_in, b->T}; bw.B = BxPlanes{sc.dPp, pstride, d.fp, b->T};
            bw.C = sc.dWcat; bw.ldc = d.fp; bw.M = d.ld_in; bw.N = d.fp; bw.K = b->T; bw.K_dev = b->meta + EAGCN_META_T; bw.tn = 1;
            bw.splits = d.bx_splits; bw.slab = d.wslab;
            use_bx = bx3_ok(bw) && (!dx || bx3_ok(bx));
        }
        if (use_bx) {
            a.planes = BxOut{sc.dPp, pstride, d.np, b->T};
            if (!w->x_planes && !input_only) {
                rc = launch_bx3_split(w->x, b->T, b->meta + EAGCN_META_T, d.ld_in, sc.xp, xstride, b->T, d.np, s);
                if (rc) return rc;
            }
        } else if (!w->x && !input_only) {
            set_error("eagcn_layer_backward: the input exists as plane images only and the plane products do not apply");
            return EAGCN_ERR_ARG;
        }
        EdgeArgs e;
        e.bt = *b; e.vc = d.vc; e.dY = sc.dY; e.Y = w->Y; e.P = w->P; e.ld = d.fp; e.sig = sc.sig;
        e.rsig = sc.rsig; e.rscale = w->rscale; e.datt = sc.datt; e.atomic = 0;
        static const bool edge_atomic = [] { const char* v = getenv("EAGCN_EDGE_SLABS"); return !(v && v[0] == '1'); }();
        bool general_rel = false;
        for (int k = 0; k < p->K; ++k) general_rel = general_rel || pp.rel_vec[k] != nullptr;
        if (edge_atomic && !general_rel) { e.datt = sc.eacc; e.atomic = 1; }
        static const bool colaunch = [] { const char* v = getenv("EAGCN_NO_COLAUNCH"); return !(v && v[0] == '1'); }();
        nedge = e.atomic ? -EDGE_COPIES : edge_grid_x(b);
        if (input_only) {
            if (lagg_bwd) {
                if (fused_bn_apply || fused_w_apply || fused_c_apply) { a.bn_tab = w->bn; a.bn_cc = eval_in ? nullptr : sc.cc; a.bn_fp = d.fp; }
                if (fused_w_apply || fused_c_apply) {
                    a.src = (ba.rg.dg || w_rows) ? sc.dY : dxout; a.lds = d.ldo;
                    a.w_aw = sc.colp + (size_t)CP_AVEW * d.fp;
                    a.w_rowm = fused_c_apply;
                    a.w_drop = ba.do_drop; a.w_thr = ba.thr; a.w_inv_keep = ba.inv_keep; a.w_seed = ba.seed; a.w_seed_dev = ba.seed_dev;
                }
                rc = launch_lagg_bwd(a, e, s, false);
            } else {
                rc = launch_agg(a, true, s);
            }
            if (rc) return rc;
            if (use_bx) {
                rc = launch_bx3(bx, nullptr, d.np, s, gemm_work, PROF_GEMM, bx3_pick_wide(bx, nullptr, b->t_hint));
            } else {
                GemmDesc gx{0, 1, b->T, d.ld_in, d.fp, sc.dP, d.fp, sc.Wcat, d.fp, dx, d.ld_in, 1, 0, gemm_work};
                gx.M_dev = b->meta + EAGCN_META_T;
                rc = launch_gemm(gx, s);
            }
            return rc;
        }
        if (lagg_bwd && e.atomic) {
            if (fused_bn_apply || fused_w_apply) { a.bn_tab = w->bn; a.bn_cc = sc.cc; a.bn_fp = d.fp; }
            if (fused_w_apply) {
                a.src = (ba.rg.dg || w_rows) ? sc.dY : dxout; a.lds = d.ldo;
                a.w_aw = sc.colp + (size_t)CP_AVEW * d.fp;
                a.w_drop = ba.do_drop; a.w_thr = ba.thr; a.w_inv_keep = ba.inv_keep; a.w_seed = ba.seed; a.w_seed_dev = ba.seed_dev;
            }
            rc = launch_lagg_bwd(a, e, s);
            if (rc) return rc;
        } else if (!forked && colaunch) {
            rc = launch_agg_edge(a, e, s);
            if (rc) return rc;
        } else {
            if (forked) { rc = stream_after(side, s); if (rc) return rc; }
            rc = launch_edge_grad(e, side);
            if (rc) return rc;
            rc = launch_agg(a, true, s);
            if (rc) return rc;
        }
        if (forked) { rc = stream_after(side, s); if (rc) return rc; }
        nsplit = d.nsplit;
        GemmDesc gw{1, 0, d.ld_in, d.fp, b->T, w->x, d.ld_in, sc.dP, d.fp, sc.dWcat, d.fp, nsplit, d.wslab, gemm_work};
        gw.K_dev = b->meta + EAGCN_META_T;
        GemmDesc gx{0, 1, b->T, d.ld_in, d.fp, sc.dP, d.fp, sc.Wcat, d.fp, dx, d.ld_in, 1, 0, gemm_work};
        gx.M_dev = b->meta + EAGCN_META_T;
        static const bool pair = [] { const char* v = getenv("EAGCN_NO_PAIR"); return !(v && v[0] == '1'); }();
        static const bool use3 = [] { const char* v = getenv("EAGCN_NO_GEMM3"); return !(v && v[0] == '1'); }();
        DwScatter dsc;
        for (int k = 0; k < EAGCN_MAX_VIEWS; ++k) dsc.dW[k] = gp.dW[k];
        dsc.vc = d.vc;
        dsc.in = in;
        if (use_bx) {
            bx_wide = dx ? bx3_pick_wide(bx, &bw, b->t_hint) : bx3_pick_wide(bw, nullptr, b->t_hint);
            rc = dx ? launch_bx3(bx, &bw, d.np, s, 2.0 * gemm_work, PROF_GEMM_PAIR, bx_wide) : launch_bx3(bw, nullptr, d.np, s, gemm_work, PROF_GEMM, bx_wide);
            if (rc) return rc;
            nsplit = d.bx_splits;
            bx_slabs = true;
            bx_per = (dx && bx3_pair_policy()) ? std::max(1, bx3_grid() >> 3) : 0;
        } else if (use3 && !forked && dx && gemm3_layer(d.ld_in) && gemm3_ok(gw) && gemm3_ok(gx) && gemm3_xk_enabled()) {
            rc = launch_gemm3_pair(gx, gw, nullptr, sc.gws, gemm3_workspace_bytes(), s, d.wslab);
            if (rc) return rc;
            nsplit = 1;
            xk_G = gemm3_grid();
        } else if (use3 && !forked && dx && gemm3_layer(d.ld_in) && gemm3_ok(gw) && gemm3_ok(gx)) {
            rc = launch_gemm3_pair(gx, gw, &dsc, sc.gws, gemm3_workspace_bytes(), s);
            if (rc) return rc;
            nsplit = 0;
        } else if (dx && !forked && colaunch && pair) {
            rc = launch_gemm_pair(gx, gw, s);
            if (rc) return rc;
        } else {
            rc = launch_gemm(gw, side);
            if (rc) return rc;
            if (dx) { rc = launch_gemm(gx, s); if (rc) return rc; }
        }
    }
    if (b->T == 0 && input_only) return EAGCN_OK;
    if (b->T == 0) {
        for (int k = 0; k < p->K; ++k)
            { int rcz = zero_fill(gp.dW[k], (size_t)d.fin * p->width[k] * sizeof(float), side); if (rcz) return rcz; }
    }
    {
        const int wblocks = nsplit > 0 ? cdiv((int)d.wslab, 256) : 0;
        double* edge_src = nedge == -EDGE_COPIES ? sc.eacc : sc.datt;
        const int edge_drain = edge_src == sc.eacc ? 1 : 0;
        static const bool defer_env = [] { const char* v = getenv("EAGCN_NO_EDGE_DEFER"); return !(v && v[0] == '1'); }();
        if (defer_env && drain_out && edge_drain && wblocks == 0 && !forked && b->T > 0) {
            drain_out->eacc = sc.eacc; drain_out->K = p->K; drain_out->rsig = sc.rsig;
            for (int k = 0; k < EAGCN_MAX_VIEWS; ++k) {
                drain_out->datt_w[k] = gp.datt_w[k]; drain_out->dself_r[k] = gp.dself_r[k]; drain_out->channels[k] = pp.channels[k];
            }
            return EAGCN_OK;
        }
        ProfScope psu(PROF_PACK, side);
        unpack_grads_kernel<<<wblocks + cdiv(p->K * EDGE_SLAB, 16), 256, 0, side>>>(gp, pp, d.vc, in, d.ld_in, d.fp, sc.dWcat,
                                                                                    bx_slabs ? -nsplit : nsplit, d.wslab, edge_src, nedge, sc.rsig,
                                                                                    wblocks, b->meta, xk_G, edge_drain, bx_per, bx_wide);
        EAGCN_LAUNCH_CHECK();
    }
    if (forked) { rc = stream_after(s, side); if (rc) return rc; }
    return EAGCN_OK;
}

extern "C" int eagcn_attention_dense(const eagcn_batch* b, const eagcn_layer_params* p, float* out, void* stream) {
    hipStream_t s = (hipStream_t)stream;
    EAGCN_CHECK_ARG(b && p && out, "eagcn_attention_dense: null argument");
    EAGCN_CHECK_ARG(p->K == b->K, "eagcn_attention_dense: view count mismatch");
    EAGCN_CHECK_ARG(b->code, "eagcn_attention_dense: batch has no code map");
    ParamPtrs pp;
    memset(&pp, 0, sizeof(pp));
    for (int k = 0; k < p->K; ++k) {
        EAGCN_CHECK_ARG(p->att_w[k], "eagcn_attention_dense: view %d has no attention weight", k);
        pp.att_w[k] = p->att_w[k];
        pp.channels[k] = b->channels[k];
        pp.rel_vec[k] = b->rel_vec[k]; pp.rel_c[k] = b->rel_c[k];
    }
    const size_t total = (size_t)b->K * b->B * b->N * b->N;
    attention_dense_kernel<<<ew_grid(total), 256, 0, s>>>(*b, pp, out);
    EAGCN_LAUNCH_CHECK();
    return EAGCN_OK;
}
```

Measured before the change: 699,800.

## Add thin-K GEMM kernels and defer weight-gradient slab reduction into the next unpack

Adds dedicated kernels for skinny GEMMs (NN with K<=32 and TN with M<=32), used instead of the generic tiled path when the shape qualifies. It also lets an upper layer's backward defer its weight-gradient slab reduction, handing the pending slabs down so the next layer's unpack_grads launch reduces them alongside its own. The aim is fewer launches and less tile waste for the small first-layer shapes. In exchange it adds a pending-list protocol, a fixed pairwise summation order for edge drains, and extra scratch regions per layer.

```diff
diff --git a/eagcn_amd/build.py b/eagcn_amd/build.py
--- a/eagcn_amd/build.py
+++ b/eagcn_amd/build.py
@@ -8,7 +8,7 @@
 CSRC = os.path.join(HERE, 'csrc')
 LIBDIR = os.path.join(HERE, 'lib')
 LIB = os.path.join(LIBDIR, 'libeagcn_hip.so')
-HIP_SOURCES = ['index.hip', 'gemm.hip', 'gemm3.hip', 'gemm_bx3.hip', 'gemm_bx3w.hip', 'agg.hip', 'lagg.hip', 'lagg_in.hip', 'gat.hip', 'pool.hip', 'layer.hip', 'readout.hip', 'head.hip', 'head2.hip', 'loss.hip', 'attr.hip']
+HIP_SOURCES = ['index.hip', 'gemm.hip', 'gemm_thin.hip', 'gemm3.hip', 'gemm_bx3.hip', 'gemm_bx3w.hip', 'agg.hip', 'lagg.hip', 'lagg_in.hip', 'gat.hip', 'pool.hip', 'layer.hip', 'readout.hip', 'head.hip', 'head2.hip', 'loss.hip', 'attr.hip']
 CPP_SOURCES = ['api.cpp']
 HEADERS = ['common.h', 'kernels.h', 'lagg_kernel.h', 'gemm_x6.h', 'bx3.h', os.path.join('..', '..', 'include', 'eagcn_hip.h')]
 ARCH = 'gfx950'
diff --git a/eagcn_amd/csrc/common.h b/eagcn_amd/csrc/common.h
--- a/eagcn_amd/csrc/common.h
+++ b/eagcn_amd/csrc/common.h
@@ -246,6 +246,17 @@
     int prof_tag = PROF_GEMM;
 };
 int launch_gemm(const GemmDesc& g, hipStream_t s);
+__host__ __device__ __forceinline__ int dw_used_splits(int cap, int Kx) {
+    const int by_rows = Kx >> 7;
+    const int n = cap < by_rows ? cap : by_rows;
+    return n > 1 ? n : 1;
+}
+int gemm_dw_slabs(const GemmDesc& g);
+bool gemm_thin_nn_ok(const GemmDesc& g);
+bool gemm_thin_tn_ok(const GemmDesc& g);
+int gemm_thin_tn_slabs(const GemmDesc& g);
+int launch_gemm_thin_nn(const GemmDesc& g, hipStream_t s);
+int launch_gemm_thin_tn(const GemmDesc& g, hipStream_t s);
 int launch_gemm_pair(const GemmDesc& dx, const GemmDesc& dw, hipStream_t s);
 
 }
diff --git a/eagcn_amd/csrc/gemm.hip b/eagcn_amd/csrc/gemm.hip
--- a/eagcn_amd/csrc/gemm.hip
+++ b/eagcn_amd/csrc/gemm.hip
@@ -204,7 +204,7 @@
 }
 
 __device__ __forceinline__ int eff_splits(const GemmDesc& g, int Kx) {
-    return g.K_dev ? max(1, min(g.splits, Kx >> 7)) : g.splits;
+    return g.K_dev ? dw_used_splits(g.splits, Kx) : g.splits;
 }
 
 __device__ __forceinline__ int xcd_remap(int lin, int nwg) {
@@ -306,15 +306,32 @@
     return launch_x6_cfg<64, 64, 1>(g, s);
 }
 
-int launch_gemm(const GemmDesc& g0, hipStream_t s) {
+static void set_vec(GemmDesc& g) {
+    g.vecA = (g.lda % 4) == 0 && ((g.ta ? g.M : g.K) % 4) == 0 && (reinterpret_cast<uintptr_t>(g.A) % 16) == 0;
+    g.vecB = (g.ldb % 4) == 0 && ((g.tb ? g.K : g.N) % 4) == 0 && (reinterpret_cast<uintptr_t>(g.B) % 16) == 0;
+}
+static int gemm_cfg_forced() {
+    static const int forced = [] { const char* e = getenv("EAGCN_GEMM_CFG"); return e ? atoi(e) : -1; }();
+    return forced;
+}
+static bool take_thin_nn(const GemmDesc& g) { return gemm_cfg_forced() < 0 && !use_x6(g) && gemm_thin_nn_ok(g); }
+static bool take_thin_tn(const GemmDesc& g) { return gemm_cfg_forced() < 0 && !use_x6(g) && gemm_thin_tn_ok(g); }
+
+int gemm_dw_slabs(const GemmDesc& g0) {
+    GemmDesc g = g0;
+    set_vec(g);
+    return take_thin_tn(g) ? gemm_thin_tn_slabs(g) : g.splits;
+}
+
+static int launch_gemm_impl(const GemmDesc& g0, hipStream_t s, bool thin) {
     if (g0.M <= 0 || g0.N <= 0) return EAGCN_OK;
     EAGCN_CHECK_ARG(g0.splits >= 1, "gemm: splits must be >= 1");
     GemmDesc g = g0;
-    g.vecA = (g.lda % 4) == 0 && ((g.ta ? g.M : g.K) % 4) == 0 && (reinterpret_cast<uintptr_t>(g.A) % 16) == 0;
-    g.vecB = (g.ldb % 4) == 0 && ((g.tb ? g.K : g.N) % 4) == 0 && (reinterpret_cast<uintptr_t>(g.B) % 16) == 0;
+    set_vec(g);
+    if (thin && take_thin_nn(g)) return launch_gemm_thin_nn(g, s);
+    if (thin && take_thin_tn(g)) return launch_gemm_thin_tn(g, s);
     if (g.splits > 1) EAGCN_CHECK_ARG(g.vecA && g.vecB, "gemm: split-K needs float4-aligned operands");
-    static const int forced = [] { const char* e = getenv("EAGCN_GEMM_CFG"); return e ? atoi(e) : -1; }();
-    int cfg = forced;
+    int cfg = gemm_cfg_forced();
     if (cfg < 0 && use_x6(g)) return launch_x6(g, s, use_x6(g));
     if (cfg < 0) {
         const long tiles128 = (long)cdiv(g.M, 128) * cdiv(g.N, 128) * g.splits;
@@ -329,6 +346,7 @@
         default: return launch_cfg<64, 64, 16, 4>(g, s);
     }
 }
+int launch_gemm(const GemmDesc& g, hipStream_t s) { return launch_gemm_impl(g, s, true); }
 
 int launch_gemm_pair(const GemmDesc& dx, const GemmDesc& dw, hipStream_t s) {
     GemmDesc g0 = dx, g1 = dw;
@@ -339,7 +357,7 @@
     const bool ok = g0.ta == 0 && g0.tb == 1 && g0.splits == 1 && !g0.K_dev && g1.ta == 1 && g1.tb == 0 && !g1.M_dev &&
                     (g1.splits == 1 || (g1.vecA && g1.vecB)) && g0.M > 0 && g0.N > 0 && g1.M > 0 && g1.N > 0;
     if (!ok) {
-        int rc = launch_gemm(dw, s);
+        int rc = launch_gemm_impl(dw, s, false);
         return rc ? rc : launch_gemm(dx, s);
     }
     const int first1 = (cdiv(g0.M, 64) * cdiv(g0.N, 64) + 7) / 8 * 8;
diff --git a/eagcn_amd/csrc/gemm_thin.hip b/eagcn_amd/csrc/gemm_thin.hip
--- /dev/null
+++ b/eagcn_amd/csrc/gemm_thin.hip
@@ -0,0 +1,157 @@
+#include <stdlib.h>
+
+#include "common.h"
+
+namespace eagcn {
+
+constexpr int THIN_NN_ROWS = 8;
+constexpr int THIN_TN_WAVES = 8;
+constexpr int THIN_TN_COLS = 64;
+constexpr int THIN_TN_RPW = 16;
+constexpr int THIN_TN_TILE = THIN_TN_WAVES * THIN_TN_RPW;
+
+template <int KR>
+__global__ __launch_bounds__(256) void gemm_thin_nn_kernel(GemmDesc g, const float* __restrict__ A, const float* __restrict__ B,
+                                                            float* __restrict__ Cout) {
+    const int Mx = g.M_dev ? min(*g.M_dev, g.M) : g.M;
+    const int wave = __builtin_amdgcn_readfirstlane(threadIdx.x >> 6), lane = threadIdx.x & 63;
+    const int row0 = ((int)blockIdx.x * 4 + wave) * THIN_NN_ROWS;
+    if (row0 >= Mx) return;
+    const int col = ((int)blockIdx.y * 64 + lane) * 4;
+    const bool cok = col < g.N;
+    float4 b[KR];
+#pragma unroll
+    for (int k = 0; k < KR; ++k)
+        b[k] = cok ? *reinterpret_cast<const float4*>(B + (size_t)k * g.ldb + col) : make_float4(0.f, 0.f, 0.f, 0.f);
+    const int rend = min(row0 + THIN_NN_ROWS, Mx);
+#pragma unroll 2
+    for (int r = row0; r < rend; ++r) {
+        const float* __restrict__ a = A + (size_t)r * g.lda;
+        float4 c = make_float4(0.f, 0.f, 0.f, 0.f);
+#pragma unroll
+        for (int k = 0; k < KR; ++k) {
+            const float av = a[k];
+            c.x = fmaf(av, b[k].x, c.x); c.y = fmaf(av, b[k].y, c.y); c.z = fmaf(av, b[k].z, c.z); c.w = fmaf(av, b[k].w, c.w);
+        }
+        if (cok) *reinterpret_cast<float4*>(Cout + (size_t)r * g.ldc + col) = c;
+    }
+}
+
+template <int MR>
+__global__ __launch_bounds__(THIN_TN_WAVES * 64) void gemm_thin_tn_kernel(GemmDesc g, const float* __restrict__ A,
+                                                                            const float* __restrict__ B, float* __restrict__ Cout) {
+    constexpr int RED = THIN_TN_WAVES * MR * THIN_TN_COLS, STAGE = THIN_TN_TILE * MR;
+    static_assert(RED >= STAGE && RED * 4 <= 65536, "LDS image");
+    __shared__ __attribute__((aligned(16))) float smem[RED];
+    const int Kx = g.K_dev ? min(*g.K_dev, g.K) : g.K;
+    const int nsp = g.K_dev ? dw_used_splits(g.splits, Kx) : g.splits;
+    const int z = blockIdx.y;
+    if (z >= nsp) return;
+    const int kchunk = (Kx + nsp - 1) / nsp;
+    const int kbeg = z * kchunk, kend = min(Kx, kbeg + kchunk);
+    const int wave = __builtin_amdgcn_readfirstlane(threadIdx.x >> 6), lane = threadIdx.x & 63;
+    const int n0 = (int)blockIdx.x * THIN_TN_COLS;
+    const bool cok = n0 + lane < g.N;
+    const float* __restrict__ Bp = B + n0 + (cok ? lane : 0);
+    float acc[MR];
+#pragma unroll
+    for (int m = 0; m < MR; ++m) acc[m] = 0.0f;
+    for (int t0 = kbeg; t0 < kend; t0 += THIN_TN_TILE) {
+        float bv[THIN_TN_RPW];
+#pragma unroll
+        for (int u = 0; u < THIN_TN_RPW; ++u) {
+            const int r = t0 + wave + u * THIN_TN_WAVES;
+            bv[u] = r < kend ? Bp[(size_t)r * g.ldb] : 0.0f;
+        }
+        const int nq = min(THIN_TN_TILE, kend - t0) * (MR / 4);
+        for (int q = threadIdx.x; q < nq; q += THIN_TN_WAVES * 64) {
+            const int row = q / (MR / 4), mq = (q % (MR / 4)) * 4;
+            *reinterpret_cast<float4*>(smem + row * MR + mq) = *reinterpret_cast<const float4*>(A + (size_t)(t0 + row) * g.lda + mq);
+        }
+        __syncthreads();
+#pragma unroll
+        for (int u = 0; u < THIN_TN_RPW; ++u) {
+            const int lr = wave + u * THIN_TN_WAVES;
+            if (t0 + lr < kend) {
+                const float* a = smem + lr * MR;
+#pragma unroll
+                for (int m = 0; m < MR; ++m) acc[m] = fmaf(a[m], bv[u], acc[m]);
+            }
+        }
+        __syncthreads();
+    }
+#pragma unroll
+    for (int m = 0; m < MR; ++m) smem[(wave * MR + m) * THIN_TN_COLS + lane] = acc[m];
+    __syncthreads();
+    float* __restrict__ C = Cout + (size_t)z * g.slab;
+    for (int e = threadIdx.x; e < MR * THIN_TN_COLS; e += THIN_TN_WAVES * 64) {
+        const int m = e / THIN_TN_COLS, c = e % THIN_TN_COLS;
+        float t = smem[e];
+#pragma unroll
+        for (int w = 1; w < THIN_TN_WAVES; ++w) t += smem[w * MR * THIN_TN_COLS + e];
+        if (n0 + c < g.N) C[(size_t)m * g.ldc + n0 + c] = t;
+    }
+}
+
+static bool thin_enabled() {
+    static const bool on = [] { const char* v = getenv("EAGCN_NO_THIN_GEMM"); return !(v && v[0] == '1'); }();
+    return on;
+}
+static bool aligned16(const void* p) { return (reinterpret_cast<uintptr_t>(p) % 16) == 0; }
+
+bool gemm_thin_nn_ok(const GemmDesc& g) {
+    return thin_enabled() && g.ta == 0 && g.tb == 0 && g.K >= 4 && g.K <= 32 && (g.K % 4) == 0 && g.splits == 1 && !g.K_dev &&
+           g.prof_tag != PROF_HEAD && g.vecB && (g.lda % 4) == 0 && aligned16(g.A) && (g.ldc % 4) == 0 && aligned16(g.C) &&
+           cdiv(g.N, 256) <= 65535;
+}
+bool gemm_thin_tn_ok(const GemmDesc& g) {
+    return thin_enabled() && g.ta == 1 && g.tb == 0 && g.M >= 4 && g.M <= 32 && !g.M_dev && g.prof_tag != PROF_HEAD && g.vecA &&
+           g.vecB && (g.ldc % 4) == 0 && aligned16(g.C) && (g.slab % 4) == 0;
+}
+int gemm_thin_tn_slabs(const GemmDesc& g) {
+    return std::max(1, std::min(std::min(g.splits, 16), 256 / std::max(1, cdiv(g.N, THIN_TN_COLS))));
+}
+
+template <int KR>
+static void thin_nn_go(const GemmDesc& g, hipStream_t s) {
+    gemm_thin_nn_kernel<KR><<<dim3(cdiv(g.M, 4 * THIN_NN_ROWS), cdiv(g.N, 256)), 256, 0, s>>>(g, g.A, g.B, g.C);
+}
+int launch_gemm_thin_nn(const GemmDesc& g, hipStream_t s) {
+    ProfScope ps(g.prof_tag, s, g.work > 0.0 ? g.work : 2.0 * g.M * g.N * g.K);
+    switch (g.K) {
+        case 4: thin_nn_go<4>(g, s); break;
+        case 8: thin_nn_go<8>(g, s); break;
+        case 12: thin_nn_go<12>(g, s); break;
+        case 16: thin_nn_go<16>(g, s); break;
+        case 20: thin_nn_go<20>(g, s); break;
+        case 24: thin_nn_go<24>(g, s); break;
+        case 28: thin_nn_go<28>(g, s); break;
+        default: thin_nn_go<32>(g, s); break;
+    }
+    EAGCN_LAUNCH_CHECK();
+    return EAGCN_OK;
+}
+
+template <int MR>
+static void thin_tn_go(const GemmDesc& g, hipStream_t s) {
+    gemm_thin_tn_kernel<MR><<<dim3(cdiv(g.N, THIN_TN_COLS), g.splits), THIN_TN_WAVES * 64, 0, s>>>(g, g.A, g.B, g.C);
+}
+int launch_gemm_thin_tn(const GemmDesc& g0, hipStream_t s) {
+    GemmDesc g = g0;
+    g.splits = gemm_thin_tn_slabs(g0);
+    ProfScope ps(g.prof_tag, s, g.work > 0.0 ? g.work : 2.0 * g.M * g.N * g.K);
+    switch (g.M) {
+        case 4: thin_tn_go<4>(g, s); break;
+        case 8: thin_tn_go<8>(g, s); break;
+        case 12: thin_tn_go<12>(g, s); break;
+        case 16: thin_tn_go<16>(g, s); break;
+        case 20: thin_tn_go<20>(g, s); break;
+        case 24: thin_tn_go<24>(g, s); break;
+        case 28: thin_tn_go<28>(g, s); break;
+        default: thin_tn_go<32>(g, s); break;
+    }
+    EAGCN_LAUNCH_CHECK();
+    return EAGCN_OK;
+}
+
+}
diff --git a/eagcn_amd/csrc/head.hip b/eagcn_amd/csrc/head.hip
--- a/eagcn_amd/csrc/head.hip
+++ b/eagcn_amd/csrc/head.hip
@@ -142,6 +142,7 @@
     double* hws;
     double* hsb;
     void* layer; size_t layer_bytes;
+    float* dwdef[4];
 };
 static size_t carve_scratch(void* base, const eagcn_batch* b, const eagcn_model* m, ModelScratch* out) {
     Carver2 c(base);
@@ -171,6 +172,8 @@
     s.dpad = c.take<float>((size_t)EAGCN_MAX_VIEWS * ldmax);
     s.layer_bytes = lbytes;
     s.layer = c.take<char>(lbytes);
+    s.dwdef[0] = nullptr;
+    for (int l = 1; l < 4; ++l) s.dwdef[l] = l < m->n_layers ? c.take<float>(layer_dw_slab_floats(b, &m->layer[l])) : nullptr;
     if (out) *out = s;
     return c.off;
 }
@@ -650,6 +653,8 @@
     EdgeDrain pend_in, pend_out;
     pend_in.eacc = nullptr;
     pend_out.eacc = nullptr;
+    DwPendList dw_pending;
+    dw_pending.n = 0;
     for (int l = layer_hi; l >= layer_lo; --l) {
         const int t = top_l - l;
         float* cur = (t & 1) ? sc.dxb : sc.dxa;
@@ -665,12 +670,15 @@
         w.x_planes = l > 0 ? sv.L[l - 1].xout_planes : nullptr;
         const bool top = l == top_l;
         const float* dpad = (weighted && top) ? sc.dpad : nullptr;
+        DwDefer dw_defer{(l > layer_lo && !input_only) ? sc.dwdef[l] : nullptr, &dw_pending};
         RC(layer_backward_impl(b, &m->layer[l], &w, top ? nullptr : cur, top ? &rgd : nullptr, dpad,
                                l > 0 ? other : dx0, input_only ? nullptr : &lg[l], stream, top && sampled, top ? &zb : nullptr,
-                               pend_in.eacc ? &pend_in : nullptr, (l > layer_lo && !input_only) ? &pend_out : nullptr, input_only));
+                               pend_in.eacc ? &pend_in : nullptr, (l > layer_lo && !input_only) ? &pend_out : nullptr, input_only,
+                               &dw_defer));
         pend_in = pend_out;
         if (l == layer_lo) pend_in.eacc = nullptr;
     }
+    EAGCN_CHECK_ARG(dw_pending.n == 0, "eagcn_model_backward: a weight-gradient slab sum was left pending");
     if (forked) RC(stream_after(s, side));
     return EAGCN_OK;
 }
diff --git a/eagcn_amd/csrc/kernels.h b/eagcn_amd/csrc/kernels.h
--- a/eagcn_amd/csrc/kernels.h
+++ b/eagcn_amd/csrc/kernels.h
@@ -202,12 +202,30 @@
     double* eacc; int K;
     float* datt_w[EAGCN_MAX_VIEWS]; float* dself_r[EAGCN_MAX_VIEWS]; int channels[EAGCN_MAX_VIEWS];
     const float* rsig;
-};
+    int tree;
+};
+constexpr int DW_PENDING_MAX = 3;
+struct DwPending {
+    float* dW[EAGCN_MAX_VIEWS];
+    ViewCols vc;
+    ColMapD in;
+    const float* slabs;
+    size_t slab;
+    int ld_in, fp;
+    int nsplit;
+    int wblocks, xk_G, bx_per, bx_wide;
+};
+struct DwPendList { int n; DwPending d[DW_PENDING_MAX]; };
+struct DwDefer {
+    float* region;
+    DwPendList* list;
+};
+size_t layer_dw_slab_floats(const eagcn_batch* b, const eagcn_layer_params* p);
 int layer_backward_impl(const eagcn_batch* b, const eagcn_layer_params* p, const eagcn_layer_bufs* w,
                         const float* dxout, const ReadoutGrad* rg, const float* dpad_row, float* dx,
                         const eagcn_layer_grads* g, void* stream, bool dpad_views = false,
                         const ZeroJob* zero_after = nullptr, const EdgeDrain* drain_in = nullptr, EdgeDrain* drain_out = nullptr,
-                        bool input_only = false);
+                        bool input_only = false, DwDefer* defer = nullptr);
 int model_backward_input_packed(const eagcn_batch* b, const eagcn_model* m, const int64_t* size, void* saved, size_t saved_bytes,
                                 void* scratch, size_t scratch_bytes, const float* dout, const float* dgraph_rep,
                                 const eagcn_layer_grads* lg, const eagcn_head_grads* hg, float** dx0, void* stream, const char* who);
diff --git a/eagcn_amd/csrc/layer.hip b/eagcn_amd/csrc/layer.hip
--- a/eagcn_amd/csrc/layer.hip
+++ b/eagcn_amd/csrc/layer.hip
@@ -360,6 +360,8 @@
             double t = 0.0;
 #pragma unroll
             for (int z = 0; z < EDGE_COPIES; ++z) { t += v[z]; a.drain.eacc[((size_t)z * K + k) * EDGE_SLAB + c] = 0.0; }
+            static_assert(EDGE_COPIES == 8, "pairwise order of unpack_grads' sixteen lanes");
+            if (a.drain.tree) t = ((v[0] + v[4]) + (v[2] + v[6])) + ((v[1] + v[5]) + (v[3] + v[7]));
             float* dw = nullptr;
             float* dr = nullptr;
             int ch = 0;
@@ -571,18 +573,14 @@
     }
 }
 
-__global__ __launch_bounds__(256) void unpack_grads_kernel(GradPtrs gp, ParamPtrs pp, ViewCols vc, ColMapD in,
-                                                            int ld_in, int fp, const float* __restrict__ dWcat,
-                                                            int nsplit, size_t slab, double* __restrict__ datt,
-                                                            int nedge, const float* __restrict__ rsig, int wblocks,
-                                                            const int32_t* __restrict__ meta, int xk_G, int edge_drain, int bx_per, int bx_wide) {
-    nedge = nedge < 0 ? -nedge : min(nedge, (meta[EAGCN_META_T] + 15) / 16);
+__device__ __forceinline__ void unpack_slabs(float* const* dW, const ViewCols& vc, const ColMapD& in, int ld_in, int fp,
+                                             const float* __restrict__ dWcat, int nsplit, size_t slab,
+                                             const int32_t* __restrict__ meta, int xk_G, int bx_per, int bx_wide, int tid) {
     const int bxm = bx_wide ? BX3W_BM : BX3_BM, bxn = bx_wide ? BX3W_BN : BX3_BN;
     nsplit = nsplit < 0 ? bx3_used_splits_wave(-nsplit, meta[EAGCN_META_T], ((ld_in + bxm - 1) / bxm) * ((fp + bxn - 1) / bxn),
                                           bx_per > 0 ? ((meta[EAGCN_META_T] + bxm - 1) / bxm) * ((ld_in + bxn - 1) / bxn) : 0, max(1, (fp + 31) >> 5), bx_per)
-                        : max(1, min(nsplit, meta[EAGCN_META_T] >> 7));
-    if ((int)blockIdx.x < wblocks) {
-        const int tid = blockIdx.x * blockDim.x + threadIdx.x;
+                        : dw_used_splits(nsplit, meta[EAGCN_META_T]);
+    {
         if (xk_G > 0) {
             const int e = tid;
             if (e >= ld_in * fp) return;
@@ -600,7 +598,7 @@
             float t = 0.0f;
 #pragma unroll
             for (int x = 0; x < G3_XSEG; ++x) t += v[x];
-            gp.dW[k][(size_t)fi * vc.width[k] + f] = T > 0 ? t : 0.0f;
+            dW[k][(size_t)fi * vc.width[k] + f] = T > 0 ? t : 0.0f;
             return;
         }
         const int sub = tid & 3;
@@ -627,7 +625,32 @@
 #pragma unroll
         for (int j = 0; j < 4; ++j) { t[j] += __shfl_xor(t[j], 1); t[j] += __shfl_xor(t[j], 2); }
         const float tv = sub == 0 ? t[0] : sub == 1 ? t[1] : sub == 2 ? t[2] : t[3];
-        if (f + sub < vc.width[k]) gp.dW[k][(size_t)fi * vc.width[k] + f + sub] = tv;
+        if (f + sub < vc.width[k]) dW[k][(size_t)fi * vc.width[k] + f + sub] = tv;
+    }
+}
+
+__global__ __launch_bounds__(256) void unpack_grads_kernel(GradPtrs gp, ParamPtrs pp, ViewCols vc, ColMapD in,
+                                                            int ld_in, int fp, const float* __restrict__ dWcat,
+                                                            int nsplit, size_t slab, double* __restrict__ datt,
+                                                            int nedge, const float* __restrict__ rsig, int wblocks,
+                                                            const int32_t* __restrict__ meta, int xk_G, int edge_drain, int bx_per, int bx_wide,
+                                                            int own_blocks, DwPendList pend) {
+    if ((int)blockIdx.x >= own_blocks) {
+        int first = own_blocks;
+        for (int i = 0; i < pend.n; ++i) {
+            const DwPending& d = pend.d[i];
+            if ((int)blockIdx.x < first + d.wblocks) {
+                unpack_slabs(d.dW, d.vc, d.in, d.ld_in, d.fp, d.slabs, d.nsplit, d.slab, meta, d.xk_G, d.bx_per, d.bx_wide,
+                             ((int)blockIdx.x - first) * blockDim.x + threadIdx.x);
+                return;
+            }
+            first += d.wblocks;
+        }
+        return;
+    }
+    nedge = nedge < 0 ? -nedge : min(nedge, (meta[EAGCN_META_T] + 15) / 16);
+    if ((int)blockIdx.x < wblocks) {
+        unpack_slabs(gp.dW, vc, in, ld_in, fp, dWcat, nsplit, slab, meta, xk_G, bx_per, bx_wide, blockIdx.x * blockDim.x + threadIdx.x);
         return;
     }
     const int er = ((int)blockIdx.x - wblocks) * 16 + (threadIdx.x >> 4), sl = threadIdx.x & 15;
@@ -777,6 +800,8 @@
     if (s) *s = t;
     return c.off;
 }
+static size_t dw_slab_floats(const LayerDims& d) { return d.wslab * std::max(std::max(d.nsplit, G3_XSEG), d.np ? d.bx_splits : 1); }
+size_t layer_dw_slab_floats(const eagcn_batch* b, const eagcn_layer_params* p) { return dw_slab_floats(layer_dims(b, p)); }
 static size_t carve_bwd(void* base, const eagcn_batch* b, const LayerDims& d, BwdScratch* s) {
     Carver c(base);
     BwdScratch t;
@@ -792,7 +817,7 @@
     t.dY = c.take<float>((size_t)std::max(b->T, 1) * d.fp);
     t.dP = c.take<float>((size_t)std::max(b->T, 1) * d.fp);
     t.cc = c.take<float>((size_t)2 * d.fp);
-    t.dWcat = c.take<float>(d.wslab * std::max(std::max(d.nsplit, G3_XSEG), d.np ? d.bx_splits : 1));
+    t.dWcat = c.take<float>(dw_slab_floats(d));
     t.slab = c.take<double>((size_t)d.gxb * d.fp * 2);
     t.slab_da = c.take<double>((size_t)d.gxb * cdiv(d.fp, 1024) * EAGCN_MAX_VIEWS);
     t.datt = c.take<double>((size_t)edge_grid_x(b) * EAGCN_MAX_VIEWS * EDGE_SLAB);
@@ -1089,6 +1114,15 @@
 #undef EAGCN_BWD
 }
 
+static bool edge_defer_on() {
+    static const bool on = [] { const char* v = getenv("EAGCN_NO_EDGE_DEFER"); return !(v && v[0] == '1'); }();
+    return on;
+}
+static bool dw_defer_on() {
+    static const bool on = [] { const char* v = getenv("EAGCN_NO_DW_DEFER"); return !(v && v[0] == '1'); }();
+    return on;
+}
+
 extern "C" int eagcn_layer_backward(const eagcn_batch* b, const eagcn_layer_params* p, const eagcn_layer_bufs* w,
                                     const float* dxout, const float* dpad_row, float* dx,
                                     const eagcn_layer_grads* g, void* stream) {
@@ -1103,7 +1137,7 @@
 int eagcn::layer_backward_impl(const eagcn_batch* b, const eagcn_layer_params* p, const eagcn_layer_bufs* w,
                                const float* dxout, const ReadoutGrad* rg, const float* dpad_row, float* dx,
                                const eagcn_layer_grads* g, void* stream, bool dpad_views, const ZeroJob* zero_after,
-                               const EdgeDrain* drain_in, EdgeDrain* drain_out, bool input_only) {
+                               const EdgeDrain* drain_in, EdgeDrain* drain_out, bool input_only, DwDefer* defer) {
     if (drain_out) drain_out->eacc = nullptr;
     hipStream_t s = (hipStream_t)stream;
     int rc = check_layer(b, p, "eagcn_layer_backward");
@@ -1267,6 +1301,8 @@
     int bx_wide = 0;
     hipStream_t side = w->aux_stream ? (hipStream_t)w->aux_stream : s;
     const bool forked = side != s;
+    float* dwbuf = sc.dWcat;
+    bool dw_deferred = false;
     if (b->T > 0) {
         AggArgs a;
         a.bt = *b; a.vc = d.vc; a.src = sc.dY; a.lds = d.fp; a.dst = sc.dP; a.ldd = d.fp;
@@ -1276,11 +1312,17 @@
         memset(&bx, 0, sizeof(bx));
         memset(&bw, 0, sizeof(bw));
         bool use_bx = false;
+        static const bool edge_atomic = [] { const char* v = getenv("EAGCN_EDGE_SLABS"); return !(v && v[0] == '1'); }();
+        bool general_rel = false;
+        for (int k = 0; k < p->K; ++k) general_rel = general_rel || pp.rel_vec[k] != nullptr;
+        dw_deferred = edge_defer_on() && dw_defer_on() && drain_out && defer && defer->region && defer->list &&
+                      defer->list->n < DW_PENDING_MAX && edge_atomic && !general_rel && !forked && !input_only;
+        if (dw_deferred) dwbuf = defer->region;
         if (d.np && !w->aux_stream) {
             bx.A = BxPlanes{sc.dPp, pstride, d.fp, b->T}; bx.B = BxPlanes{sc.Wp, d.wpslab, d.fp, d.ld_in}; bx.C = dx; bx.ldc = d.ld_in;
             bx.M = b->T; bx.N = d.ld_in; bx.K = d.fp; bx.M_dev = b->meta + EAGCN_META_T; bx.tn = 0; bx.splits = 1;
             bw.A = BxPlanes{w->x_planes ? w->x_planes : sc.xp, xstride, d.ld_in, b->T}; bw.B = BxPlanes{sc.dPp, pstride, d.fp, b->T};
-            bw.C = sc.dWcat; bw.ldc = d.fp; bw.M = d.ld_in; bw.N = d.fp; bw.K = b->T; bw.K_dev = b->meta + EAGCN_META_T; bw.tn = 1;
+            bw.C = dwbuf; bw.ldc = d.fp; bw.M = d.ld_in; bw.N = d.fp; bw.K = b->T; bw.K_dev = b->meta + EAGCN_META_T; bw.tn = 1;
             bw.splits = d.bx_splits; bw.slab = d.wslab;
             use_bx = bx3_ok(bw) && (!dx || bx3_ok(bx));
         }
@@ -1297,9 +1339,6 @@
         EdgeArgs e;
         e.bt = *b; e.vc = d.vc; e.dY = sc.dY; e.Y = w->Y; e.P = w->P; e.ld = d.fp; e.sig = sc.sig;
         e.rsig = sc.rsig; e.rscale = w->rscale; e.datt = sc.datt; e.atomic = 0;
-        static const bool edge_atomic = [] { const char* v = getenv("EAGCN_EDGE_SLABS"); return !(v && v[0] == '1'); }();
-        bool general_rel = false;
-        for (int k = 0; k < p->K; ++k) general_rel = general_rel || pp.rel_vec[k] != nullptr;
         if (edge_atomic && !general_rel) { e.datt = sc.eacc; e.atomic = 1; }
         static const bool colaunch = [] { const char* v = getenv("EAGCN_NO_COLAUNCH"); return !(v && v[0] == '1'); }();
         nedge = e.atomic ? -EDGE_COPIES : edge_grid_x(b);
@@ -1347,7 +1386,7 @@
         }
         if (forked) { rc = stream_after(side, s); if (rc) return rc; }
         nsplit = d.nsplit;
-        GemmDesc gw{1, 0, d.ld_in, d.fp, b->T, w->x, d.ld_in, sc.dP, d.fp, sc.dWcat, d.fp, nsplit, d.wslab, gemm_work};
+        GemmDesc gw{1, 0, d.ld_in, d.fp, b->T, w->x, d.ld_in, sc.dP, d.fp, dwbuf, d.fp, nsplit, d.wslab, gemm_work};
         gw.K_dev = b->meta + EAGCN_META_T;
         GemmDesc gx{0, 1, b->T, d.ld_in, d.fp, sc.dP, d.fp, sc.Wcat, d.fp, dx, d.ld_in, 1, 0, gemm_work};
         gx.M_dev = b->meta + EAGCN_META_T;
@@ -1379,6 +1418,7 @@
         } else {
             rc = launch_gemm(gw, side);
             if (rc) return rc;
+            nsplit = gemm_dw_slabs(gw);
             if (dx) { rc = launch_gemm(gx, s); if (rc) return rc; }
         }
     }
@@ -1391,18 +1431,35 @@
         const int wblocks = nsplit > 0 ? cdiv((int)d.wslab, 256) : 0;
         double* edge_src = nedge == -EDGE_COPIES ? sc.eacc : sc.datt;
         const int edge_drain = edge_src == sc.eacc ? 1 : 0;
-        static const bool defer_env = [] { const char* v = getenv("EAGCN_NO_EDGE_DEFER"); return !(v && v[0] == '1'); }();
-        if (defer_env && drain_out && edge_drain && wblocks == 0 && !forked && b->T > 0) {
+        if (edge_defer_on() && drain_out && edge_drain && (wblocks == 0 || dw_deferred) && !forked && b->T > 0) {
             drain_out->eacc = sc.eacc; drain_out->K = p->K; drain_out->rsig = sc.rsig;
+            drain_out->tree = wblocks > 0 ? 1 : 0;
+            if (wblocks > 0) {
+                DwPending& pd = defer->list->d[defer->list->n++];
+                memset(&pd, 0, sizeof(pd));
+                for (int k = 0; k < EAGCN_MAX_VIEWS; ++k) pd.dW[k] = gp.dW[k];
+                pd.vc = d.vc; pd.in = in; pd.slabs = dwbuf; pd.slab = d.wslab; pd.ld_in = d.ld_in; pd.fp = d.fp;
+                pd.nsplit = bx_slabs ? -nsplit : nsplit; pd.wblocks = wblocks; pd.xk_G = xk_G; pd.bx_per = bx_per; pd.bx_wide = bx_wide;
+            }
             for (int k = 0; k < EAGCN_MAX_VIEWS; ++k) {
                 drain_out->datt_w[k] = gp.datt_w[k]; drain_out->dself_r[k] = gp.dself_r[k]; drain_out->channels[k] = pp.channels[k];
             }
             return EAGCN_OK;
         }
+        EAGCN_CHECK_ARG(!dw_deferred, "eagcn_layer_backward: a deferred slab sum without its edge hand-down");
+        DwPendList pend;
+        pend.n = 0;
+        int pblocks = 0;
+        if (defer && defer->list && defer->list->n > 0) {
+            pend = *defer->list;
+            defer->list->n = 0;
+            for (int i = 0; i < pend.n; ++i) pblocks += pend.d[i].wblocks;
+        }
+        const int own_blocks = wblocks + cdiv(p->K * EDGE_SLAB, 16);
         ProfScope psu(PROF_PACK, side);
-        unpack_grads_kernel<<<wblocks + cdiv(p->K * EDGE_SLAB, 16), 256, 0, side>>>(gp, pp, d.vc, in, d.ld_in, d.fp, sc.dWcat,
-                                                                                    bx_slabs ? -nsplit : nsplit, d.wslab, edge_src, nedge, sc.rsig,
-                                                                                    wblocks, b->meta, xk_G, edge_drain, bx_per, bx_wide);
+        unpack_grads_kernel<<<own_blocks + pblocks, 256, 0, side>>>(gp, pp, d.vc, in, d.ld_in, d.fp, dwbuf,
+                                                                    bx_slabs ? -nsplit : nsplit, d.wslab, edge_src, nedge, sc.rsig,
+                                                                    wblocks, b->meta, xk_G, edge_drain, bx_per, bx_wide, own_blocks, pend);
         EAGCN_LAUNCH_CHECK();
     }
     if (forked) { rc = stream_after(s, side); if (rc) return rc; }
```

Result: slower. 554,400 (-20.8%).
